# TengdaHan/DPC

Measured on AMD Instinct MI355X. Metric: clips/sec (train step, B x8x3x5xHxW), higher is better.
Workload: dtype bf16; 1 GPU; cfg2: resnet18 2d3d, img_dim 128, seq_len 5, num_seq 8, pred_step 3, batch 128/GPU, full train step (fwd+CE/top-k+bwd+all-reduce+Adam); global_batch=128, parallelism=dp1, init=reference init, random, launch=hipGraph replay, streams=2

## Files before the change

### dpc_amd/_lib.py

```python
from __future__ import annotations

import ctypes as C
import os
from typing import Optional

import torch

_HERE = os.path.dirname(os.path.abspath(__file__))
HIP_LIB_PATH = os.path.join(_HERE, "libdpc_hip.so")
EMU_LIB_PATH = os.path.join(os.path.dirname(_HERE), "tests", "simt_emu", "libdpc_emu.so")

F32, BF16 = 0, 1
ERR_ARG, ERR_LAUNCH, ERR_UNSUPPORTED = -1, -2, -3
ABI_VERSION = 2


def dtype_code(dt: torch.dtype) -> int:
    if dt == torch.float32:
        return F32
    if dt == torch.bfloat16:
        return BF16
    raise TypeError(f"unsupported dtype {dt}")


class ConvDesc(C.Structure):
    _fields_ = [(n, C.c_int32) for n in (
        "dtype_in", "dtype_out", "mode", "N", "RT", "RH", "RW", "ST", "SH", "SW", "Ci", "src_ld",
        "Co", "ldw", "ldo", "KT", "KH", "KW", "st", "sh", "sw", "pt", "ph", "pw")]


class GruChainDesc(C.Structure):
    _fields_ = ([(n, C.c_int32) for n in ("dtype", "M", "D", "SQ", "P", "n_agg", "n_steps", "reserved")] +
                [("p_drop", C.c_float), ("reserved2", C.c_uint32), ("seed", C.c_uint64)] +
                [(n, C.c_void_p) for n in ("step_dev", "drop_masks", "packed", "bias_u", "bias_r", "bias_o", "bias_1", "bias_2",
                                           "X_all", "H_all", "HR_all", "U_all", "R_all", "O_all", "P1_all", "pred",
                                           "d_pred", "G_all", "dP1", "dP2", "d_x", "ws", "d_hlast")])


class LcHeadDesc(C.Structure):
    _fields_ = ([(n, C.c_int32) for n in ("dtype", "B", "SQ", "D", "num_class", "train")] +
                [("p_drop", C.c_float), ("momentum", C.c_float), ("eps", C.c_float), ("reserved", C.c_uint32), ("seed", C.c_uint64)] +
                [(n, C.c_void_p) for n in ("step_dev", "drop_mask", "h_last", "bn_weight", "bn_bias", "bn_running_mean", "bn_running_var",
                                           "bn_num_batches", "fc_weight", "fc_bias", "target", "ctx", "xhat", "bn_out", "y", "stat",
                                           "logits", "dlogits", "row_ws", "result", "g_fc_weight", "g_fc_bias", "g_bn_weight",
                                           "g_bn_bias", "dctx", "d_hlast", "d_bn_out")])


class AdamSegment(C.Structure):
    _fields_ = [("begin", C.c_int64), ("end", C.c_int64), ("lr", C.c_float), ("weight_decay", C.c_float), ("active", C.c_int32),
                ("reserved", C.c_int32)]


ADAM_MAX_SEGMENTS = 512


class GradState(C.Structure):
    _fields_ = [("sumsq", C.c_double), ("norm", C.c_float), ("coef", C.c_float), ("skip", C.c_int32), ("n_skipped", C.c_int32),
                ("n_clipped", C.c_int32), ("reserved", C.c_int32)]


GRAD_PARTIALS = 1024
ACCUM_ADD, ACCUM_FINISH = 0, 1


class LambSegment(C.Structure):
    _fields_ = [("begin", C.c_int64), ("end", C.c_int64), ("lr", C.c_float), ("weight_decay", C.c_float), ("active", C.c_int32),
                ("adapt", C.c_int32), ("chunk0", C.c_int32), ("n_chunks", C.c_int32), ("reserved", C.c_int32 * 2)]


class LambChunk(C.Structure):
    _fields_ = [("begin", C.c_int64), ("len", C.c_int32), ("seg", C.c_int32)]


class LambRecord(C.Structure):
    _fields_ = [("sum_p2", C.c_double), ("sum_u2", C.c_double), ("pnorm", C.c_float), ("unorm", C.c_float), ("ratio", C.c_float),
                ("reserved", C.c_int32)]


LAMB_CHUNK = 4096

LR_CONSTANT, LR_COSINE, LR_LINEAR, LR_MULTISTEP = 0, 1, 2, 3
LR_MAX_MILESTONES = 8


class LrSchedule(C.Structure):
    _fields_ = [("kind", C.c_int32), ("warmup_steps", C.c_int32), ("total_steps", C.c_int32), ("n_milestones", C.c_int32),
                ("min_mult", C.c_double), ("gamma", C.c_double), ("milestones", C.c_int32 * LR_MAX_MILESTONES)]


class LrState(C.Structure):
    _fields_ = [("mult", C.c_float), ("k", C.c_int32), ("reserved", C.c_int32 * 2)]


class ConvEpilogue(C.Structure):
    _fields_ = [(n, C.c_void_p) for n in ("addend", "addend_mask", "bn_raw", "bn_mask", "bn_mean", "bn_invstd", "stats")]


class Resample(C.Structure):
    _fields_ = [("xb", C.c_void_p), ("xk", C.c_void_p), ("yb", C.c_void_p), ("yk", C.c_void_p), ("ksx", C.c_int32), ("ksy", C.c_int32)]


class RecipeDesc(C.Structure):
    _fields_ = ([(n, C.c_double) for n in ("sized_p", "gray_p", "jitter_p", "brightness", "contrast", "saturation", "hue")] +
                [("flip_code", C.c_int32), ("flags", C.c_int32)])


RECIPE_JITTER_CONSISTENT, RECIPE_SCALE_AFTER_SIZED = 1, 2


def recipe_slots(n_frames: int) -> int:
    return 58 + 9 * n_frames


class PackEntry(C.Structure):
    _fields_ = [("in_", C.c_void_p), ("out", C.c_void_p), ("d0", C.c_int32), ("d1", C.c_int32), ("d2", C.c_int32), ("block0", C.c_int32),
                ("s0", C.c_int64), ("s1", C.c_int64), ("s2", C.c_int64)]


class Copy2dEntry(C.Structure):
    _fields_ = [("src", C.c_void_p), ("dst", C.c_void_p), ("src_ld", C.c_int64), ("dst_ld", C.c_int64), ("rows", C.c_int32), ("cols", C.c_int32),
                ("block0", C.c_int32), ("pad", C.c_int32)]


class DpcError(RuntimeError):
    pass


_vp, _i32, _i64, _f32, _f64 = C.c_void_p, C.c_int32, C.c_int64, C.c_float, C.c_double
_SIGS = {
    "dpc_abi_version": [],
    "dpc_conv_stats_rows": [C.POINTER(ConvDesc)],
    "dpc_conv_igemm": [C.POINTER(ConvDesc), _vp, _vp, _vp, _vp, _vp, _vp],
    "dpc_conv_igemm_ex": [C.POINTER(ConvDesc), _vp, _vp, _vp, C.POINTER(ConvEpilogue), _vp],
    "dpc_gemm_nt_splitk": [_i32, _i32, _i32, _i32, _vp, _i32, _vp, _i32, _vp, C.POINTER(_i32), _vp],
    "dpc_gemm_tn_splitk": [_i32, _i32, _i32, _i32, _vp, _i32, _vp, _i32, _vp, C.POINTER(_i32), _vp],
    "dpc_conv_wgrad": [C.POINTER(ConvDesc), _vp, _vp, _i32, _vp, C.POINTER(_i32), _vp],
    "dpc_conv_plan": [C.POINTER(ConvDesc), _i32, _i32, _i32, C.c_char_p, _i32],
    "dpc_last_kernel": [C.c_char_p, _i32],
    "dpc_set_reserved_cus": [_i32],
    "dpc_set_f32_matmul": [_i32],
    "dpc_diag_squat": [_i32, _i32, _i32, _i32, _i32, _vp, _i64, _vp, _vp, _vp],
    "dpc_pack3d": [_vp, _vp, _i32, _i32, _i32, _i32, _i64, _i64, _i64, _vp],
    "dpc_pack3d_multi": [_vp, _i32, _i32, _i32, _vp],
    "dpc_reduce_unpack": [_vp, _i32, _vp, _i32, _i32, _i32, _i64, _i64, _i64, _i32, _vp],
    "dpc_transpose2d_bf16x2": [_vp, _vp, _i32, _vp, _vp, _i32, _i32, _i32, _vp],
    "dpc_transpose2d": [_vp, _i32, _i32, _vp, _i32, _i32, _i32, _i32, _vp],
    "dpc_pack_input_s2d": [_vp, _vp, _i32, _i32, _i32, _i32, _i32, _vp],
    "dpc_synthetic_input": [_vp, _vp, _i32, _i32, _i32, _i32, _i32, C.c_uint64, _vp, _vp],
    "dpc_synthetic_labels": [_vp, _i32, _i32, C.c_uint64, _vp, _vp],
    "dpc_pack_stem_weight": [_vp, _vp, _i32, _i32, _vp],
    "dpc_unpack_stem_wgrad": [_vp, _i32, _vp, _i32, _vp],
    "dpc_bn_finalize": [_vp, _i32, _i32, _f64, _vp, _vp, _f32, _vp, _vp, _vp, _vp, _vp],
    "dpc_bn_apply": [_vp, _vp, _i32, _i64, _i32, _vp, _vp, _vp, _vp, _vp, _i32, _vp, _vp],
    "dpc_bn_bwd_reduce": [_vp, _vp, _vp, _vp, _i32, _i64, _i32, _vp, _vp, _i32, _vp, C.POINTER(_i32), _vp],
    "dpc_bn_bwd_finalize": [_vp, _i32, _i32, _f64, _vp, _vp, _vp, _vp],
    "dpc_bn_bwd_apply": [_vp, _vp, _vp, _vp, _i32, _i64, _i32, _vp, _vp, _vp, _vp, _i32, _vp, _vp, _vp],
    "dpc_bn_relu_maxpool_fwd": [_vp, _i32, _i32, _i32, _i32, _i32, _vp, _vp, _vp, _vp, _vp],
    "dpc_maxpool_bwd": [_vp, _vp, _i32, _i32, _i32, _i32, _i32, _vp, _vp],
    "dpc_tpool_split_fwd": [_vp, _i32, _i32, _i32, _i32, _i32, _i32, _i32, _vp, _vp, _vp],
    "dpc_tpool_split_bwd": [_vp, _vp, _vp, _i32, _i32, _i32, _i32, _i32, _i32, _i32, _vp, _vp],
    "dpc_colsum": [_vp, _i32, _i32, _i32, _i32, _vp, _i32, _vp, _i64, _vp],
    "dpc_pool_bn_bwd_reduce": [_vp, _vp, _vp, _i32, _i32, _i32, _i32, _i32, _vp, _vp, _vp, C.POINTER(_i32), _vp],
    "dpc_pooled_bn_bwd_reduce": [_vp, _vp, _vp, _i32, _i64, _i32, _vp, _vp, _vp, C.POINTER(_i32), _vp],
    "dpc_pool_bn_bwd_apply": [_vp, _vp, _vp, _i32, _i32, _i32, _i32, _i32, _vp, _vp, _vp, _vp, _vp, _vp],
    "dpc_mask_gen": [_vp, _i32, _i32, _i32, _vp],
    "dpc_ce_topk": [_vp, _i32, _i32, _i32, _vp, _vp, _vp, _i32, _i32, _vp],
    "dpc_ce_topk_bf16": [_vp, _i32, _i32, _i32, _vp, _vp, _vp, _i32, _vp],
    "dpc_step_advance": [_vp, _vp, _f64, _f64, _vp],
    "dpc_adam_dev": [_vp, _vp, _vp, _vp, _i64, _f32, _f64, _f64, _f32, _f32, _vp, _f32, _vp],
    "dpc_adam_groups_dev": [_vp, _vp, _vp, _vp, _i64, _vp, _i32, _f64, _f64, _f32, _vp, _f32, _vp],
    "dpc_grad_sumsq": [_vp, _i64, _vp, _i32, _vp, _vp],
    "dpc_grad_verdict": [_vp, _i32, _f64, _i32, _vp, _vp],
    "dpc_step_advance_gated": [_vp, _vp, _f64, _f64, _vp, _vp],
    "dpc_adam_dev_ex": [_vp, _vp, _vp, _vp, _i64, _f32, _f64, _f64, _f32, _f32, _vp, _f32, _vp, _vp],
    "dpc_adam_groups_dev_ex": [_vp, _vp, _vp, _vp, _i64, _vp, _i32, _f64, _f64, _f32, _vp, _f32, _vp, _vp],
    "dpc_grad_scale": [_vp, _i64, _vp, _i32, _vp, _vp],
    "dpc_grad_accumulate": [_vp, _vp, _i64, _i64, _i64, _vp, _i32, _i32, _f32, _vp],
    "dpc_adam_dev_ema": [_vp, _vp, _vp, _vp, _i64, _f32, _f64, _f64, _f32, _f32, _vp, _f32, _vp, _vp, _vp, _f32, _vp],
    "dpc_adam_groups_dev_ema": [_vp, _vp, _vp, _vp, _i64, _vp, _i32, _f64, _f64, _f32, _vp, _f32, _vp, _vp, _vp, _f32, _vp],
    "dpc_arena_swap": [_vp, _vp, _i64, _vp],
    "dpc_step_advance_sched": [_vp, _vp, _f64, _f64, _vp, C.POINTER(LrSchedule), _vp, _vp],
    "dpc_adam_dev_sched": [_vp, _vp, _vp, _vp, _i64, _f32, _f64, _f64, _f32, _f32, _vp, _f32, _vp, _vp, _vp, _f32, _vp, _vp],
    "dpc_adam_groups_dev_sched": [_vp, _vp, _vp, _vp, _i64, _vp, _i32, _f64, _f64, _f32, _vp, _f32, _vp, _vp, _vp, _f32, _vp, _vp],
    "dpc_adamw_dev": [_vp, _vp, _vp, _vp, _i64, _f32, _f64, _f64, _f32, _f32, _vp, _f32, _vp, _vp, _vp, _f32, _vp, _vp],
    "dpc_adamw_groups_dev": [_vp, _vp, _vp, _vp, _i64, _vp, _i32, _f64, _f64, _f32, _vp, _f32, _vp, _vp, _vp, _f32, _vp, _vp],
    "dpc_lamb_build_chunks": [C.POINTER(LambSegment), _i32, _i64, C.POINTER(LambChunk), _i32],
    "dpc_lamb_moments": [_vp, _vp, _vp, _vp, _i64, _vp, _i32, _vp, _i32, _f64, _f64, _f32, _vp, _f32, _vp, _vp, _vp],
    "dpc_lamb_ratios": [_vp, _i32, _vp, _i32, _vp, _vp, _vp],
    "dpc_lamb_apply": [_vp, _vp, _vp, _i64, _vp, _i32, _vp, _i32, _f32, _vp, _vp, _vp, _vp, _vp, _f32, _vp, _vp],
    "dpc_counter_advance": [_vp, _vp],
    "dpc_copy2d_f32": [_vp, _i64, _vp, _i64, _i32, _i32, _vp],
    "dpc_copy2d_multi": [_vp, _i32, _i32, _vp],
    "dpc_dropout_mask": [_vp, _i64, _f32, C.c_uint64, _vp, _vp],
    "dpc_gru_pack": [_vp, _vp, _vp, _vp, _vp, _i32, _i32, _vp, _vp],
    "dpc_gru_chain_fwd": [C.POINTER(GruChainDesc), _vp],
    "dpc_gru_chain_bwd": [C.POINTER(GruChainDesc), _vp],
    "dpc_score_ws_floats": [_i32, _i32, C.POINTER(_i64), C.POINTER(_i64)],
    "dpc_score_fwd": [_vp, _vp, _i32, _i32, _vp, _vp, _vp, _vp, _vp, _vp],
    "dpc_score_bwd": [_vp, _vp, _vp, _i32, _i32, _i32, _vp, _i32, _vp, _vp],
    "dpc_ce_finalize": [_vp, _i32, _vp, _vp],
    "dpc_bn_finalize_running": [_vp, _i32, _i32, _f64, _vp, _vp, _f32, _vp, _vp, _vp, _vp, _vp, _vp, _vp, _f32, _vp],
    "dpc_bn_eval_coeffs": [_vp, _vp, _vp, _vp, _f32, _i32, _vp, _vp, _vp, _vp, _vp],
    "dpc_relu_tpool_fwd": [_vp, _i32, _i32, _i32, _i32, _i32, _i32, _vp, _vp],
    "dpc_relu_tpool_bwd": [_vp, _vp, _i32, _i32, _i32, _i32, _i32, _i32, _vp, _vp],
    "dpc_lc_head_fwd": [C.POINTER(LcHeadDesc), _vp],
    "dpc_lc_head_bwd": [C.POINTER(LcHeadDesc), _vp],
    "dpc_frames_to_input": [_vp, _i32, _i32, _i32, _i32, _vp, _vp, _i32, _i32, _i32, _i32, _i32, _vp, _vp, _i32, _i32,
                            C.POINTER(C.c_float), C.POINTER(C.c_float), _vp, _vp, _i32, _vp],
    "dpc_frames_to_input_ex": [_vp, _i32, _i32, _i32, _i32, _vp, _vp, _i32, _i32, _i32, _i32, _i32, C.POINTER(Resample), _vp, _vp, _vp,
                               C.POINTER(C.c_float), C.POINTER(C.c_float), _vp, _vp, _i32, _vp],
    "dpc_video_windows_to_input": [_vp, _i32, _i32, _i32, _i32, _vp, _i32, _i32, _i32, _i32, _i32, C.POINTER(Resample),
                                   C.POINTER(C.c_float), C.POINTER(C.c_float), _vp, _vp, _i32, _vp],
    "dpc_store_to_input": [_vp, _i32, _i64, _i32, _i32, _vp, _vp, _i32, _i32, _i32, _i32, _i32, C.POINTER(Resample), _vp, _vp, _vp,
                           C.POINTER(C.c_float), C.POINTER(C.c_float), _vp, _vp, _i32, _vp, _vp],
    "dpc_draw_recipe": [C.POINTER(RecipeDesc), _vp, _vp, _vp, _i32, _i32, _i32, _i32, _i32, _i32, _i32, _i32, _i32, _vp, C.c_uint64, _vp, _vp,
                        _vp, _vp, _vp, _vp, _vp, _vp, _vp, _vp, _vp],
    "dpc_draw_recipe_ex": [C.POINTER(RecipeDesc), _vp, _vp, _vp, _vp, _vp, _i32, _i32, _i32, _i32, _i32, _i32, _i32, _i32, _i32, _vp, C.c_uint64,
                           _vp, _vp, _vp, _vp, _vp, _vp, _vp, _vp, _vp, _vp, _vp, _vp],
    "dpc_lc_test_accumulate": [_vp, _i32, _i32, _i32, _i32, _vp, _vp, _vp, _vp],
    "dpc_lc_test_finish": [_vp, _vp, _vp, _i32, _i32, _vp, _vp, _vp, _vp, _vp],
    "dpc_embed_accumulate": [_vp, _i32, _i32, _i32, _i32, _vp, _vp, _vp],
    "dpc_embed_finish": [_vp, _vp, _i32, _f32, _vp, _vp],
    "dpc_knn_ws_bytes": [_i32, _i32, _i32],
    "dpc_knn_topk": [_vp, _i32, _i32, _vp, _i32, _i32, _i32, _i32, _vp, _i32, _vp, _vp, _vp, _i64, _vp],
    "dpc_knn_recall": [_vp, _i32, _i32, _vp, _vp, _i32, _i32, _vp, _i32, _vp, _vp, _vp, _vp],
    "dpc_stem_wgrad_fused": [C.POINTER(ConvDesc), _vp, _vp, _vp, _vp, _vp, _vp, _vp, _vp, _vp, C.POINTER(_i32), _vp],
    "dpc_adam": [_vp, _vp, _vp, _vp, _i64, _f32, _f32, _f32, _f32, _f32, _f32, _f32, _f32, _vp],
}


class Lib:

    def __init__(self, path: str, kind: str):
        if not os.path.exists(path):
            raise DpcError(
                f"{path} not found: build it with `make` (or __graft_entry__.build()); "
                "dpc_amd has no CPU/eager fallback")
        self.kind = kind
        self.path = path
        self.c = C.CDLL(path)
        self._bound = {}
        if self.call("dpc_abi_version") != ABI_VERSION:
            raise DpcError("ABI version mismatch")

    def _fn(self, name: str):
        fn = self._bound.get(name)
        if fn is None:
            fn = getattr(self.c, name)
            fn.argtypes = _SIGS[name]
            fn.restype = C.c_int
            self._bound[name] = fn
        return fn

    def missing_symbols(self):
        return [n for n in _SIGS if not hasattr(self.c, n)]

    def stream(self) -> C.c_void_p:
        if self.kind == "hip":
            return C.c_void_p(torch.cuda.current_stream().cuda_stream)
        return C.c_void_p(0)

    def call(self, name: str, *args) -> int:
        conv = [C.c_void_p(a.data_ptr()) if isinstance(a, torch.Tensor) else a for a in args]
        rc = self._fn(name)(*conv)
        if rc < 0:
            raise DpcError(f"{name} failed with code {rc}")
        return rc


PLAN_IGEMM, PLAN_WGRAD, PLAN_ADDEND, PLAN_STATS, PLAN_ADDEND_MASK, PLAN_BNRED = 0, 1, 1, 2, 4, 8


def conv_plan(lib: "Lib", desc: ConvDesc, op: int = PLAN_IGEMM, addend: bool = False, stats: bool = False, dy_ld: int = 0,
              addend_mask: bool = False, bnred: bool = False) -> str:
    buf = C.create_string_buffer(192)
    flags = ((PLAN_ADDEND if addend else 0) | (PLAN_STATS if stats else 0) | (PLAN_ADDEND_MASK if addend_mask else 0) |
             (PLAN_BNRED if bnred else 0))
    rc = lib._fn("dpc_conv_plan")(C.byref(desc), op, flags, dy_ld or desc.Co, buf, 192)
    if rc == -3:
        return ""
    if rc < 0:
        raise DpcError(f"dpc_conv_plan failed with code {rc}")
    return buf.value.decode()


def last_kernel(lib: "Lib") -> str:
    buf = C.create_string_buffer(192)
    lib.call("dpc_last_kernel", buf, 192)
    return buf.value.decode()
# ... 27 lines not shown
```

### dpc_amd/csrc/conv_wgrad.hip

```cpp
#include "conv_common.h"
#include <stdlib.h>

struct WgradParams {
    GatherGeom g;
    const void* src;
    const void* dy;
    float* part;
    int Co, dy_ld;
    int nks, kcps;
    int ntm, ntn;
    int x6;
};

template <class T> struct Transposer;
template <> struct Transposer<float> {
    static __device__ __forceinline__ void run(const u32x4 (&v)[4], u32x4 (&o)[4]) {
        DPC_UNROLL
        for (int c = 0; c < 4; ++c) {
            u32x4 t = {v[0][c], v[1][c], v[2][c], v[3][c]};
            o[c] = t;
        }
    }
};
template <> struct Transposer<bf16_t> {
// ... 79 lines not shown
        u_pg[i] = loc / per_row;
        u_tp[i] = decode_k(g, tile_n * TN + u_cu[i] * E);
    }

    f32x16 acc[MI][NT];
    DPC_UNROLL
    for (int i = 0; i < MI; ++i)
        DPC_UNROLL
        for (int j = 0; j < NT; ++j)
            DPC_UNROLL
            for (int r = 0; r < 16; ++r) acc[i][j][r] = 0.f;

    const char* const zero = (const char*)dpc_zero16;
    u32x4 rv[NU][E];
    auto load_chunk = [&](int chunk) {
        DPC_UNROLL
        for (int i = 0; i < NU; ++i) {
            const int m_first = chunk * BKP + u_pg[i] * E;
            if (!u_on[i]) continue;
            if (u_isA[i]) {
                const int co = tile_m * TM + u_cu[i] * E;
                const bool cok = co + E <= p.dy_ld && co < p.Co;
                const char* a = (const char*)p.dy + ((long long)m_first * p.dy_ld + co) * esz;
                DPC_UNROLL
                for (int e = 0; e < E; ++e) {
                    const bool ok = cok && m_first + e < g.M;
                    rv[i][e] = *(const u32x4*)(ok ? a + (long long)e * p.dy_ld * esz : zero);
                }
            } else if (ROWFAST) {
                const RowIt it = rowit_decode(g, m_first < g.M ? m_first : 0);
                const TapPos& tp = u_tp[i];
                const int ti = it.rt * g.st - g.pt + tp.kt, hi = it.rh * g.sh - g.ph + tp.kh;
                const int wi0 = it.rw * g.sw - g.pw + tp.kw;
                const bool rok = tp.ok && m_first < g.M && (unsigned)ti < (unsigned)g.ST && (unsigned)hi < (unsigned)g.SH;
                const long long off0 = ((((long long)(it.n * g.ST + ti) * g.SH + hi) * g.SW) + wi0) * g.src_ld + tp.ci;
                const char* a = (const char*)p.src + off0 * esz;
                const long long step = (long long)g.sw * g.src_ld * esz;
                DPC_UNROLL
                for (int e = 0; e < E; ++e) {
                    const bool ok = rok && (unsigned)(wi0 + e * g.sw) < (unsigned)g.SW;
                    rv[i][e] = *(const u32x4*)(ok ? a + e * step : zero);
                }
            } else {
                RowIt it = rowit_decode(g, m_first < g.M ? m_first : 0);
                DPC_UNROLL
                for (int e = 0; e < E; ++e) {
                    const int m = m_first + e;
                    long long off = gather_off(g, rowit_pos(g, it), u_tp[i]);
                    if (m >= g.M) off = -1;
                    rv[i][e] = *(const u32x4*)(off >= 0 ? (const char*)p.src + off * esz : zero);
                    rowit_next(g, it);
                }
            }
        }
    };
    auto store_chunk = [&](int buf) {
        unsigned char* As = lds + buf * (TM + TN) * 128;
        unsigned char* Bs = As + TM * 128;
        DPC_UNROLL
        for (int i = 0; i < NU; ++i) {
            if (!u_on[i]) continue;
            u32x4 o[E];
            Transposer<T>::run(rv[i], o);
            unsigned char* base = u_isA[i] ? As : Bs;
            DPC_UNROLL
            for (int c = 0; c < E; ++c) *(u32x4*)(base + lds_unit_off3(u_cu[i] * E + c, u_pg[i])) = o[c];
        }
    };

    if (c_begin < c_end) {
        load_chunk(c_begin);
        store_chunk(0);
    }
    __syncthreads();
    for (int ch = c_begin; ch < c_end; ++ch) {
        const int buf = (ch - c_begin) & 1;
        if (ch + 1 < c_end) load_chunk(ch + 1);
        const unsigned char* As = lds + buf * (TM + TN) * 128;
        const unsigned char* Bs = As + TM * 128;
        bool done = false;
        if constexpr (sizeof(T) == 4) {
            if (p.x6) {
                DPC_UNROLL
                for (int kp = 0; kp < 2; ++kp) {
                    const int u0 = 4 * kp + lhi, u1 = u0 + 2;
                    Split3 sa[MI], sb[NT];
                    DPC_UNROLL
                    for (int i = 0; i < MI; ++i)
                        sa[i] = split3_f32x8(*(const u32x4*)(As + lds_unit_off3(wm * (TM / 2) + i * 32 + l31, u0)),
                                             *(const u32x4*)(As + lds_unit_off3(wm * (TM / 2) + i * 32 + l31, u1)));
                    DPC_UNROLL
                    for (int j = 0; j < NT; ++j)
                        sb[j] = split3_f32x8(*(const u32x4*)(Bs + lds_unit_off3(wn * (TN / 2) + j * 32 + l31, u0)),
                                             *(const u32x4*)(Bs + lds_unit_off3(wn * (TN / 2) + j * 32 + l31, u1)));
                    DPC_UNROLL
                    for (int i = 0; i < MI; ++i)
                        DPC_UNROLL
                        for (int j = 0; j < NT; ++j) acc[i][j] = mfma_f32x6(sa[i], sb[j], acc[i][j]);
                }
                done = true;
            }
        }
        if (!done) {
        DPC_UNROLL
        for (int kk = 0; kk < 4; ++kk) {
            const int unit = 2 * kk + lhi;
            u32x4 fa[MI], fb[NT];
            DPC_UNROLL
            for (int i = 0; i < MI; ++i) fa[i] = *(const u32x4*)(As + lds_unit_off3(wm * (TM / 2) + i * 32 + l31, unit));
            DPC_UNROLL
            for (int j = 0; j < NT; ++j) fb[j] = *(const u32x4*)(Bs + lds_unit_off3(wn * (TN / 2) + j * 32 + l31, unit));
            DPC_UNROLL
            for (int i = 0; i < MI; ++i)
                DPC_UNROLL
                for (int j = 0; j < NT; ++j) acc[i][j] = mfma_unit<T>(fa[i], fb[j], acc[i][j]);
        }
        }
        if (ch + 1 < c_end) store_chunk(buf ^ 1);
        __syncthreads();
    }

    DPC_UNROLL
    for (int j = 0; j < NT; ++j) {
        const int col = tile_n * TN + wn * (TN / 2) + j * 32 + l31;
        if (col < g.Kp) {
            DPC_UNROLL
            for (int i = 0; i < MI; ++i)
                DPC_UNROLL
                for (int r = 0; r < 16; ++r) {
                    const int row = tile_m * TM + wm * (TM / 2) + i * 32 + (r & 3) + 8 * (r >> 2) + 4 * lhi;
                    if (row < p.Co) p.part[((long long)ks * p.Co + row) * g.Kp + col] = acc[i][j][r];
                }
        }
    }
}


struct Wgrad2Params {
    GatherGeom g;
    const void* src;
    const void* dy;
    float* part;
    int Co, dy_ld;
    int nks, kcps;
    int ntm, ntn;
    int lRW, lRH;
    int RWm, RHm;
    int Mv;
    int xcd_remap;
    int x6;
};

template <class T, int NWM, int NWN, bool PU>
__global__ __launch_bounds__(64 * NWM * NWN, 2) void wgrad2_kernel(Wgrad2Params p) {
    constexpr int E = Elt<T>::PER16;
    constexpr int ESZ = (int)sizeof(T);
    constexpr int BKP = 8 * E;
    constexpr int RB = 64 * ESZ;
    constexpr int SPR = RB / 16;
    constexpr int RPI = 64 / SPR;
    constexpr int SUB = BKP * RB;
    constexpr int NW = NWM * NWN, NS = NWM + NWN;
    constexpr int RR = (8 + NW - 1) / NW;
    constexpr int STAGE = NS * SUB;
    constexpr int TM = 64 * NWM, TN = 64 * NWN;
    __shared__ __attribute__((aligned(1024))) unsigned char lds[2 * STAGE];

    const GatherGeom& g = p.g;
    const int tid = threadIdx.x;
    const int lane = tid & 63;
#ifdef DPC_SIMT_EMU
    const int wv = tid >> 6;
#else
    const int wv = __builtin_amdgcn_readfirstlane(tid >> 6);
#endif
    const int wm = wv / NWN, wn = wv % NWN;
    const int l31 = lane & 31, lhi = lane >> 5;
    int id = blockIdx.x;
    if (p.xcd_remap) {
        const int nwg = gridDim.x, q = nwg >> 3, r = nwg & 7, x = id & 7;
        id = (x < r ? x * (q + 1) : r * (q + 1) + (x - r) * q) + (id >> 3);
    }
    const int tile_n = id % p.ntn; id /= p.ntn;
    const int tile_m = id % p.ntm;
    const int ks = id / p.ntm;

    const int nchunks_total = (p.Mv + BKP - 1) / BKP;
    const int c_begin = ks * p.kcps;
    const int c_end = (c_begin + p.kcps < nchunks_total) ? c_begin + p.kcps : nchunks_total;

    const int rowlane = lane / SPR, pslot = lane % SPR;
    const int lslot = (ESZ == 2) ? (pslot ^ (2 * (rowlane & 3))) : pslot;
    const int cch = lslot * E;
    int r_row[RR], r_w[RR], r_h[RR], r_q[RR], r_dh[RR], r_real[RR];
    bool r_wok[RR];
    DPC_UNROLL
    for (int rr = 0; rr < RR; ++rr) {
        const int r = (wv + rr * NW) * RPI + rowlane;
        r_row[rr] = r;
        r_w[rr] = (r & p.RWm) * g.sw - g.pw;
        r_h[rr] = ((r >> p.lRW) & p.RHm) * g.sh - g.ph;
        r_q[rr] = r >> (p.lRW + p.lRH);
        r_dh[rr] = r >> p.lRW;
        r_wok[rr] = (r & p.RWm) < g.RW;
        r_real[rr] = r_dh[rr] * g.RW + (r & p.RWm);
    }
    int a_off[RR][NWM];
    DPC_UNROLL
    for (int sa = 0; sa < NWM; ++sa) {
        const int co = tile_m * TM + sa * 64 + cch;
        const bool ok = co + E <= p.dy_ld && co < p.Co;
        DPC_UNROLL
        for (int rr = 0; rr < RR; ++rr) a_off[rr][sa] = ok && r_wok[rr] ? (r_real[rr] * p.dy_ld + co) * ESZ : -1;
    }
    TapPos tp[NWN];
    int b_off[RR][NWN], b_h[RR][NWN];
    const int ldb = g.src_ld * ESZ;
    DPC_UNROLL
    for (int sb = 0; sb < NWN; ++sb) {
        tp[sb] = decode_k(g, tile_n * TN + sb * 64 + cch);
        DPC_UNROLL
        for (int rr = 0; rr < RR; ++rr) {
            const int wi = r_w[rr] + tp[sb].kw;
            const bool ok = tp[sb].ok && (unsigned)wi < (unsigned)g.SW;
            b_h[rr][sb] = ok ? r_h[rr] + tp[sb].kh : (1 << 29);
            b_off[rr][sb] = ((tp[sb].kt * g.SH + r_h[rr] + tp[sb].kh) * g.SW + wi) * ldb + tp[sb].ci * ESZ;
        }
    }

    f32x16 acc[2][2];
    DPC_UNROLL
    for (int i = 0; i < 2; ++i)
        DPC_UNROLL
        for (int j = 0; j < 2; ++j)
            DPC_UNROLL
            for (int r = 0; r < 16; ++r) acc[i][j][r] = 0.f;

    const char* const zero = (const char*)dpc_zero16;
    auto issue = [&](int chunk, int buf) {
        const int m0 = chunk * BKP;
        unsigned char* stage = lds + buf * STAGE;
        const unsigned q0 = (unsigned)m0 >> (p.lRW + p.lRH);
        const int h0v = PU ? (int)(((unsigned)m0 >> p.lRW) & (unsigned)p.RHm) : 0;
        const int h0 = h0v * g.sh;
        const long long m0r = PU ? ((long long)q0 * g.RH + h0v) * g.RW : (long long)m0;
        const char* abase = (const char*)p.dy + m0r * p.dy_ld * ESZ;
        const char* bbase = (const char*)p.src;
        bool tv[NWN];
        if (PU) {
            const unsigned n = fdiv(q0, g.dRT);
            const int t00 = ((int)q0 - (int)n * g.RT) * g.st - g.pt;
            bbase += (long long)(((int)n * g.ST + t00) * g.SH + h0) * g.SW * ldb;
            DPC_UNROLL
            for (int sb = 0; sb < NWN; ++sb) tv[sb] = (unsigned)(t00 + tp[sb].kt) < (unsigned)g.ST;
        }
        DPC_UNROLL
        for (int rr = 0; rr < RR; ++rr) {
            const int rg = wv + rr * NW;
            if (rg < 8) {
                const bool mok = m0 + r_row[rr] < p.Mv && r_wok[rr] && (!PU || h0v + r_dh[rr] < g.RH);
                DPC_UNROLL
                for (int sa = 0; sa < NWM; ++sa)
                    glds16((mok & (a_off[rr][sa] >= 0)) ? abase + a_off[rr][sa] : zero, stage + sa * SUB + rg * 1024, lane);
                if (PU) {
                    DPC_UNROLL
                    for (int sb = 0; sb < NWN; ++sb) {
                        const bool ok = mok & tv[sb] & ((unsigned)(h0 + b_h[rr][sb]) < (unsigned)g.SH);
                        glds16(ok ? bbase + b_off[rr][sb] : zero, stage + (NWM + sb) * SUB + rg * 1024, lane);
                    }
                } else {
                    const unsigned q = q0 + (unsigned)r_q[rr];
                    const unsigned n = fdiv(q, g.dRT);
                    const int t0 = ((int)q - (int)n * g.RT) * g.st - g.pt;
                    const char* pb = bbase + (long long)(((int)n * g.ST + t0) * g.SH) * g.SW * ldb;
                    DPC_UNROLL
                    for (int sb = 0; sb < NWN; ++sb) {
                        const bool ok = mok & ((unsigned)(t0 + tp[sb].kt) < (unsigned)g.ST) & ((unsigned)b_h[rr][sb] < (unsigned)g.SH);
                        glds16(ok ? pb + b_off[rr][sb] : zero, stage + (NWM + sb) * SUB + rg * 1024, lane);
                    }
                }
            }
        }
    };

    int fo[2];
    if (ESZ == 2) {
        const int gq = lane >> 4, s16 = lane & 15;
        DPC_UNROLL
        for (int i = 0; i < 2; ++i) {
            const int colb = (i * 32 + (gq & 1) * 16 + 4 * (s16 & 3)) * 2;
            fo[i] = ((gq >> 1) * 8 + (s16 >> 2)) * RB + ((((colb >> 4) ^ (2 * (s16 >> 2))) & 7) << 4) + (colb & 15);
        }
    } else {
        DPC_UNROLL
        for (int i = 0; i < 2; ++i) fo[i] = lhi * RB + (i * 32 + l31) * 4;
    }

    auto compute = [&](int buf) {
        const unsigned char* As = lds + buf * STAGE + wm * SUB;
        const unsigned char* Bs = lds + buf * STAGE + (NWM + wn) * SUB;
#ifndef DPC_SIMT_EMU
        if constexpr (ESZ == 2) {
            constexpr int LOOKAHEAD = 4;
            const uint32_t as = (uint32_t)(uintptr_t)(__attribute__((address_space(3))) const unsigned char*)As;
            const uint32_t bs = (uint32_t)(uintptr_t)(__attribute__((address_space(3))) const unsigned char*)Bs;
            uint32_t ad[2][2];
            DPC_UNROLL
            for (int i = 0; i < 2; ++i) { ad[0][i] = as + fo[i]; ad[1][i] = bs + fo[i]; }
            u32x2 lo[2][2][2], hi[2][2][2];
            auto load = [&](auto Ic) {
                constexpr int I = decltype(Ic)::value;
                constexpr int kk = I / 4, r4 = I % 4;
                constexpr int op = (r4 == 1 || r4 == 2) ? 1 : 0, fr = (r4 >= 2) ? 1 : 0;
                asm volatile("ds_read_b64_tr_b16 %0, %1 offset:%2" : "=v"(lo[kk & 1][op][fr]) : "v"(ad[op][fr]), "n"((kk * 16) * RB) : "memory");
                __builtin_amdgcn_sched_barrier(0);
                asm volatile("ds_read_b64_tr_b16 %0, %1 offset:%2" : "=v"(hi[kk & 1][op][fr]) : "v"(ad[op][fr]), "n"((kk * 16 + 4) * RB) : "memory");
                __builtin_amdgcn_sched_barrier(0);
            };
            __builtin_amdgcn_sched_barrier(0);
            static_for<16>([&](auto Mc) {
                constexpr int m = decltype(Mc)::value;
                constexpr int kk = m / 4, q = m % 4;
                constexpr int idx = 4 * kk + (q == 0 ? 1 : q == 1 ? 2 : 3);
                constexpr int idx_prev = m == 0 ? -1 : (q == 0 ? 4 * (kk - 1) + 3 : 4 * kk + (q == 1 ? 1 : q == 2 ? 2 : 3));
                constexpr int f_prev = m == 0 ? 0 : (idx_prev + 1 + LOOKAHEAD < 16 ? idx_prev + 1 + LOOKAHEAD : 16);
                constexpr int f_now = idx + 1 + LOOKAHEAD < 16 ? idx + 1 + LOOKAHEAD : 16;
                static_for<f_now - f_prev>([&](auto Dc) { load(std::integral_constant<int, f_prev + decltype(Dc)::value>{}); });
                asm volatile("s_waitcnt lgkmcnt(%0)" ::"n"(2 * (f_now - idx - 1)) : "memory");
                __builtin_amdgcn_sched_barrier(0);
                constexpr int i = q >> 1, j = q & 1, s = kk & 1;
                const u32x4 av = {lo[s][0][i][0], lo[s][0][i][1], hi[s][0][i][0], hi[s][0][i][1]};
                const u32x4 bv = {lo[s][1][j][0], lo[s][1][j][1], hi[s][1][j][0], hi[s][1][j][1]};
                acc[i][j] = mfma_32x32x16_bf16(av, bv, acc[i][j]);
                __builtin_amdgcn_sched_barrier(0);
            });
            return;
        }
#endif
        if (ESZ == 2) {
            DPC_UNROLL
            for (int kk = 0; kk < 4; ++kk) {
                u32x4 fa[2], fb[2];
                DPC_UNROLL
                for (int i = 0; i < 2; ++i) {
                    const u32x2 a0 = lds_read_tr16(As + fo[i] + (kk * 16) * RB);
                    const u32x2 a1 = lds_read_tr16(As + fo[i] + (kk * 16 + 4) * RB);
                    const u32x2 b0 = lds_read_tr16(Bs + fo[i] + (kk * 16) * RB);
                    const u32x2 b1 = lds_read_tr16(Bs + fo[i] + (kk * 16 + 4) * RB);
                    u32x4 ta = {a0[0], a0[1], a1[0], a1[1]};
                    u32x4 tb = {b0[0], b0[1], b1[0], b1[1]};
                    fa[i] = ta; fb[i] = tb;
                }
                DPC_UNROLL
                for (int i = 0; i < 2; ++i)
                    DPC_UNROLL
                    for (int j = 0; j < 2; ++j) acc[i][j] = mfma_32x32x16_bf16(fa[i], fb[j], acc[i][j]);
            }
        } else if (p.x6) {
            DPC_UNROLL
            for (int s16 = 0; s16 < BKP / 16; ++s16) {
                Split3 sa[2], sb[2];
                DPC_UNROLL
                for (int i = 0; i < 2; ++i) {
                    float xa[8], xb[8];
                    DPC_UNROLL
                    for (int e = 0; e < 8; ++e) {
                        xa[e] = *(const float*)(As + fo[i] + 2 * (8 * s16 + e) * RB);
                        xb[e] = *(const float*)(Bs + fo[i] + 2 * (8 * s16 + e) * RB);
                    }
                    sa[i] = split3_f32(xa);
                    sb[i] = split3_f32(xb);
                }
                DPC_UNROLL
                for (int i = 0; i < 2; ++i)
                    DPC_UNROLL
                    for (int j = 0; j < 2; ++j) acc[i][j] = mfma_f32x6(sa[i], sb[j], acc[i][j]);
            }
        } else {
            DPC_UNROLL
            for (int s2 = 0; s2 < BKP / 2; ++s2) {
                float fa[2], fb[2];
                DPC_UNROLL
                for (int i = 0; i < 2; ++i) {
                    fa[i] = *(const float*)(As + fo[i] + 2 * s2 * RB);
                    fb[i] = *(const float*)(Bs + fo[i] + 2 * s2 * RB);
                }
                DPC_UNROLL
                for (int i = 0; i < 2; ++i)
                    DPC_UNROLL
                    for (int j = 0; j < 2; ++j) acc[i][j] = mfma_32x32x2_f32(fa[i], fb[j], acc[i][j]);
            }
        }
    };

    if (c_begin < c_end) issue(c_begin, 0);
    __syncthreads();
    for (int ch = c_begin; ch < c_end; ++ch) {
        const int buf = (ch - c_begin) & 1;
        if (ch + 1 < c_end) issue(ch + 1, buf ^ 1);
        compute(buf);
        __syncthreads();
    }

    DPC_UNROLL
    for (int j = 0; j < 2; ++j) {
        const int col = tile_n * TN + wn * 64 + j * 32 + l31;
        if (col < g.Kp) {
            DPC_UNROLL
            for (int i = 0; i < 2; ++i)
                DPC_UNROLL
                for (int r = 0; r < 16; ++r) {
                    const int row = tile_m * TM + wm * 64 + i * 32 + (r & 3) + 8 * (r >> 2) + 4 * lhi;
                    if (row < p.Co) p.part[((long long)ks * p.Co + row) * g.Kp + col] = acc[i][j][r];
                }
        }
    }
}

template <class T, int NWM, int NWN>
static int launch_wgrad2_t(const Wgrad2Params& p, bool pu, hipStream_t stream) {
    dim3 grid((unsigned)(p.ntm * p.ntn * p.nks)), block(64 * NWM * NWN);
    dpc_plan_detail("T=%s nwm=%d nwn=%d padded=%d", sizeof(T) == 2 ? "bf16" : "f32", NWM, NWN,
                    (int)(((p.RWm + 1) != p.g.RW) || ((p.RHm + 1) != p.g.RH)));
    if (pu) {
        DPC_LAUNCH((wgrad2_kernel<T, NWM, NWN, true>), grid, block, stream, p);
    } else {
        DPC_LAUNCH((wgrad2_kernel<T, NWM, NWN, false>), grid, block, stream, p);
    }
    return dpc_launch_status();
}

template <class T>
static int launch_wgrad2(const Wgrad2Params& p, int nwm, int nwn, bool pu, hipStream_t stream) {
    if (nwm == 1 && nwn == 3) return launch_wgrad2_t<T, 1, 3>(p, pu, stream);
    if (nwm == 1 && nwn == 4) return launch_wgrad2_t<T, 1, 4>(p, pu, stream);
    if (nwm == 2 && nwn == 2) return launch_wgrad2_t<T, 2, 2>(p, pu, stream);
    return launch_wgrad2_t<T, 2, 3>(p, pu, stream);
}

template <class T, bool RF>
static int launch_wgrad_rf(const WgradParams& p, int tm, int tn, hipStream_t stream) {
    dim3 grid((unsigned)(p.ntm * p.ntn * p.nks)), block(256);
    dpc_plan_detail("T=%s", sizeof(T) == 2 ? "bf16" : "f32");
    if (tm == 64 && tn == 64) {
        DPC_LAUNCH((wgrad_kernel<T, 64, 64, RF>), grid, block, stream, p);
    } else if (tm == 64 && tn == 128) {
        DPC_LAUNCH((wgrad_kernel<T, 64, 128, RF>), grid, block, stream, p);
    } else {
        DPC_LAUNCH((wgrad_kernel<T, 128, 128, RF>), grid, block, stream, p);
    }
    return dpc_launch_status();
}

template <class T>
static int launch_wgrad(const WgradParams& p, int tm, int tn, hipStream_t stream) {
    if (p.g.RW % Elt<T>::PER16 == 0) return launch_wgrad_rf<T, true>(p, tm, tn, stream);
    return launch_wgrad_rf<T, false>(p, tm, tn, stream);
}

extern "C" int dpc_conv_wgrad(const dpc_conv_desc* d, const void* src, const void* dy, int32_t dy_ld,
                              float* part, int32_t* nsplit, dpc_stream_t stream_) {
    hipStream_t stream = (hipStream_t)stream_;
    WgradParams p;
    p.x6 = dpc_f32_matmul_mode();
    if (!d || d->mode != 0) return DPC_ERR_ARG;
    int rc = make_gather_geom(d, &p.g);
    if (rc) return rc;
    const int per16 = d->dtype_in == DPC_BF16 ? 8 : 4;
    if (dy_ld % per16 || dy_ld < d->Co) return DPC_ERR_UNSUPPORTED;
    rc = dpc_wgrad_patch_try(d, src, dy, dy_ld, part, nsplit, stream);
    if (rc != 1) return rc;
    rc = dpc_wgrad_stem_try(d, src, dy, dy_ld, part, nsplit, stream);
    if (rc != 1) return rc;
    const int bkp = 8 * per16;
    int rwp = 1, rhp = 1;
    while (rwp < d->RW) rwp <<= 1;
    while (rhp < d->RH) rhp <<= 1;
    const bool padded = rwp != d->RW || rhp != d->RH;
    const long long mv = (long long)d->N * d->RT * rhp * rwp;
    static const int pad_on = getenv("DPC_WGRAD2_PAD") ? atoi(getenv("DPC_WGRAD2_PAD")) : 1;
    const bool v2 = bkp % rwp == 0 && mv < (1ll << 31) &&
                    (!padded || (pad_on && (rwp * rhp) % bkp == 0 && (long long)d->RW * d->RH * 10 >= (long long)rwp * rhp * 6));
    const int lrw = ilog2_exact(rwp), lrh = ilog2_exact(rhp);
    const int nchunks = (int)(((v2 ? mv : (long long)p.g.M) + bkp - 1) / bkp);
    int tm, tn, nwm = 0, nwn = 0;
    if (v2) {
        nwm = d->Co > 64 ? 2 : 1;
        const int na = nwm == 1 ? 4 : 2, nb = 3;
        const int pa = (p.g.Kp + 64 * na - 1) / (64 * na) * (64 * na), pb = (p.g.Kp + 64 * nb - 1) / (64 * nb) * (64 * nb);
        nwn = (pb < pa) ? nb : na;
        tm = 64 * nwm; tn = 64 * nwn;
    } else {
        tm = d->Co > 64 ? 128 : 64;
        tn = (p.g.Kp >= 128 || tm == 128) ? 128 : 64;
    }
    p.ntm = (d->Co + tm - 1) / tm;
    p.ntn = (p.g.Kp + tn - 1) / tn;
    static const int min_chunks = getenv("DPC_WGRAD_MINCHUNKS") ? atoi(getenv("DPC_WGRAD_MINCHUNKS")) : 16;
    static const int target_blocks = getenv("DPC_WGRAD_BLOCKS") ? atoi(getenv("DPC_WGRAD_BLOCKS")) : 512;
    int want = target_blocks / (p.ntm * p.ntn);
    if (want > nchunks / min_chunks) want = nchunks / min_chunks;
    if (want < 1) want = 1;
    if (want > nchunks) want = nchunks;
    p.kcps = (nchunks + want - 1) / want;
    p.nks = (nchunks + p.kcps - 1) / p.kcps;
    if (nsplit) *nsplit = p.nks;
    if (!part) return DPC_OK;
    if (!src || !dy) return DPC_ERR_ARG;
    p.src = src; p.dy = dy; p.part = part; p.Co = d->Co; p.dy_ld = dy_ld;
    if (v2) {
        Wgrad2Params q;
        q.g = p.g; q.src = src; q.dy = dy; q.part = part; q.Co = d->Co; q.dy_ld = dy_ld;
        q.nks = p.nks; q.kcps = p.kcps; q.ntm = p.ntm; q.ntn = p.ntn; q.lRW = lrw; q.lRH = lrh;
        q.RWm = rwp - 1; q.RHm = rhp - 1; q.Mv = (int)mv; q.x6 = p.x6;
        q.xcd_remap = 1;
        const bool pu = (rwp * rhp) % bkp == 0;
        if (d->dtype_in == DPC_F32) return launch_wgrad2<float>(q, nwm, nwn, pu, stream);
        return launch_wgrad2<bf16_t>(q, nwm, nwn, pu, stream);
    }
    if (d->dtype_in == DPC_F32) return launch_wgrad<float>(p, tm, tn, stream);
    return launch_wgrad<bf16_t>(p, tm, tn, stream);
}
```

### dpc_amd/csrc/gru.hip

```cpp
#include "dpc_rt.h"
#include "../../include/dpc_hip.h"
#include "philox.h"

static inline unsigned grid_for(long long n, int block = 256, int cap = 8192) {
    long long g = (n + block - 1) / block;
    if (g < 1) g = 1;
    if (g > cap) g = cap;
    return (unsigned)g;
}

template <class T>
__global__ __launch_bounds__(256) void colsum_kernel(const T* x, int ld, int M, int D, float* out, int rows_per_y) {
    __shared__ float red[8][32];
    const int col = blockIdx.x * 32 + (threadIdx.x & 31);
    const int rg = threadIdx.x >> 5;
    const int m0 = blockIdx.y * rows_per_y;
    const int m1 = (m0 + rows_per_y < M) ? m0 + rows_per_y : M;
    float s = 0.f;
    if (col < D)
        for (int m = m0 + rg; m < m1; m += 8) s += Elt<T>::to_f32(x[(long long)m * ld + col]);
    red[rg][threadIdx.x & 31] = s;
    __syncthreads();
    if (threadIdx.x < 32 && col < D) {
        float t = 0.f;
        DPC_UNROLL
        for (int g = 0; g < 8; ++g) t += red[g][threadIdx.x];
        out[(long long)blockIdx.y * D + col] = t;
    }
}

__global__ void colsum_finish_kernel(const float* ws, int ny, int D, float* out, int accumulate) {
    const int d = blockIdx.x * blockDim.x + threadIdx.x;
    if (d >= D) return;
    float t = 0.f;
    for (int y = 0; y < ny; ++y) t += ws[(long long)y * D + d];
    out[d] = accumulate ? out[d] + t : t;
}

extern "C" int dpc_colsum(const void* x, int32_t dtype, int32_t ld, int32_t M, int32_t D, float* out, int32_t accumulate,
                          float* ws, int64_t ws_floats, dpc_stream_t stream_) {
    hipStream_t stream = (hipStream_t)stream_;
    if (!x || !out || M <= 0 || D <= 0 || ld < D) return DPC_ERR_ARG;
    int ny = (M + 255) / 256;
    if (ny > 64) ny = 64;
    if (!ws || ws_floats < (long long)ny * D) return DPC_ERR_ARG;
    const int rpy = (M + ny - 1) / ny;
    dim3 grid((D + 31) / 32, ny), block(256);
    if (dtype == DPC_F32) {
        DPC_LAUNCH((colsum_kernel<float>), grid, block, stream, (const float*)x, ld, M, D, ws, rpy);
    } else if (dtype == DPC_BF16) {
        DPC_LAUNCH((colsum_kernel<bf16_t>), grid, block, stream, (const bf16_t*)x, ld, M, D, ws, rpy);
    } else {
        return DPC_ERR_ARG;
    }
    DPC_LAUNCH(colsum_finish_kernel, dim3((D + 255) / 256), dim3(256), stream, (const float*)ws, ny, D, out, accumulate);
    return dpc_launch_status();
}

__global__ void dropout_mask_kernel(float* mask, long long n4, long long n, unsigned long long seed, const int32_t* step_dev,
                                    uint32_t thresh24, float inv_keep) {
    const uint32_t step = (uint32_t)step_dev[0];
    for (long long i = (long long)blockIdx.x * blockDim.x + threadIdx.x; i < n4; i += (long long)gridDim.x * blockDim.x) {
        float k[4];
        dropout_keep4(seed, step, (uint32_t)i, thresh24, inv_keep, k);
        if (i * 4 + 4 <= n) {
            ((f32x4*)mask)[i] = f32x4{k[0], k[1], k[2], k[3]};
        } else {
            for (long long e = i * 4; e < n; ++e) mask[e] = k[e - i * 4];
        }
    }
}

extern "C" int dpc_dropout_mask(float* mask, int64_t n, float p, uint64_t seed, const int32_t* step_dev, dpc_stream_t stream_) {
    hipStream_t stream = (hipStream_t)stream_;
    if (!mask || n <= 0 || !step_dev || !(p >= 0.f) || !(p < 1.f) || n >= (1ll << 33)) return DPC_ERR_ARG;
    const long long n4 = (n + 3) / 4;
    DPC_LAUNCH(dropout_mask_kernel, dim3(grid_for(n4)), dim3(256), stream, mask, n4, (long long)n, (unsigned long long)seed, step_dev,
               dropout_thresh24(p), 1.f / (1.f - p));
    return dpc_launch_status();
}
```

### dpc_amd/csrc/pack.hip

```cpp
#include "dpc_rt.h"
#include "../../include/dpc_hip.h"

template <class TO>
__global__ void pack3d_kernel(const float* in, TO* out, int d0, int d1, int d2, long long s0, long long s1, long long s2) {
    const long long n = (long long)d0 * d1 * d2;
    for (long long i = (long long)blockIdx.x * blockDim.x + threadIdx.x; i < n; i += (long long)gridDim.x * blockDim.x) {
        const int i2 = (int)(i % d2);
        const long long q = i / d2;
        const int i1 = (int)(q % d1);
        const int i0 = (int)(q / d1);
        out[i] = Elt<TO>::from_f32(in[i0 * s0 + i1 * s1 + i2 * s2]);
    }
}

static inline unsigned grid_for(long long n, int block = 256, int cap = 4096) {
    long long g = (n + block - 1) / block;
    if (g < 1) g = 1;
    if (g > cap) g = cap;
    return (unsigned)g;
}

extern "C" int dpc_pack3d(const float* in, void* out, int32_t dtype_out, int32_t d0, int32_t d1, int32_t d2,
                          int64_t s0, int64_t s1, int64_t s2, dpc_stream_t stream_) {
    hipStream_t stream = (hipStream_t)stream_;
    if (!in || !out || d0 <= 0 || d1 <= 0 || d2 <= 0) return DPC_ERR_ARG;
    const long long n = (long long)d0 * d1 * d2;
    if (dtype_out == DPC_F32) {
        DPC_LAUNCH((pack3d_kernel<float>), dim3(grid_for(n)), dim3(256), stream, in, (float*)out, d0, d1, d2, (long long)s0, (long long)s1, (long long)s2);
    } else if (dtype_out == DPC_BF16) {
        DPC_LAUNCH((pack3d_kernel<bf16_t>), dim3(grid_for(n)), dim3(256), stream, in, (bf16_t*)out, d0, d1, d2, (long long)s0, (long long)s1, (long long)s2);
    } else {
        return DPC_ERR_ARG;
    }
    return dpc_launch_status();
}

template <class TO>
__global__ void pack3d_multi_kernel(const dpc_pack_entry* tab, int n_entries, TO* ) {
    int e = 0;
    while (e + 1 < n_entries && (int)blockIdx.x >= tab[e + 1].block0) ++e;
    const dpc_pack_entry t = tab[e];
    const long long n = (long long)t.d0 * t.d1 * t.d2;
    const int nblk = (e + 1 < n_entries ? tab[e + 1].block0 : (int)gridDim.x) - t.block0;
    const float* in = (const float*)t.in;
    TO* out = (TO*)t.out;
    constexpr int TJ = 64, TI_MAX = 64;
    __shared__ float tile[TJ][TI_MAX + 1];
    if (t.s1 == 1 && t.d1 <= TI_MAX && t.d1 > 1) {
        const int nj = (t.d2 + TJ - 1) / TJ;
        const int ntiles = t.d0 * nj;
        for (int tl = (int)blockIdx.x - t.block0; tl < ntiles; tl += nblk) {
            const int i0 = tl / nj, j0 = (tl - i0 * nj) * TJ;
            const int jn = t.d2 - j0 < TJ ? t.d2 - j0 : TJ;
            const float* src = in + (long long)i0 * t.s0 + (long long)j0 * t.s2;
            for (int idx = threadIdx.x; idx < jn * t.d1; idx += blockDim.x) {
                const int j = idx / t.d1, i1 = idx - j * t.d1;
                tile[j][i1] = src[(long long)j * t.s2 + i1];
            }
            __syncthreads();
            TO* dst = out + ((long long)i0 * t.d1) * t.d2 + j0;
            for (int idx = threadIdx.x; idx < t.d1 * TJ; idx += blockDim.x) {
                const int i1 = idx / TJ, j = idx - i1 * TJ;
                if (j < jn) dst[(long long)i1 * t.d2 + j] = Elt<TO>::from_f32(tile[j][i1]);
            }
            __syncthreads();
        }
        return;
    }
    for (long long i = (long long)((int)blockIdx.x - t.block0) * blockDim.x + threadIdx.x; i < n; i += (long long)nblk * blockDim.x) {
        const int i2 = (int)(i % t.d2);
        const long long q = i / t.d2;
        const int i1 = (int)(q % t.d1);
        const int i0 = (int)(q / t.d1);
        out[i] = Elt<TO>::from_f32(in[i0 * t.s0 + i1 * t.s1 + i2 * t.s2]);
    }
}

extern "C" int dpc_pack3d_multi(const dpc_pack_entry* table_dev, int32_t n_entries, int32_t total_blocks, int32_t dtype_out,
                                dpc_stream_t stream_) {
    hipStream_t stream = (hipStream_t)stream_;
    if (!table_dev || n_entries <= 0 || total_blocks < n_entries) return DPC_ERR_ARG;
    if (dtype_out == DPC_F32) {
        DPC_LAUNCH((pack3d_multi_kernel<float>), dim3((unsigned)total_blocks), dim3(256), stream, table_dev, n_entries, (float*)nullptr);
    } else if (dtype_out == DPC_BF16) {
        DPC_LAUNCH((pack3d_multi_kernel<bf16_t>), dim3((unsigned)total_blocks), dim3(256), stream, table_dev, n_entries, (bf16_t*)nullptr);
    } else {
        return DPC_ERR_ARG;
    }
    return dpc_launch_status();
}

__global__ __launch_bounds__(256) void reduce_unpack_kernel(const float* part, int nsplit, float* out, int d0, int d1, int d2, long long s0,
                                     long long s1, long long s2, int accumulate) {
    __shared__ float red[8][32];
    const long long n = (long long)d0 * d1 * d2;
    const int ol = threadIdx.x & 31, sl = threadIdx.x >> 5;
    const long long i = (long long)blockIdx.x * 32 + ol;
    float s = 0.f;
    if (i < n)
        for (int k = sl; k < nsplit; k += 8) s += part[(long long)k * n + i];
    red[sl][ol] = s;
    __syncthreads();
    if (sl == 0 && i < n) {
        float t = 0.f;
        DPC_UNROLL
        for (int k = 0; k < 8; ++k) t += red[k][ol];
        const int i2 = (int)(i % d2);
        const long long q = i / d2;
        const int i1 = (int)(q % d1);
        const int i0 = (int)(q / d1);
        float* o = out + i0 * s0 + i1 * s1 + i2 * s2;
        *o = accumulate ? (*o + t) : t;
    }
}

__global__ __launch_bounds__(256) void reduce_unpack4_kernel(const float* part, int nsplit, float* out, int d0, int d1, int d2, long long s0,
                                      long long s1, long long s2, int accumulate) {
    __shared__ float red[8][32][4];
    const long long n = (long long)d0 * d1 * d2;
    const int ol = threadIdx.x & 31, sl = threadIdx.x >> 5;
    const long long i = ((long long)blockIdx.x * 32 + ol) * 4;
    float acc[8][4];
    DPC_UNROLL
    for (int j = 0; j < 8; ++j)
        DPC_UNROLL
        for (int e = 0; e < 4; ++e) acc[j][e] = 0.f;
    if (i < n) {
        int k = sl;
        for (; k + 56 < nsplit; k += 64) {
            u32x4 v[8];
            DPC_UNROLL
            for (int j = 0; j < 8; ++j) v[j] = *(const u32x4*)(part + (long long)(k + 8 * j) * n + i);
            DPC_UNROLL
            for (int j = 0; j < 8; ++j)
                DPC_UNROLL
                for (int e = 0; e < 4; ++e) acc[j][e] += unit_get<float>(v[j], e);
        }
        DPC_UNROLL
        for (int j = 0; j < 8; ++j)
            if (k + 8 * j < nsplit) {
                const u32x4 v0 = *(const u32x4*)(part + (long long)(k + 8 * j) * n + i);
                DPC_UNROLL
                for (int e = 0; e < 4; ++e) acc[j][e] += unit_get<float>(v0, e);
            }
    }
    float a[4], b[4];
    DPC_UNROLL
    for (int e = 0; e < 4; ++e) {
        a[e] = (acc[0][e] + acc[1][e]) + (acc[2][e] + acc[3][e]);
        b[e] = (acc[4][e] + acc[5][e]) + (acc[6][e] + acc[7][e]);
    }
    DPC_UNROLL
    for (int e = 0; e < 4; ++e) red[sl][ol][e] = a[e] + b[e];
    __syncthreads();
    if (sl == 0 && i < n) {
        const int i2 = (int)(i % d2);
        const long long q = i / d2;
        const int i1 = (int)(q % d1);
        const int i0 = (int)(q / d1);
        float* o = out + i0 * s0 + i1 * s1 + i2 * s2;
        DPC_UNROLL
        for (int e = 0; e < 4; ++e) {
            float t = 0.f;
            DPC_UNROLL
            for (int k = 0; k < 8; ++k) t += red[k][ol][e];
            o[e * s2] = accumulate ? (o[e * s2] + t) : t;
        }
    }
}

template <int NS>
__global__ __launch_bounds__(256) void reduce_unpack_few_kernel(const float* part, float* out, int d0, int d1, int d2, long long s0, long long s1,
                                                                long long s2, int accumulate) {
    const long long n = (long long)d0 * d1 * d2;
    const long long i = ((long long)blockIdx.x * 256 + threadIdx.x) * 4;
    if (i >= n) return;
    u32x4 v[NS];
    DPC_UNROLL
    for (int k = 0; k < NS; ++k) v[k] = *(const u32x4*)(part + (long long)k * n + i);
    const int i2 = (int)(i % d2);
    const long long q = i / d2;
    const int i1 = (int)(q % d1);
    const int i0 = (int)(q / d1);
    float* o = out + i0 * s0 + i1 * s1 + i2 * s2;
    DPC_UNROLL
    for (int e = 0; e < 4; ++e) {
        float t = 0.f;
        DPC_UNROLL
        for (int k = 0; k < NS; ++k) t += unit_get<float>(v[k], e);
        o[e * s2] = accumulate ? (o[e * s2] + t) : t;
    }
}

constexpr int RUT_CW = 64, RUT_MAXT = 32;
__global__ __launch_bounds__(256) void reduce_unpack_t_kernel(const float* part, int nsplit, float* out, int Co, int taps, int Ci, int accumulate) {
    __shared__ float tile[RUT_CW * (RUT_MAXT + 1)];
    const int co = blockIdx.x, c0 = blockIdx.y * RUT_CW;
    const int cw = Ci - c0 < RUT_CW ? Ci - c0 : RUT_CW;
    const int ldt = taps | 1;
    const long long n = (long long)Co * taps * Ci;
    const float* base = part + ((long long)co * taps) * Ci + c0;
    for (int e = threadIdx.x; e < taps * RUT_CW; e += 256) {
        const int tap = e / RUT_CW, c = e - tap * RUT_CW;
        if (c < cw) {
            const float* p = base + (long long)tap * Ci + c;
            float a0 = 0.f, a1 = 0.f, a2 = 0.f, a3 = 0.f;
            int k = 0;
            for (; k + 4 <= nsplit; k += 4) {
                a0 += p[(long long)k * n];
                a1 += p[(long long)(k + 1) * n];
                a2 += p[(long long)(k + 2) * n];
                a3 += p[(long long)(k + 3) * n];
            }
            for (; k < nsplit; ++k) a0 += p[(long long)k * n];
            tile[c * ldt + tap] = (a0 + a1) + (a2 + a3);
        }
    }
    __syncthreads();
    float* o = out + ((long long)co * Ci + c0) * taps;
    for (int j = threadIdx.x; j < cw * taps; j += 256) {
        const int c = j / taps, tap = j - c * taps;
        const float v = tile[c * ldt + tap];
        o[j] = accumulate ? o[j] + v : v;
    }
}

extern "C" int dpc_reduce_unpack(const float* part, int32_t nsplit, float* out, int32_t d0, int32_t d1, int32_t d2,
                                 int64_t s0, int64_t s1, int64_t s2, int32_t accumulate, dpc_stream_t stream_) {
    hipStream_t stream = (hipStream_t)stream_;
    if (!part || !out || nsplit <= 0 || d0 <= 0 || d1 <= 0 || d2 <= 0) return DPC_ERR_ARG;
    if (nsplit <= 16 && d1 > 1 && d1 <= RUT_MAXT && s1 == 1 && s2 == d1 && s0 == (int64_t)d1 * d2 && d0 <= 65535) {
        DPC_LAUNCH(reduce_unpack_t_kernel, dim3((unsigned)d0, (unsigned)((d2 + RUT_CW - 1) / RUT_CW)), dim3(256), stream, part, nsplit, out, d0, d1, d2,
                   accumulate);
        return dpc_launch_status();
    }
    const long long n = (long long)d0 * d1 * d2;
    if (d2 % 4 == 0 && ((uintptr_t)part % 16) == 0 && nsplit <= 8) {
        const dim3 grid((unsigned)((n / 4 + 255) / 256)), block(256);
#define DPC_RUF(NS) case NS: DPC_LAUNCH((reduce_unpack_few_kernel<NS>), grid, block, stream, part, out, d0, d1, d2, (long long)s0, (long long)s1, (long long)s2, accumulate); break
        switch (nsplit) { DPC_RUF(1); DPC_RUF(2); DPC_RUF(3); DPC_RUF(4); DPC_RUF(5); DPC_RUF(6); DPC_RUF(7); DPC_RUF(8); }
#undef DPC_RUF
        return dpc_launch_status();
    }
    if (d2 % 4 == 0 && ((uintptr_t)part % 16) == 0) {
        DPC_LAUNCH(reduce_unpack4_kernel, dim3((unsigned)((n / 4 + 31) / 32)), dim3(256), stream, part, nsplit, out, d0, d1, d2, (long long)s0, (long long)s1,
                   (long long)s2, accumulate);
        return dpc_launch_status();
    }
    DPC_LAUNCH(reduce_unpack_kernel, dim3((unsigned)((n + 31) / 32)), dim3(256), stream, part, nsplit, out, d0, d1, d2, (long long)s0, (long long)s1, (long long)s2, accumulate);
    return dpc_launch_status();
}

template <class TI, class TO>
__global__ void transpose2d_kernel(const TI* in, int ld_in, TO* out, int ld_out, int rows, int cols) {
    __shared__ float tile[32][33];
    const int bx = blockIdx.x * 32, by = blockIdx.y * 32;
    const int tx = threadIdx.x & 31, ty = threadIdx.x >> 5;
    for (int r = ty; r < 32; r += 8) {
        const int row = by + r, col = bx + tx;
        tile[r][tx] = (row < rows && col < cols) ? Elt<TI>::to_f32(in[(long long)row * ld_in + col]) : 0.f;
    }
    __syncthreads();
    for (int r = ty; r < 32; r += 8) {
        const int orow = bx + r, ocol = by + tx;
        if (orow < cols && ocol < rows) out[(long long)orow * ld_out + ocol] = Elt<TO>::from_f32(tile[tx][r]);
    }
}

extern "C" int dpc_transpose2d(const void* in, int32_t dtype_in, int32_t ld_in, void* out, int32_t dtype_out,
                               int32_t ld_out, int32_t rows, int32_t cols, dpc_stream_t stream_) {
    hipStream_t stream = (hipStream_t)stream_;
    if (!in || !out || rows <= 0 || cols <= 0) return DPC_ERR_ARG;
    dim3 grid((cols + 31) / 32, (rows + 31) / 32), block(256);
    if (dtype_in == DPC_F32 && dtype_out == DPC_F32) {
        DPC_LAUNCH((transpose2d_kernel<float, float>), grid, block, stream, (const float*)in, ld_in, (float*)out, ld_out, rows, cols);
    } else if (dtype_in == DPC_F32 && dtype_out == DPC_BF16) {
        DPC_LAUNCH((transpose2d_kernel<float, bf16_t>), grid, block, stream, (const float*)in, ld_in, (bf16_t*)out, ld_out, rows, cols);
    } else if (dtype_in == DPC_BF16 && dtype_out == DPC_BF16) {
        DPC_LAUNCH((transpose2d_kernel<bf16_t, bf16_t>), grid, block, stream, (const bf16_t*)in, ld_in, (bf16_t*)out, ld_out, rows, cols);
    } else if (dtype_in == DPC_BF16 && dtype_out == DPC_F32) {
        DPC_LAUNCH((transpose2d_kernel<bf16_t, float>), grid, block, stream, (const bf16_t*)in, ld_in, (float*)out, ld_out, rows, cols);
    } else {
        return DPC_ERR_ARG;
    }
    return dpc_launch_status();
}

__global__ __launch_bounds__(256) void transpose2d_bf16x2_kernel(const bf16_t* in0, const bf16_t* in1, int ld_in, bf16_t* out0, bf16_t* out1, int ld_out,
                                                                int rows, int cols) {
    __shared__ unsigned short tile[64][66];
    const bf16_t* in = blockIdx.z ? in1 : in0;
    bf16_t* out = blockIdx.z ? out1 : out0;
    const int bx = blockIdx.x * 64, by = blockIdx.y * 64;
    const int t = threadIdx.x;
    {
        DPC_UNROLL
        for (int it = 0; it < 2; ++it) {
            const int r = (t >> 3) + 32 * it, u = t & 7;
            const int row = by + r, col = bx + u * 8;
            u32x4 v = {0u, 0u, 0u, 0u};
            if (row < rows && col + 7 < cols) v = *(const u32x4*)(in + (long long)row * ld_in + col);
            else if (row < rows) {
                unsigned short e[8];
                DPC_UNROLL
                for (int k = 0; k < 8; ++k) e[k] = col + k < cols ? *(const unsigned short*)(in + (long long)row * ld_in + col + k) : (unsigned short)0;
                v[0] = e[0] | ((unsigned)e[1] << 16); v[1] = e[2] | ((unsigned)e[3] << 16);
                v[2] = e[4] | ((unsigned)e[5] << 16); v[3] = e[6] | ((unsigned)e[7] << 16);
            }
            DPC_UNROLL
            for (int k = 0; k < 4; ++k) {
                tile[r][u * 8 + 2 * k] = (unsigned short)(v[k] & 0xffffu);
                tile[r][u * 8 + 2 * k + 1] = (unsigned short)(v[k] >> 16);
            }
        }
    }
    __syncthreads();
    DPC_UNROLL
    for (int it = 0; it < 2; ++it) {
        const int c = (t >> 3) + 32 * it, u = t & 7;
        const int orow = bx + c, ocol = by + u * 8;
        if (orow >= cols) continue;
        unsigned short e[8];
        DPC_UNROLL
        for (int k = 0; k < 8; ++k) e[k] = tile[u * 8 + k][c];
        if (ocol + 7 < rows) {
            const u32x4 v = {e[0] | ((unsigned)e[1] << 16), e[2] | ((unsigned)e[3] << 16), e[4] | ((unsigned)e[5] << 16), e[6] | ((unsigned)e[7] << 16)};
            *(u32x4*)(out + (long long)orow * ld_out + ocol) = v;
        } else {
            DPC_UNROLL
            for (int k = 0; k < 8; ++k)
                if (ocol + k < rows) *(unsigned short*)(out + (long long)orow * ld_out + ocol + k) = e[k];
        }
    }
}

extern "C" int dpc_transpose2d_bf16x2(const void* in0, const void* in1, int32_t ld_in, void* out0, void* out1, int32_t ld_out, int32_t rows,
                                      int32_t cols, dpc_stream_t stream_) {
    hipStream_t stream = (hipStream_t)stream_;
    if (!in0 || !out0 || rows <= 0 || cols <= 0 || ld_in < cols || ld_out < rows) return DPC_ERR_ARG;
    if (ld_in % 8 || ld_out % 8 || (((uintptr_t)in0 | (uintptr_t)in1 | (uintptr_t)out0 | (uintptr_t)out1) % 16)) return DPC_ERR_UNSUPPORTED;
    dim3 grid((cols + 63) / 64, (rows + 63) / 64, in1 ? 2 : 1), block(256);
    DPC_LAUNCH(transpose2d_bf16x2_kernel, grid, block, stream, (const bf16_t*)in0, (const bf16_t*)in1, ld_in, (bf16_t*)out0, (bf16_t*)out1, ld_out, rows, cols);
    return dpc_launch_status();
}

template <class TO>
__global__ void pack_input_s2d_kernel(const float* in, TO* out, int BN, int T, int H, int W, int rev) {
    const int Hb = H / 2, Wb = W / 2;
    const long long cells = (long long)BN * T * Hb * Wb;
    const long long stride = (long long)gridDim.x * blockDim.x, first = (long long)blockIdx.x * blockDim.x + threadIdx.x;
    const long long nsweep = first < cells ? (cells - 1 - first) / stride + 1 : 0;
    for (long long k = 0; k < nsweep; ++k) {
        const long long i = first + (rev ? nsweep - 1 - k : k) * stride;
        const unsigned ci = (unsigned)i;
        const unsigned q1 = ci / (unsigned)Wb;
        const int wb = (int)(ci - q1 * (unsigned)Wb);
        const unsigned q2 = q1 / (unsigned)Hb;
        const int hb = (int)(q1 - q2 * (unsigned)Hb);
        const unsigned n_ = q2 / (unsigned)T;
        const int t = (int)(q2 - n_ * (unsigned)T);
        const int n = (int)n_;
        float v[16];
        DPC_UNROLL
        for (int k = 12; k < 16; ++k) v[k] = 0.f;
        DPC_UNROLL
        for (int c = 0; c < 3; ++c)
            DPC_UNROLL
            for (int sy = 0; sy < 2; ++sy) {
                const float* p = in + ((((long long)n * 3 + c) * T + t) * H + (2 * hb + sy)) * W + 2 * wb;
                const float2 x = *(const float2*)p;
                v[(sy * 2 + 0) * 3 + c] = x.x;
                v[(sy * 2 + 1) * 3 + c] = x.y;
            }
        u32x4* o = (u32x4*)(out + i * 16);
        constexpr int EPO = Elt<TO>::PER16;
        DPC_UNROLL
        for (int k = 0; k < 16 / EPO; ++k) o[k] = unit_pack<TO>(v + k * EPO);
    }
}

extern "C" int dpc_pack_input_s2d(const float* block, void* out, int32_t dtype_out, int32_t BN, int32_t T, int32_t H,
                                  int32_t W, dpc_stream_t stream_) {
    hipStream_t stream = (hipStream_t)stream_;
    if (!block || !out || BN <= 0 || T <= 0 || H <= 0 || W <= 0) return DPC_ERR_ARG;
    if ((H & 1) || (W & 1)) return DPC_ERR_UNSUPPORTED;
    const long long cells = (long long)BN * T * (H / 2) * (W / 2);
    static const int rev = getenv("DPC_PACK_REV") ? atoi(getenv("DPC_PACK_REV")) : 0;
    static const int cap = getenv("DPC_PACK_GRID") ? atoi(getenv("DPC_PACK_GRID")) : 16384;
    if (rev && (dtype_out == DPC_F32 || dtype_out == DPC_BF16)) dpc_plan_detail("rev");
    if (dtype_out == DPC_F32) {
        DPC_LAUNCH((pack_input_s2d_kernel<float>), dim3(grid_for(cells, 256, cap)), dim3(256), stream, block, (float*)out, BN, T, H, W, rev);
    } else if (dtype_out == DPC_BF16) {
        DPC_LAUNCH((pack_input_s2d_kernel<bf16_t>), dim3(grid_for(cells, 256, cap)), dim3(256), stream, block, (bf16_t*)out, BN, T, H, W, rev);
    } else {
        return DPC_ERR_ARG;
    }
    return dpc_launch_status();
}

template <class TO>
__global__ void pack_stem_weight_kernel(const float* w, TO* out, int Co) {
    const int n = Co * 256;
// ... 124 lines not shown
```

### dpc_amd/engine.py

```python
from __future__ import annotations

import atexit
import contextlib
import ctypes as C
import os
import weakref
import math
from typing import Dict, List, Optional, Sequence, Tuple

import torch

from . import _lib as L
from .plan import LAYER_PLAN, LAYER_WIDTH, block_geometry, fold_decision, out_shape_of, unit_descs, walk_blocks
BN_EPS = 1e-5


def param_shapes(network: str, widths: Sequence[int] = LAYER_WIDTH) -> "Dict[str, Tuple[int, ...]]":
    D = widths[3]
    out: Dict[str, Tuple[int, ...]] = {}
    out["backbone.conv1.weight"] = (widths[0], 3, 1, 7, 7)
    out["backbone.bn1.weight"] = (widths[0],)
    out["backbone.bn1.bias"] = (widths[0],)
    for pre, cin, planes, is3d, stride, has_ds, _ in walk_blocks(network, widths):
        pre, k = "backbone." + pre, block_geometry(is3d, stride)[0]
        out[pre + "conv1.weight"] = (planes, cin) + k
        out[pre + "bn1.weight"] = (planes,)
        out[pre + "bn1.bias"] = (planes,)
        out[pre + "conv2.weight"] = (planes, planes) + k
        out[pre + "bn2.weight"] = (planes,)
        out[pre + "bn2.bias"] = (planes,)
        if has_ds:
            out[pre + "downsample.0.weight"] = (planes, cin, 1, 1, 1)
            out[pre + "downsample.1.weight"] = (planes,)
            out[pre + "downsample.1.bias"] = (planes,)
    for gate in ("reset_gate", "update_gate", "out_gate"):
        out[f"agg.ConvGRUCell_00.{gate}.weight"] = (D, 2 * D, 1, 1)
        out[f"agg.ConvGRUCell_00.{gate}.bias"] = (D,)
    for idx in (0, 2):
        out[f"network_pred.{idx}.weight"] = (D, D, 1, 1)
        out[f"network_pred.{idx}.bias"] = (D,)
    return out


class KernelTimer:

    def __init__(self, names):
        self.names = set(names)
        self.records = []
        self.enabled = True

    def timed(self, eng, name, args):
        if not self.enabled:
            return eng.lib.call(name, *args, eng.lib.stream())
        a, b = torch.cuda.Event(enable_timing=True), torch.cuda.Event(enable_timing=True)
        a.record()
        rc = eng.lib.call(name, *args, eng.lib.stream())
        b.record()
        fl, by = algorithmic_cost(name, args)
        xf = fl * executed_fraction(name, args, L.last_kernel(eng.lib)) if fl else 0.0
        self.records.append((TIMER_FAMILY.get(name, name), eng._tag, a, b, fl, by, xf))
        return rc

    def summary(self, steps: int = 1):
        torch.cuda.synchronize()
        out = {}
        times = [r[2].elapsed_time(r[3]) for r in self.records]
        n = len(times)
        if steps > 1 and n % steps == 0:
            per = n // steps
            same = all(self.records[i][0] == self.records[i % per][0] for i in range(n))
            if same:
                for i in range(per):
                    col = sorted(times[i + k * per] for k in range(steps))
                    med = col[len(col) // 2] if len(col) % 2 else 0.5 * (col[len(col) // 2 - 1] + col[len(col) // 2])
                    for k in range(steps):
                        times[i + k * per] = med
        for (name, tag, a, b, fl, by, xf), ms in zip(self.records, times):
            for key in (name,) + ((f"tag:{tag}",) if tag else ()):
                d = out.setdefault(key, {"launches": 0, "ms": 0.0, "flops": 0.0, "bytes": 0.0, "executed_flops": 0.0})
                d["launches"] += 1
                d["ms"] += ms
                d["flops"] += fl
                d["bytes"] += by
                d["executed_flops"] += xf
        return out


TIMER_FAMILY = {"dpc_conv_igemm_ex": "dpc_conv_igemm"}
HBM_FAMILY = ("dpc_bn_apply", "dpc_bn_bwd_reduce", "dpc_bn_bwd_apply", "dpc_bn_relu_maxpool_fwd", "dpc_pool_bn_bwd_apply",
              "dpc_pooled_bn_bwd_reduce", "dpc_pack_input_s2d")


def _esz(dc):
    return 2 if dc == L.BF16 else 4


def algorithmic_cost(name, args):
    if name == "dpc_bn_apply":
        n = args[3] * args[4] * _esz(args[2])
        return 0.0, float(n * (2 + (args[7] is not None)) + (n // 16 if args[11] is not None else 0))
    if name == "dpc_bn_bwd_reduce":
        n = args[5] * args[6] * _esz(args[4])
        return 0.0, float(2 * n + (n // 16 if args[2] is not None else (n if args[1] is not None else 0)))
    if name == "dpc_bn_bwd_apply":
        n = args[5] * args[6] * _esz(args[4])
        return 0.0, float(3 * n + (n if args[13] is not None else 0) + (n // 16 if args[2] is not None else (n if args[1] is not None else 0)))
    if name == "dpc_bn_relu_maxpool_fwd":
        e, NT, H, W, Cc = _esz(args[1]), args[2], args[3], args[4], args[5]
        return 0.0, float(NT * H * W * Cc * e + NT * ((H - 1) // 2 + 1) * ((W - 1) // 2 + 1) * Cc * (e + 1))
    if name == "dpc_pool_bn_bwd_apply":
        e, NT, H, W, Cc = _esz(args[3]), args[4], args[5], args[6], args[7]
        return 0.0, float(2 * NT * H * W * Cc * e + NT * ((H - 1) // 2 + 1) * ((W - 1) // 2 + 1) * Cc * (e + 1))
    if name == "dpc_pooled_bn_bwd_reduce":
        return 0.0, float(args[4] * args[5] * (2 * _esz(args[3]) + 1))
    if name == "dpc_pack_input_s2d":
        px = args[3] * args[4] * args[5] * args[6]
        return 0.0, float(px * 3 * 4 + px * 4 * _esz(args[2]))
    if name == "dpc_score_fwd":
        return 2.0 * args[2] * args[2] * args[3], float(2 * args[2] * args[3] * 2)
    if name == "dpc_score_bwd":
        return 2.0 * args[4] * args[4] * args[5], float(2 * args[4] * args[5] * 2 + args[4] * args[5] * 4)
    if name in ("dpc_gemm_nt_splitk", "dpc_gemm_tn_splitk"):
        e = _esz(args[0])
        return 2.0 * args[1] * args[2] * args[3], float((args[1] + args[2]) * args[3] * e + args[1] * args[2] * 4)
    if name not in ("dpc_conv_igemm", "dpc_conv_igemm_ex", "dpc_conv_wgrad"):
        return 0.0, 0.0
    d = args[0]._obj
    esz = 2 if d.dtype_in == L.BF16 else 4
    osz = 2 if d.dtype_out == L.BF16 else 4
    taps = d.KT * d.KH * d.KW
    rows_out = d.N * d.RT * d.RH * d.RW
    rows_src = d.N * d.ST * d.SH * d.SW
    if name in ("dpc_conv_igemm", "dpc_conv_igemm_ex") and d.mode == 1:
        macs = rows_src * d.Ci * d.Co * taps
    else:
        macs = rows_out * d.Co * d.Ci * taps
    if taps == 16 and d.Ci == 16 and d.KT == 1:
        macs = macs * 147 // 256
    if name == "dpc_conv_igemm":
        by = rows_src * d.Ci * esz + d.Co * d.Ci * taps * esz + rows_out * d.Co * osz
    elif name == "dpc_conv_igemm_ex":
        ep = args[4]._obj
        n = rows_out * d.Co * osz
        by = rows_src * d.Ci * esz + d.Co * d.Ci * taps * esz + n
        by += (n if ep.addend else 0) + (n // 16 if ep.addend_mask else 0) + (n if ep.bn_raw else 0) + (n // 16 if ep.bn_mask else 0)
        name = "dpc_conv_igemm"
    else:
        by = rows_src * d.Ci * esz + rows_out * d.Co * esz + d.Co * d.Ci * taps * 4
    return 2.0 * macs, float(by)


def executed_fraction(name, args, kernel: str) -> float:
    if name not in ("dpc_conv_igemm", "dpc_conv_igemm_ex") or not kernel.startswith("igemm_ws_kernel"):
        return 1.0
    if os.environ.get("DPC_IGEMM_WS_TGROUP", "1") == "0":
        return 1.0
    d = args[0]._obj
    unit = d.st == 1 and d.sh == 1 and d.sw == 1
# ... 117 lines not shown
        self._coef_ready = False
        e.call("dpc_bn_bwd_apply", dy, None if mask is not None else y, mask, self.raw, dc, self.rows, self.Co, self.mean,
               self.invstd, e.PRM[self.bnname + ".weight"], e.coef, gated, dx, dz)

    def bn_prepare(self, dy: torch.Tensor, y: Optional[torch.Tensor], relu: bool, ext_mask: Optional[torch.Tensor] = None):
        e = self.eng
        dc = L.dtype_code(e.cdtype)
        mask = ext_mask if ext_mask is not None else (self.mask if relu else None)
        gated = int(relu or ext_mask is not None)
        if self.reduced_rows:
            prow, self.reduced_rows = self.reduced_rows, 0
        else:
            pr = C.c_int32(0)
            e.call("dpc_bn_bwd_reduce", dy, None if mask is not None else y, mask, self.raw, dc, self.rows, self.Co, self.mean,
                   self.invstd, gated, e.stats, C.byref(pr))
            prow = pr.value
        e.call("dpc_bn_bwd_finalize", e.stats, prow, self.Co, float(self.rows), e.G[self.bnname + ".weight"],
               e.G[self.bnname + ".bias"], e.coef)
        self._coef_ready = True

    def wgrad(self, x: torch.Tensor, draw: torch.Tensor):
        e = self.eng
        ns = C.c_int32(0)
        e.call("dpc_conv_wgrad", C.byref(self.desc_w), x, draw, self.Co, e.part, C.byref(ns))
        g = e.G[self.wname]
        if self.stem:
            e.call("dpc_unpack_stem_wgrad", e.part, ns.value, g, self.Co)
        else:
            Ci, t = self.Ci, self.taps
            e.call("dpc_reduce_unpack", e.part, ns.value, g, self.Co, t, Ci, Ci * t, 1, t, 0)

    def dgrad(self, draw: torch.Tensor, dx: torch.Tensor, addend: Optional[torch.Tensor], addend_mask: Optional[torch.Tensor] = None,
              red: "Optional[_ConvBN]" = None):
        e = self.eng
        e.side_wait()
        if addend_mask is None and red is None:
            e.call("dpc_conv_igemm", C.byref(self.desc_d), draw, self.wd, dx, addend, None)
            return
        ep = L.ConvEpilogue()
        ep.addend = addend.data_ptr() if addend is not None else None
        ep.addend_mask = addend_mask.data_ptr() if addend_mask is not None else None
        if red is not None:
            ep.bn_raw, ep.bn_mean, ep.bn_invstd = red.raw.data_ptr(), red.mean.data_ptr(), red.invstd.data_ptr()
            ep.bn_mask = red.mask.data_ptr() if red.mask is not None else None
            ep.stats = e.stats.data_ptr()
        e.call("dpc_conv_igemm_ex", C.byref(self.desc_d), draw, self.wd, dx, C.byref(ep))
        if red is not None:
            red.reduced_rows = self.stat_rows_d if not e.reserve_cus else e.lib.call("dpc_conv_stats_rows", C.byref(self.desc_d))


class _Block:

    def __init__(self, eng, pre: str, Ci: int, Co: int, is3d: bool, stride: int, in_shape, has_ds: bool, final_relu: bool):
        self.eng = eng
        k, s, p = block_geometry(is3d, stride)
        self.c1 = _ConvBN(eng, pre + "conv1.weight", pre + "bn1", Ci, Co, k, s, p, in_shape)
        self.c2 = _ConvBN(eng, pre + "conv2.weight", pre + "bn2", Co, Co, k, (1, 1, 1), p, self.c1.out_shape)
        self.ds = _ConvBN(eng, pre + "downsample.0.weight", pre + "downsample.1", Ci, Co, (1, 1, 1), s, (0, 0, 0),
                          in_shape) if has_ds else None
        self.final_relu = final_relu
        self.site = pre[len("backbone."):]
        self.out_shape = self.c2.out_shape
        self.Co = Co
        self.act1 = eng.empty(self.c1.out_shape + (Co,), eng.cdtype)
        self.out = eng.empty(self.out_shape + (Co,), eng.cdtype)
        self.x_in: Optional[torch.Tensor] = None

    def units(self):
        return [u for u in (self.c1, self.c2, self.ds) if u is not None]

    def forward(self, x):
        self.x_in = x
        self.c1.forward(x)
        self.c1.apply(self.act1, relu=True)
        self.c2.forward(self.act1)
        if self.ds is not None:
            self.ds.forward(x)
            self.c2.apply(self.out, relu=self.final_relu, res=self.ds.raw, res_unit=self.ds)
        else:
            self.c2.apply(self.out, relu=self.final_relu, res=x)
        return self.out

    def plan_backward(self, prev: "Optional[_Block]"):
        e = self.eng
        fold_c1, gate, fold_prev = (False, False, False) if not e.fold else fold_decision(
            e.lib, self.c1.desc_d, self.c2.desc_d, self.ds is not None, self.final_relu, prev is not None)
        red = bool(int(os.environ.get("DPC_FOLD_RED", "1")))
        self.fold_c1, self.gate, self.fold_prev = red and fold_c1, gate, red and fold_prev
        self.prev = prev

    def backward(self, dout: torch.Tensor, need_dx: bool = True) -> Optional[torch.Tensor]:
        e = self.eng
        oshape = tuple(self.out.shape)
        ishape = tuple(self.x_in.shape)
        omask = self.c2.mask if self.final_relu else None
        draw2 = e.scratch(oshape, exclude=[dout])
        dz = None
        if self.ds is None and not self.gate and need_dx:
            dz = e.scratch(oshape, exclude=[dout, draw2])
        self.c2.bn_backward(dout, self.out if self.final_relu else None, self.final_relu, draw2, dz)
        draw_d = None
        if self.ds is not None:
            draw_d = e.scratch(oshape, exclude=[dout, draw2])
            self.ds.bn_backward(dout, None, False, draw_d, ext_mask=omask)
        dact1 = e.scratch(oshape, exclude=[dout, draw2, draw_d, dz])
        self.c2.dgrad(draw2, dact1, None, red=self.c1 if self.fold_c1 else None)
        if self.fold_c1:
            self.c1.bn_prepare(dact1, self.act1, True)
        with e.side(reads=[draw2, draw_d], site=self.site + "c2"):
            if self.ds is not None:
                self.ds.wgrad(self.x_in, draw_d)
            self.c2.wgrad(self.act1, draw2)
        draw1 = draw2 if e._side is None or e.timer is not None else e.scratch(oshape, exclude=[dout, draw2, draw_d, dz, dact1])
        self.c1.bn_backward(dact1, self.act1, True, draw1)
        if not need_dx:
            with e.side(reads=[draw1], site=self.site + "c1"):
                self.c1.wgrad(self.x_in, draw1)
            return None
        if self.ds is not None:
            dx = e.scratch(ishape, exclude=[])
            self.c1.dgrad(draw1, dx, None)
            self.ds.dgrad(draw_d, dx, dx)
        elif self.gate:
            dx = dout
            self.c1.dgrad(draw1, dx, dout, addend_mask=omask, red=self.prev.c2 if self.fold_prev else None)
            if self.fold_prev:
                pv = self.prev
                pv.c2.bn_prepare(dx, pv.out if pv.final_relu else None, pv.final_relu)
        else:
            dx = dact1
            self.c1.dgrad(draw1, dx, dz)
        with e.side(reads=[draw1], site=self.site + "c1"):
            self.c1.wgrad(self.x_in, draw1)
        return dx


ENGINES: "weakref.WeakValueDictionary[int, BackboneEngine]" = weakref.WeakValueDictionary()


def engine_of(param: torch.Tensor) -> "Optional[BackboneEngine]":
    a = param.data_ptr()
    for base, eng in list(ENGINES.items()):
        if base <= a < base + eng.flat_p.numel() * 4:
            return eng
    return None


class BackboneEngine:
    BN_MOMENTUM = 0.1

    def __init__(self, shapes: "Dict[str, Tuple[int, ...]]", network: str, sample_size: int, num_seq: int, seq_len: int, batch: int,
                 device, compute_dtype, widths: Sequence[int], lib: Optional[L.Lib], lr: float, wd: float, gru_dropout: float, seed: int,
                 stem_fused: bool | None = None, fold: bool | None = None, reserve_cus: int | None = None,
                 f32_matmul: str | None = None, bn_running: bool = False):
        self.device = torch.device(device)
        self.lib = L.lib_for(self.device, lib)
        self.cdtype = compute_dtype
        self.network, self.size, self.N, self.SL, self.B = network, sample_size, num_seq, seq_len, batch
        self.widths = tuple(widths)
        self.D = widths[3]
        self.lr, self.wd, self.p_drop = lr, wd, gru_dropout
        self.last_duration = int(math.ceil(seq_len / 4))
        self.last_size = int(math.ceil(sample_size / 32))
        self.SQ = self.last_size ** 2
        if sample_size % 2:
            raise ValueError("sample_size must be even (space-to-depth stem)")
        self._stats_need = 0
        self._part_need = 0
        self._scratch: Dict[Tuple[int, ...], List[torch.Tensor]] = {}
        self._step_count = 0
        self._groups, self._groups_key, self._seg_host, self._seg_dev, self._seg_n = None, None, None, None, 0
        self._guard, self._guard_state, self._guard_partials = None, None, None
        self._steps_unsure = False
        self._ema, self.flat_ema, self._ema_swapped = None, None, False
        self._lr_sched, self._lr_desc, self._lr_state = None, None, None
        self._opt_kind, self._opt_x1d, self._opt_key, self._opt_host = "adam", False, None, b""
        self._lamb, self._aw_seg_dev, self._aw_seg_n = None, None, 0
        self._accum_n, self._accum_pos, self.flat_acc = 1, 0, None
        self.seg_uploads = 0
        self.no_grad_params = frozenset()
        self.seed = int(seed)
        self.timer: Optional["KernelTimer"] = None
        self._tag: Optional[str] = None
        self._capture_events: Optional[list] = None
        self._captures: Dict[tuple, object] = {}
        self._capture_graphs: list = []
        self._launches = 0
        weakref.finalize(self, _park_graphs, self._capture_graphs)
        self._carved = False

        self._want_stem_fused = bool(int(os.environ.get("DPC_STEM_FUSED", "1"))) if stem_fused is None else bool(stem_fused)
        self.fold = bool(int(os.environ.get("DPC_FOLD", "1"))) if fold is None else bool(fold)
        self.reserve_cus = int(os.environ.get("DPC_RESERVE_CUS", "0")) if reserve_cus is None else int(reserve_cus)
        mm = (f32_matmul or os.environ.get("DPC_F32_MATMUL", "exact")).lower()
        if mm not in ("exact", "bf16x6"):
            raise ValueError("f32_matmul must be 'exact' or 'bf16x6'")
        self.f32_matmul = mm
        self._x6 = 1 if (mm == "bf16x6" and compute_dtype == torch.float32) else 0
        self._pack_table = None
        self._side = (torch.cuda.Stream(self.device) if self.device.type == "cuda" and int(os.environ.get("DPC_WGRAD_STREAM", "1")) else None)
        self._on_side = False
        self.side_off = frozenset(x for x in os.environ.get("DPC_SIDE_OFF", "").split(",") if x)
        self._busy = []
        self.bn_running = bool(bn_running)
        self.train_mode = True
        self.BUF: Dict[str, torch.Tensor] = {}
        self.shapes = shapes
        self.offsets: Dict[str, Tuple[int, int]] = {}
        off = 0
        for k, shp in self.shapes.items():
            n = int(math.prod(shp))
            self.offsets[k] = (off, n)
            off += (n + 3) // 4 * 4
        self.numel = off
        self.flat_p = torch.zeros(off, dtype=torch.float32, device=self.device)
        self.flat_g = torch.zeros_like(self.flat_p)
        self.flat_m = torch.zeros_like(self.flat_p)
        self.flat_v = torch.zeros_like(self.flat_p)
        self.PRM = {k: self.flat_p[o:o + n].view(self.shapes[k]) for k, (o, n) in self.offsets.items()}
        ENGINES[self.flat_p.data_ptr()] = self
        self.G = {k: self.flat_g[o:o + n].view(self.shapes[k]) for k, (o, n) in self.offsets.items()}

        BN, H = batch * num_seq, sample_size
        dt = self.cdtype
        self.x_s2d = self.empty((BN, seq_len, H // 2, H // 2, 16), dt)
        self.dev_input = torch.zeros(1, dtype=torch.int32, device=self.device)
        self._resident_ws = None
        self.stem =_ConvBN(self, "backbone.conv1.weight", "backbone.bn1", 16, widths[0], (1, 4, 4), (1, 1, 1), (0, 2, 2),
                            (BN, seq_len, H // 2, H // 2), stem=True)
        hp = (H // 2 - 1) // 2 + 1
        self.pool_shape = (BN, seq_len, hp, hp)
        self.pooled = self.empty(self.pool_shape + (widths[0],), dt)
        self.pool_arg = torch.empty(self.pool_shape + (widths[0],), dtype=torch.uint8, device=self.device)
        self.blocks: List[_Block] = []
        shape = self.pool_shape
        for pre, cin, planes, is3d, stride, has_ds, last in walk_blocks(network, widths):
            blk = _Block(self, "backbone." + pre, cin, planes, is3d, stride, shape, has_ds, final_relu=not last)
            self.blocks.append(blk)
            shape = blk.out_shape
        for i, blk in enumerate(self.blocks):
            blk.plan_backward(self.blocks[i - 1] if i > 0 else None)
        self.n_head_blocks = LAYER_PLAN[network][0]
        self.grad_split = self.offsets["backbone.layer2.0.conv1.weight"][0]
        self.feat_shape = shape
        if shape[1] != self.last_duration or shape[2] != self.last_size or shape[3] != self.last_size:
            raise ValueError(f"backbone output {shape} does not match last_duration/last_size "
                             f"({self.last_duration},{self.last_size}); see dpc/model_3d.py:24-25,53-55")
        self.units: List[_ConvBN] = [self.stem] + [u for b in self.blocks for u in b.units()]

        self.dev_step = torch.zeros(1, dtype=torch.int32, device=self.device)
        self.dev_bc = torch.ones(2, dtype=torch.float32, device=self.device)
        self.dev_draw = torch.zeros(1, dtype=torch.int32, device=self.device)

    def _build_gru(self, n_agg: int, n_steps: int, P: int):
        N, D, SQ, dt, f32 = self.N, self.D, self.SQ, self.cdtype, torch.float32
        if D % 32 or D > 256:
            raise ValueError("feature size must be a multiple of 32, at most 256 (fused ConvGRU recurrence)")
        M = self.B * SQ
        ns = n_steps
        self.M, self.n_agg, self.n_steps = M, n_agg, ns
        self.feat_relu = self.empty((N, M, D), dt)
        self.X_all = self.feat_relu[:ns]
        self.H_all = torch.zeros((ns + 1, M, D), dtype=dt, device=self.device)
        self.HR_all = self.empty((ns, M, D), dt)
        self.G_all = self.empty((ns, M, 3 * D), dt)
        self.U_all, self.R_all, self.O_all = (self.empty((ns, M, D), f32) for _ in range(3))
        self.drop_all: Optional[torch.Tensor] = None
        self.d_featrelu = self.empty((n_agg, M, D), f32)
        self.d_feat = self.empty(self.feat_shape + (D,), dt)
        self.gru_packed = self.empty((16 * D * D,), dt)
        self.gru_ws = self.empty((2, M, D), f32)
        self.dWx = self.empty((3 * D, D), f32)
        self.dWh = self.empty((2 * D, D), f32)
        self.dWo = self.empty((D, D), f32)
        self.db = self.empty((3 * D,), f32)
        for (co, kk) in ((3 * D, D), (2 * D, D), (D, D)):
            self._need_wgrad(ns * M, co, kk)
        self.need_part(64 * 3 * D)
        self._gate_table = None
        gd, Pm = L.GruChainDesc(), self.PRM
        gd.dtype, gd.M, gd.D, gd.SQ, gd.P, gd.n_agg, gd.n_steps = L.dtype_code(dt), M, D, SQ, P, n_agg, ns
        gd.p_drop, gd.seed = float(self.p_drop), self.seed
        for name, t in (("packed", self.gru_packed), ("bias_u", Pm["agg.ConvGRUCell_00.update_gate.bias"]),
                        ("bias_r", Pm["agg.ConvGRUCell_00.reset_gate.bias"]), ("bias_o", Pm["agg.ConvGRUCell_00.out_gate.bias"]),
                        ("X_all", self.X_all), ("H_all", self.H_all), ("HR_all", self.HR_all), ("U_all", self.U_all),
                        ("R_all", self.R_all), ("O_all", self.O_all), ("G_all", self.G_all), ("d_x", self.d_featrelu),
                        ("ws", self.gru_ws)):
            setattr(gd, name, t.data_ptr())
        self.gru_desc = gd

    def _gru_param_grads(self, dc):
        D, M, ns, Gm = self.D, self.M, self.n_steps, self.G
        self.gemm_tn(self.G_all, 3 * D, self.X_all, D, self.dWx, ns * M, 3 * D, D)
        self.gemm_tn(self.G_all, 3 * D, self.H_all, D, self.dWh, ns * M, 2 * D, D)
        self.gemm_tn(self.G_all[:, :, 2 * D:], 3 * D, self.HR_all, D, self.dWo, ns * M, D, D)
        self.call("dpc_colsum", self.G_all, dc, 3 * D, ns * M, 3 * D, self.db, 0, self.part, self.part.numel())
        if self._gate_table is None:
            ents = []
            for i, (g, n) in enumerate((("u", "update_gate"), ("r", "reset_gate"), ("o", "out_gate"))):
                w = Gm[f"agg.ConvGRUCell_00.{n}.weight"].view(D, 2 * D)
                ents += [(self.dWx[i * D:(i + 1) * D], D, w, 2 * D, D, D),
                         (self.dWh[i * D:(i + 1) * D] if g != "o" else self.dWo, D, w[:, D:], 2 * D, D, D),
                         (self.db[i * D:(i + 1) * D], D, Gm[f"agg.ConvGRUCell_00.{n}.bias"], D, 1, D)]
            tab = (L.Copy2dEntry * len(ents))()
            blk = 0
            for i, (src, sld, dst, dld, r, c) in enumerate(ents):
                tab[i] = L.Copy2dEntry(src.data_ptr(), dst.data_ptr(), sld, dld, r, c, blk, 0)
                blk += max(1, min(64, (r * c + 1023) // 1024))
            raw = torch.frombuffer(bytearray(bytes(tab)), dtype=torch.uint8).clone()
            self._gate_table = (raw.to(self.device), len(ents), blk)
        self.call("dpc_copy2d_multi", *self._gate_table)

    def dropout_masks_of_step(self) -> torch.Tensor:
        buf = self.empty((self.n_steps, self.M, self.D), torch.float32)
        self.call("dpc_dropout_mask", buf, buf.numel(), float(self.p_drop), self.seed, self.dev_draw)
        return buf

    def _finish_buffers(self):
        widths, dt, f32 = self.widths, self.cdtype, torch.float32
        prs = C.c_int32(0)
        ps_ = self.pool_shape
        self.lib.call("dpc_pooled_bn_bwd_reduce", None, None, None, L.dtype_code(dt), ps_[0] * ps_[1] * ps_[2] * ps_[3], widths[0],
                      None, None, None, C.byref(prs), self.lib.stream())
        self.need_stats(prs.value * 2 * widths[0])
        self.coef = self.empty((2, max(widths)), f32)
        self.stats = self.empty((max(self._stats_need, 1),), f32)
        self.part = self.empty((max(self._part_need, 1),), f32)
        ns = C.c_int32(0)
        self._stem_fused = False
        if dt == torch.bfloat16 and self._want_stem_fused:
            try:
                self._stem_fused = self.lib.call("dpc_stem_wgrad_fused", C.byref(self.stem.desc_w), None, None, None, None, None, None, None,
                                                 None, None, C.byref(ns), self.lib.stream()) == 0
            except L.DpcError:
                self._stem_fused = False
        if self._stem_fused:
            self.need_part(ns.value * widths[0] * 256)
            self.part = self.empty((max(self._part_need, 1),), f32)
            self.stem_dz = None
        else:
            self.stem_dz = self.empty(tuple(self.stem.raw.shape), dt)
        self.packed_for_step = -1

    @property
    def part(self) -> torch.Tensor:
        return self._part_side if self._on_side else self._part_main

    @part.setter
    def part(self, t: torch.Tensor):
        self._part_main = t
        self._part_side = torch.empty_like(t) if self._side is not None else t

    def empty(self, shape, dtype):
        return torch.empty(tuple(shape), dtype=dtype, device=self.device)

    def need_stats(self, n):
        self._stats_need = max(self._stats_need, int(n))

    def need_part(self, n):
        self._part_need = max(self._part_need, int(n))

    def _need_wgrad(self, M, Co, K):
        d = self._gemm_desc(M, Co, K, K, K, Co, out_f32=True)
        ns = C.c_int32(0)
        self.lib.call("dpc_conv_wgrad", C.byref(d), None, None, (Co + 7) // 8 * 8, None, C.byref(ns), self.lib.stream())
        self.need_part(ns.value * Co * K)

    def call(self, name, *args):
        self._launches += 1
        if getattr(self.lib, "_f32_mode", 0) != self._x6:
            self.lib.call("dpc_set_f32_matmul", self._x6)
            self.lib._f32_mode = self._x6
        tm = self.timer
        if tm is not None and name in tm.names:
            return tm.timed(self, name, args)
        return self.lib.call(name, *args, self.lib.stream())

    @contextlib.contextmanager
    def tag(self, name: str):
        prev, self._tag = self._tag, name
        try:
            yield
        finally:
            self._tag = prev

    def scratch(self, shape, exclude):
        pool = self._scratch.setdefault(tuple(shape), [])

        def free():
            for t in pool:
                if all(t is not x for x in exclude if x is not None) and all(t is not b for _, bufs in self._busy for b in bufs):
                    return t
            return None
        t = free()
        while t is None and self._busy:
            ev, _ = self._busy.pop(0)
            torch.cuda.current_stream(self.device).wait_event(ev)
            t = free()
        if t is None:
            t = self.empty(shape, self.cdtype)
            pool.append(t)
        return t

    @contextlib.contextmanager
    def side(self, reads=(), site: str = ""):
        if self._side is None or self.timer is not None or site in self.side_off:
            yield
            return
        main = torch.cuda.current_stream(self.device)
        ev = torch.cuda.Event()
        ev.record(main)
        self._side.wait_event(ev)
        with torch.cuda.stream(self._side):
            self._on_side = True
            try:
                yield
            finally:
                self._on_side = False
            done = torch.cuda.Event()
            done.record(self._side)
        self._busy.append((done, [t for t in reads if t is not None]))
        if self._capture_events is not None:
            self._capture_events += [ev, done]

    def side_wait(self):
        if self._busy:
            torch.cuda.current_stream(self.device).wait_event(self._busy[-1][0])

    def side_join(self):
        if self._busy:
            torch.cuda.current_stream(self.device).wait_event(self._busy[-1][0])
            self._busy.clear()

    def _gemm_desc(self, M, N, K, lda, ldb, ldo, out_f32=True):
        dc = L.dtype_code(self.cdtype)
        return L.ConvDesc(dc, L.F32 if out_f32 else dc, 0, M, 1, 1, 1, 1, 1, 1, K, lda, N, ldb, ldo, 1, 1, 1, 1, 1, 1, 0, 0, 0)

    def gemm(self, A, Bm, out, M, N, K, lda=None, ldb=None, ldo=None, addend=None, out_f32=True):
        d = self._gemm_desc(M, N, K, lda or K, ldb or K, ldo or N, out_f32)
        self.call("dpc_conv_igemm", C.byref(d), A, Bm, out, addend, None)

    def gemm_splitk(self, A, Bm, out, M, N, K, lda, ldb):
        ns = C.c_int32(0)
        self.call("dpc_gemm_nt_splitk", L.dtype_code(self.cdtype), M, N, K, A, lda, Bm, ldb, self.part, C.byref(ns))
        self.call("dpc_reduce_unpack", self.part, ns.value, out, M, 1, N, N, 0, 1, 0)

    def gemm_tn(self, dy, dy_ld, X, x_ld, out, M, Co, K):
        d = self._gemm_desc(M, Co, K, x_ld, K, Co)
        ns = C.c_int32(0)
        self.call("dpc_conv_wgrad", C.byref(d), X, dy, dy_ld, self.part, C.byref(ns))
        self.call("dpc_reduce_unpack", self.part, ns.value, out, Co, 1, K, K, 0, 1, 0)

    def load_params(self, params: Dict[str, torch.Tensor]):
        self._not_swapped("load_params")
        for k, v in params.items():
            k = k[7:] if k.startswith("module.") else k
            if k.startswith("agg.cell_list.0."):
                continue
            dst, shp = self.PRM.get(k), self.shapes.get(k)
            if dst is None or shp is None:
                raise KeyError(f"{k}: not a parameter of this {self.network} engine ({len(self.PRM)} parameters, {len(self.shapes)} shapes, "
                               f"in PRM: {k in self.PRM}, in shapes: {k in self.shapes})")
            dst.copy_(v.to(torch.float32).reshape(shp))
        self.packed_for_step = -1
        if self._ema is not None:
            self.flat_ema.copy_(self.flat_p)

    def adopt_optimizer_state(self, old: "BackboneEngine"):
        if old.numel != self.numel or list(old.offsets) != list(self.offsets):
            raise ValueError("adopt_optimizer_state: the engines hold different parameter sets")
        self.flat_m.copy_(old.flat_m)
        self.flat_v.copy_(old.flat_v)
        self.dev_step.copy_(old.dev_step)
        self.dev_bc.copy_(old.dev_bc)
        self.dev_draw.copy_(old.dev_draw)
        self._step_count, self._steps_unsure = old._step_count, old._steps_unsure
        self.lr, self.wd = old.lr, old.wd
        if old.param_groups:
            self.set_param_groups(old.param_groups)
        if old._guard_state is not None:
            self._guard_alloc()
            self._guard_state.copy_(old._guard_state)
            self._guard = old._guard
        if old.flat_ema is not None:
            old._not_swapped("adopt_optimizer_state")
            self._ema_alloc()
            self.flat_ema.copy_(old.flat_ema)
            self._ema = old._ema
        if old._lr_desc is not None:
            self._lr_alloc()
            self._lr_state.copy_(old._lr_state)
            self._lr_sched, self._lr_desc = old._lr_sched, old._lr_desc
        if old._opt_kind != "adam":
            self.set_optimizer(old._opt_kind, old._opt_x1d)
# ... 697 lines not shown
            if eng._baked_scalars() != baked:
                raise RuntimeError(f"lr / wd / dropout / gradient guard / EMA decay / lr schedule changed since this step was captured ({baked} -> {eng._baked_scalars()}): "
                                   f"call {again}")
            return run(eng, graphs)

        replay.graphs = graphs
        replay.kernels = kernels
        replay.events = events
        replay.refill = refill
        for k, v in attrs.items():
            setattr(replay, k, v)
        self._capture_graphs.append(_Capture(graphs, events))
        if not all(kernels):
            raise L.DpcError(f"the captured {what} step was cut into an empty hipGraph (kernel launches per graph: {kernels})")
        self._captures[key] = replay
        return replay

    def _forward_loss(self, block: Optional[torch.Tensor], train: bool):
        raise NotImplementedError

    def _backward_reaches_backbone(self) -> bool:
        return True

    def capture_train_step(self, block: Optional[torch.Tensor], allreduce=None, warmup: int = 2, refill=None):
        buf = self.x_s2d if block is None else block
        need_backbone = self._backward_reaches_backbone()
        key = (buf.data_ptr(), tuple(buf.shape), id(allreduce) if allreduce is not None else None, self.reserve_cus, tuple(sorted(self.side_off)),
               id(refill) if refill is not None else None, tuple(sorted(self.no_grad_params))) + self._baked_scalars()
        two_bucket = allreduce is not None and hasattr(allreduce, "start")
        split = self.grad_split if need_backbone else 0
        tail, head, whole, result = self.flat_g[self.grad_split:], self.flat_g[:split], self.flat_g, self.result

        def warm():
            for _ in range(warmup):
                self.train_step(block, allreduce=allreduce)

        def body(cut):
            self._forward_loss(block, True)
            if two_bucket and not need_backbone:
                self.backward(on_tail_ready=lambda _tail: None)
                cut()
            else:
                self.backward(on_tail_ready=cut if two_bucket else None)
                if allreduce is not None:
                    cut()
            host_steps, unsure = self._step_count, self._steps_unsure
            self.adam_step()
            self._step_count, self._steps_unsure = host_steps, unsure

        def run(eng, graphs):
            eng._not_swapped("replay of a captured train step")
            graphs[0].replay()
            if two_bucket:
                allreduce.start(tail)
                if need_backbone:
                    graphs[1].replay()
                allreduce.finish(head)
                graphs[-1].replay()
            elif allreduce is not None:
                allreduce(whole)
                graphs[1].replay()
            eng._count_step()
            eng.packed_for_step = -1
            return result

        if self._accum_n > 1:
            return self._capture_accum_step(key, block, buf, allreduce, warmup, refill, run)
        return self._capture(key, "train", "capture_train_step() again (it captures a new step for the new values)", warm, body, run,
                             refill, block=buf)

    def _capture_accum_step(self, key: tuple, block, buf, allreduce, warmup: int, refill, run_last):
        hit = self._captures.get(key)
        if hit is not None:
            return hit
        n, result = self._accum_n, self.result
        again = "capture_train_step() again (it captures a new step for the new values)"
        if warmup and self._accum_pos:
            raise RuntimeError("capture_train_step: a warm-up under gradient accumulation runs whole cycles and must start at a cycle "
                               f"boundary ({self._accum_pos} of {n} micro-batches are pending)")

        def warm():
            for _ in range(warmup * n):
                self.train_step(block, allreduce=allreduce)

        def body_micro(cut):
            self._forward_loss(block, True)
            self.backward()
            self._accum_launch(L.ACCUM_ADD, 0, self.numel)

        def run_micro(eng, graphs):
            eng._not_swapped("replay of a captured train step")
            graphs[0].replay()
            return result

        def body_last(cut):
            self._forward_loss(block, True)
            self._accum_finish_and_exchange(allreduce, cut)
            host_steps, unsure = self._step_count, self._steps_unsure
            self.adam_step()
            self._step_count, self._steps_unsure = host_steps, unsure

        micro = self._capture(key + ("micro",), "train", again, warm, body_micro, run_micro, refill, block=buf)
        last = self._capture(key + ("last",), "train", again, lambda: None, body_last, run_last, refill, block=buf)
        me = weakref.ref(self)

        def replay():
            eng = me()
            if eng is None:
                raise RuntimeError("replay of a captured train step whose engine is gone")
            if eng._accum_pos < n - 1:
                res = micro()
                eng._accum_pos += 1
            else:
                res = last()
                eng._accum_pos = 0
            return res

        replay.micro, replay.last = micro, last
        replay.graphs, replay.kernels = micro.graphs + last.graphs, micro.kernels + last.kernels
        replay.events, replay.refill, replay.block = (micro.events or []) + (last.events or []), refill, buf
        self._captures[key] = replay
        return replay

    def capture_eval_step(self, refill=None):
        key = ("eval", self.x_s2d.data_ptr(), tuple(sorted(self.side_off)), id(refill) if refill is not None else None) + self._baked_scalars()
        result = self.result

        def warm():
            if self._pack_table is None:
                self.pack_weights()

        def body(cut):
            self._forward_loss(None, False)

        def run(eng, graphs):
            graphs[0].replay()
            return result

        return self._capture(key, "evaluation", "capture_eval_step() again", warm, body, run, refill)

    def release_captures(self):
        torch.cuda.synchronize(self.device)
        self._captures.clear()
        _park_graphs(list(self._capture_graphs))
        self._capture_graphs.clear()


class DPCEngine(BackboneEngine):

    def __init__(self, network: str = "resnet18", sample_size: int = 128, num_seq: int = 8, seq_len: int = 5,
                 pred_step: int = 3, batch: int = 4, device="cuda", compute_dtype=torch.float32,
                 widths: Sequence[int] = LAYER_WIDTH, lib: Optional[L.Lib] = None,
                 lr: float = 1e-3, wd: float = 1e-5, dropout: float = 0.1, seed: int = 233, score_path: str = "auto", stem_fused: bool | None = None,
                 fold: bool | None = None, reserve_cus: int | None = None, f32_matmul: str | None = None):
        self.P = pred_step
        self.score_mode = "materialised"
        super().__init__(param_shapes(network, widths), network, sample_size, num_seq, seq_len, batch, device, compute_dtype, widths, lib,
                         lr, wd, dropout, seed, stem_fused, fold, reserve_cus, f32_matmul)
        self._build_head(score_path)
        self._finish_buffers()

    def _build_head(self, score_path: str):
        dt, f32 = self.cdtype, torch.float32
        B, P, SQ, D, N = self.B, self.P, self.SQ, self.D, self.N
        if score_path not in ("auto", "fused", "materialised"):
            raise ValueError("score_path must be auto, fused or materialised")
        self._build_gru(n_agg=N - P, n_steps=(N - P) + P - 1, P=P)
        M = self.M
        self.feat_inf = self.empty((B, P, SQ, D), dt)
        self.pred = self.empty((B, P, SQ, D), dt)
        self.P1_all = self.empty((P, M, D), dt)
        self.dP1 = self.empty((P, M, D), dt)
        self.dP2 = self.empty((P, M, D), dt)
        self.Hpred = self.H_all[self.n_agg:]
        R = B * P * SQ
        self.R = R
        self.score = self.empty((R, R), f32)
        E = 8 if dt == torch.bfloat16 else 4
        self.ld_d = (R + E - 1) // E * E
        self.dscore = self.empty((R, self.ld_d), dt)
        self.row_ws = self.empty((R, 2), f32)
        self.result = self.empty((4,), f32)
        self.predT = torch.zeros((D, self.ld_d), dtype=dt, device=self.device)
        self.finfT = torch.zeros((D, self.ld_d), dtype=dt, device=self.device)
        fusable = dt == torch.bfloat16 and D in (256, 32)
        self.score_fusable = fusable and score_path == "fused"
        self._score_fused = False
        if self.score_fusable:
            nf, nb = C.c_int64(0), C.c_int64(0)
            self.lib.call("dpc_score_ws_floats", R, D, C.byref(nf), C.byref(nb))
            self.score_ws = self.empty((max(nf.value, nb.value),), f32)
            self.score_diag, self.score_lse2 = self.empty((R,), f32), self.empty((R,), f32)
        self.score16 = None
        if dt == torch.bfloat16 and R % 64 == 0 and R <= 16384 and D in (256, 32) and not self.score_fusable and int(os.environ.get("DPC_SCORE_BF16", "1")):
            self.score16 = self.empty((R, R), dt)
        self._score16_live = False
        self.d_pred = self.empty((B, P, SQ, D), f32)
        self.d_finf = self.empty((B, P, SQ, D), f32)
        self.mask: Optional[torch.Tensor] = None
        self._need_wgrad(R, R, D)
        nsk = C.c_int32(0)
        self.lib.call("dpc_gemm_nt_splitk", L.dtype_code(dt), R, D, self.ld_d, None, self.ld_d, None, self.ld_d, None, C.byref(nsk), self.lib.stream())
        self.need_part(nsk.value * R * D)
        self._tn_splits = None
        if dt == torch.bfloat16:
            rc = self.lib._fn("dpc_gemm_tn_splitk")(L.dtype_code(dt), R, D, R, None, self.ld_d, None, self.ld_d, None, C.byref(nsk), self.lib.stream())
            if rc == 0:
                self._tn_splits = nsk.value
                self.need_part(nsk.value * R * D)
        gd, Pm = self.gru_desc, self.PRM
        for name, t in (("bias_1", Pm["network_pred.0.bias"]), ("bias_2", Pm["network_pred.2.bias"]), ("P1_all", self.P1_all),
                        ("pred", self.pred), ("d_pred", self.d_pred), ("dP1", self.dP1), ("dP2", self.dP2)):
            setattr(gd, name, t.data_ptr())

    def forward(self, block: torch.Tensor, train: bool = False, dropout_masks: Optional[torch.Tensor] = None,
                materialise: bool = True, new_draw: bool = True):
        B, N, P, SQ, D, M = self.B, self.N, self.P, self.SQ, self.D, self.M
        if block is not None:
            if tuple(block.shape) != (B, N, 3, self.SL, self.size, self.size) or block.dtype != torch.float32:
                raise ValueError(f"block must be float32 [B,N,3,SL,H,W] = {(B, N, 3, self.SL, self.size, self.size)}, got {tuple(block.shape)}")
            if block.device != self.device:
                raise ValueError("block is on the wrong device")
        x = self._backbone_forward(block)
        dc = L.dtype_code(self.cdtype)
        fs = self.feat_shape
        self.call("dpc_tpool_split_fwd", x, dc, B, N, fs[1], SQ, D, P, self.feat_relu, self.feat_inf)
        if dropout_masks is not None:
            self.drop_all = dropout_masks.to(self.device, torch.float32).contiguous()
            if tuple(self.drop_all.shape) != (self.n_steps, M, D):
                raise ValueError(f"dropout_masks must be [n_steps, M, D] = {(self.n_steps, M, D)}")
        else:
            self.drop_all = None
        gd = self.gru_desc
        gd.drop_masks = self.drop_all.data_ptr() if dropout_masks is not None else None
        draw = dropout_masks is None and train and self.p_drop > 0
        if draw and new_draw:
            self.call("dpc_counter_advance", self.dev_draw)
        gd.step_dev = self.dev_draw.data_ptr() if draw else None
        self.call("dpc_gru_chain_fwd", C.byref(gd))
        R = self.R
        self._score_fused = bool(self.score_fusable and not materialise)
        if self._score_fused:
            with self.tag("score"):
                self.call("dpc_score_fwd", self.pred, self.feat_inf, R, D, self.score_diag, self.score_lse2, self.row_ws, None,
                          self.score_ws)
            self.score_mode = "fused"
            return None
        self._score16_live = bool(self.score16 is not None and not materialise)
        if self._score16_live:
            self.score_mode = "materialised (bf16 logits)"
            with self.tag("score"):
                self.gemm(self.pred, self.feat_inf, self.score16, R, R, D, out_f32=False)
            return None
        self.score_mode = "materialised"
        with self.tag("score"):
            self.gemm(self.pred, self.feat_inf, self.score, R, R, D)
        return self.score.view(B, P, SQ, B, P, SQ)

    def get_mask(self) -> torch.Tensor:
        if self.mask is None:
            B, P, SQ = self.B, self.P, self.SQ
            self.mask = torch.empty((B, P, SQ, B, P, SQ), dtype=torch.int8, device=self.device)
            self.call("dpc_mask_gen", self.mask, B, P, SQ)
        return self.mask

    def loss_topk(self, with_grad: bool = True) -> torch.Tensor:
        R = self.R
        if self._score_fused:
            self.call("dpc_ce_finalize", self.row_ws, R, self.result)
            return self.result
        if self._score16_live:
            self.call("dpc_ce_topk_bf16", self.score16, R, R, R, self.row_ws, self.result, self.dscore if with_grad else None, self.ld_d)
            return self.result
        self.call("dpc_ce_topk", self.score, R, R, R, self.row_ws, self.result, self.dscore if with_grad else None,
                  L.dtype_code(self.cdtype), self.ld_d)
        return self.result

    def backward(self, dscore_external: Optional[torch.Tensor] = None, on_tail_ready=None):
        self._backbone_backward(self._head_backward(dscore_external), on_tail_ready)

    def _head_backward(self, dscore_external: Optional[torch.Tensor] = None) -> torch.Tensor:
        B, N, P, SQ, D, M, R = self.B, self.N, self.P, self.SQ, self.D, self.M, self.R
        dc = L.dtype_code(self.cdtype)
        if dscore_external is not None:
            src = dscore_external.reshape(R, R).to(torch.float32).contiguous()
            if self.ld_d != R:
                self.dscore.zero_()
            self.dscore[:, :R].copy_(src)
        both = self.cdtype == torch.bfloat16 and ((self._score_fused and dscore_external is None) or bool(self._tn_splits))
        if both:
            self.call("dpc_transpose2d_bf16x2", self.feat_inf, self.pred, D, self.finfT, self.predT, self.ld_d, R, D)
        else:
            self.call("dpc_transpose2d", self.feat_inf, dc, D, self.finfT, dc, self.ld_d, R, D)
        if self._score_fused and dscore_external is None:
            if not both:
                self.call("dpc_transpose2d", self.pred, dc, D, self.predT, dc, self.ld_d, R, D)
            with self.tag("score"):
                for own, oth, othT, by_owner, out in ((self.pred, self.feat_inf, self.finfT, 1, self.d_pred),
                                                      (self.feat_inf, self.pred, self.predT, 0, self.d_finf)):
                    n = self.call("dpc_score_bwd", own, oth, othT, self.ld_d, R, D, self.score_lse2, by_owner, self.score_ws)
                    self.call("dpc_reduce_unpack", self.score_ws, n, out, R, 1, D, D, 0, 1, 0)
        else:
            if self._score_fused:
                raise L.DpcError("backward(dscore_external=...) needs a materialised score: call forward(materialise=True)")
            with self.tag("score"):
                self.gemm_splitk(self.dscore, self.finfT, self.d_pred, R, D, self.ld_d, self.ld_d, self.ld_d)
                if self._tn_splits:
                    ns = C.c_int32(0)
                    self.call("dpc_gemm_tn_splitk", dc, R, D, R, self.dscore, self.ld_d, self.predT, self.ld_d, self.part, C.byref(ns))
                    self.call("dpc_reduce_unpack", self.part, ns.value, self.d_finf, R, 1, D, D, 0, 1, 0)
                else:
                    self.gemm_tn(self.dscore, self.ld_d, self.pred, D, self.d_finf, R, R, D)
        self.call("dpc_gru_chain_bwd", C.byref(self.gru_desc))
        fs = self.feat_shape
        self.call("dpc_tpool_split_bwd", self.blocks[-1].out, self.d_featrelu, self.d_finf, dc, B, N, fs[1], SQ, D, P, self.d_feat)
        with self.side(site="head"):
            self._head_param_grads(dc)
        return self.d_feat

    def _head_param_grads(self, dc):
        D, M, P, Gm = self.D, self.M, self.P, self.G
        self._gru_param_grads(dc)
        self.gemm_tn(self.dP1, D, self.Hpred, D, Gm["network_pred.0.weight"].view(D, D), P * M, D, D)
        self.gemm_tn(self.dP2, D, self.P1_all, D, Gm["network_pred.2.weight"].view(D, D), P * M, D, D)
        self.call("dpc_colsum", self.dP1, dc, D, P * M, D, Gm["network_pred.0.bias"], 0, self.part, self.part.numel())
        self.call("dpc_colsum", self.dP2, dc, D, P * M, D, Gm["network_pred.2.bias"], 0, self.part, self.part.numel())

    def _forward_loss(self, block: Optional[torch.Tensor], train: bool, dropout_masks: Optional[torch.Tensor] = None):
        self.forward(block, train=train, dropout_masks=dropout_masks, materialise=False)
        self.loss_topk(with_grad=train)

    def train_step(self, block: torch.Tensor, dropout_masks: Optional[torch.Tensor] = None, allreduce=None) -> torch.Tensor:
        self._not_swapped("train_step")
        self._forward_loss(block, True, dropout_masks=dropout_masks)
        if self._accum_n > 1:
            self._accum_micro_step(allreduce)
            return self.result
        self._backward_and_exchange(allreduce)
        self.adam_step()
        return self.result
```

### dpc_amd/lc.py

```python
from __future__ import annotations

import ctypes as C
from typing import Dict, Optional, Sequence, Tuple

import torch
import torch.nn as nn

from . import _lib as L
from .engine import BN_EPS, BackboneEngine, LAYER_WIDTH, param_shapes
from .model import _REPLICA_ERROR, _EngineModule, _attach, _init_reference_style


def lc_param_shapes(network: str, num_class: int, widths: Sequence[int] = LAYER_WIDTH) -> "Dict[str, Tuple[int, ...]]":
    base = param_shapes(network, widths)
    out = {k: v for k, v in base.items() if not k.startswith("network_pred.")}
    D = widths[3]
    out["final_bn.weight"] = (D,)
    out["final_bn.bias"] = (D,)
    out["final_fc.1.weight"] = (num_class, D)
    out["final_fc.1.bias"] = (num_class,)
    return out


def lc_state_dict_keys(network: str, num_class: int, widths: Sequence[int] = LAYER_WIDTH):
    keys = []
    shapes = lc_param_shapes(network, num_class, widths)
    names = list(shapes)
    for i, k in enumerate(names):
        keys.append(k)
        is_bn_bias = k.endswith(".bias") and (".bn" in k or k.startswith("backbone.bn1") or "downsample.1" in k or k.startswith("final_bn"))
        if is_bn_bias:
            pre = k[: -len("bias")]
            keys += [pre + "running_mean", pre + "running_var", pre + "num_batches_tracked"]
        if k == "agg.ConvGRUCell_00.out_gate.bias":
            keys += [n.replace("agg.ConvGRUCell_00.", "agg.cell_list.0.") for n in names if n.startswith("agg.ConvGRUCell_00.")]
    return keys


class LCEngine(BackboneEngine):

    def __init__(self, network: str = "resnet18", sample_size: int = 128, num_seq: int = 8, seq_len: int = 5, batch: int = 4,
                 device="cuda", compute_dtype=torch.float32, widths: Sequence[int] = LAYER_WIDTH, lib: Optional[L.Lib] = None,
                 lr: float = 1e-3, wd: float = 1e-3, dropout: float = 0.5, num_class: int = 101, gru_dropout: float = 0.1,
                 seed: int = 666):
        self.num_class = int(num_class)
        self.p_drop_fc = float(dropout)
        super().__init__(lc_param_shapes(network, self.num_class, widths), network, sample_size, num_seq, seq_len, batch, device,
                         compute_dtype, widths, lib, lr, wd, gru_dropout, seed, bn_running=True)
        self._build_head()
        self._finish_buffers()

    def _build_head(self):
        B, N, SQ, D, dt, NC = self.B, self.N, self.SQ, self.D, self.cdtype, self.num_class
        f32 = torch.float32
        self._build_gru(n_agg=N, n_steps=N, P=0)
        M = self.M
        self.d_hlast = self.empty((M, D), f32)
        self._ran_backbone_backward = True
        self._eval_ran = False
        self.d_context = self.empty((B, D), f32)
        self.BUF["final_bn.running_mean"] = torch.zeros(D, dtype=f32, device=self.device)
        self.BUF["final_bn.running_var"] = torch.ones(D, dtype=f32, device=self.device)
        self.BUF["final_bn.num_batches_tracked"] = torch.zeros((), dtype=torch.int64, device=self.device)
        self.target = torch.zeros(B, dtype=torch.int64, device=self.device)
        self.ctx, self.xhat, self.context, self.y_drop, self.dctx = (self.empty((B, D), f32) for _ in range(5))
        self.bn1d_stat = self.empty((2, D), f32)
        self.logits, self.dlogits = self.empty((B, NC), f32), self.empty((B, NC), f32)
        self.row_ws, self.result = self.empty((B, 2), f32), self.empty((2,), f32)
        Pm, gd = self.PRM, self.gru_desc
        for name, t in (("bias_1", Pm["agg.ConvGRUCell_00.out_gate.bias"]), ("bias_2", Pm["agg.ConvGRUCell_00.out_gate.bias"]),
                        ("d_hlast", self.d_hlast)):
            setattr(gd, name, t.data_ptr())
        hd = self.head_desc = L.LcHeadDesc()
        hd.dtype, hd.B, hd.SQ, hd.D, hd.num_class, hd.train = L.dtype_code(dt), B, SQ, D, NC, 1
        hd.p_drop, hd.momentum, hd.eps, hd.seed = self.p_drop_fc, self.BN_MOMENTUM, BN_EPS, self.seed
        G = self.G
        for name, t in (("h_last", self.H_all[N]), ("bn_weight", Pm["final_bn.weight"]), ("bn_bias", Pm["final_bn.bias"]),
                        ("bn_running_mean", self.BUF["final_bn.running_mean"]), ("bn_running_var", self.BUF["final_bn.running_var"]),
                        ("bn_num_batches", self.BUF["final_bn.num_batches_tracked"]), ("fc_weight", Pm["final_fc.1.weight"]),
                        ("fc_bias", Pm["final_fc.1.bias"]), ("target", self.target), ("ctx", self.ctx), ("xhat", self.xhat),
                        ("bn_out", self.context), ("y", self.y_drop), ("stat", self.bn1d_stat), ("logits", self.logits),
                        ("dlogits", self.dlogits), ("row_ws", self.row_ws), ("result", self.result),
                        ("g_fc_weight", G["final_fc.1.weight"]), ("g_fc_bias", G["final_fc.1.bias"]),
                        ("g_bn_weight", G["final_bn.weight"]), ("g_bn_bias", G["final_bn.bias"]), ("dctx", self.dctx),
                        ("d_hlast", self.d_hlast)):
            setattr(hd, name, t.data_ptr())

    def load_params(self, params: Dict[str, torch.Tensor]):
        own = {k: v for k, v in params.items() if (k[7:] if k.startswith("module.") else k) not in self.BUF}
        super().load_params(own)
        for k, v in params.items():
            k2 = k[7:] if k.startswith("module.") else k
            if k2 in self.BUF:
                self.BUF[k2].copy_(v.to(self.BUF[k2].dtype).reshape(self.BUF[k2].shape))

    def state_dict(self) -> Dict[str, torch.Tensor]:
        self._not_swapped("state_dict")
        self._not_mid_cycle("state_dict")
        out = {}
        for k in lc_state_dict_keys(self.network, self.num_class, self.widths):
            if k in self.PRM:
                out[k] = self.PRM[k].detach().clone()
            elif k in self.BUF:
                out[k] = self.BUF[k].detach().clone()
            else:
                out[k] = out[k.replace("agg.cell_list.0.", "agg.ConvGRUCell_00.")]
        return out

    def set_labels(self, target: torch.Tensor):
        self.target.copy_(target.reshape(self.B).to(self.device, torch.int64))

    def fill_synthetic(self, seed: int, block: Optional[torch.Tensor] = None):
        super().fill_synthetic(seed, block)
        self.call("dpc_synthetic_labels", self.target, self.B, self.num_class, int(seed) & 0xFFFFFFFFFFFFFFFF, self.dev_input)

    def forward(self, block: torch.Tensor, target: Optional[torch.Tensor] = None, train: bool = False,
                gru_masks: Optional[torch.Tensor] = None, fc_mask: Optional[torch.Tensor] = None):
        B, N, SQ, D, M = self.B, self.N, self.SQ, self.D, self.M
        if block is not None and (tuple(block.shape) != (B, N, 3, self.SL, self.size, self.size) or block.dtype != torch.float32):
            raise ValueError(f"block must be float32 [B,N,3,SL,H,W] = {(B, N, 3, self.SL, self.size, self.size)}")
        self.train_mode = bool(train)
        if target is not None:
            self.set_labels(target)
        if not train:
            self._eval_ran = True
        x = self._backbone_forward(block)
        dc = L.dtype_code(self.cdtype)
        self.call("dpc_relu_tpool_fwd", x, dc, B, N, self.feat_shape[1], SQ, D, self.feat_relu)
        gd, hd = self.gru_desc, self.head_desc
        self._keep = (gru_masks, fc_mask)
        if gru_masks is not None:
            gru_masks = gru_masks.to(self.device, torch.float32).contiguous()
            self._keep = (gru_masks, fc_mask)
        gd.drop_masks = gru_masks.data_ptr() if gru_masks is not None else None
        if train and (gru_masks is None or fc_mask is None):
            self.call("dpc_counter_advance", self.dev_draw)
        gd.step_dev = self.dev_draw.data_ptr() if (gru_masks is None and train and self.p_drop > 0) else None
        self.call("dpc_gru_chain_fwd", C.byref(gd))
        if fc_mask is not None:
            fc_mask = fc_mask.to(self.device, torch.float32).contiguous()
            self._keep = (gru_masks, fc_mask)
        hd.train = int(train)
        hd.drop_mask = fc_mask.data_ptr() if fc_mask is not None else None
        hd.step_dev = self.dev_draw.data_ptr()
        self.call("dpc_lc_head_fwd", C.byref(hd))
        return self.logits.view(B, 1, self.num_class), self.context.view(B, 1, D)

    def grad_wanted(self, wanted=None) -> Tuple[bool, bool]:
        if wanted is None:
            skip = set(self.frozen_params()) | set(self.no_grad_params)
            wanted = [k for k in self.offsets if k not in skip]
        backbone = any(k.startswith("backbone.") for k in wanted)
        return backbone, backbone or any(k.startswith("agg.") for k in wanted)

    def _first_bucket(self) -> torch.Tensor:
        return self.flat_g[:self.grad_split] if self._ran_backbone_backward else self.flat_g[:0]

    def backward(self, on_tail_ready=None, d_output: Optional[torch.Tensor] = None, d_context: Optional[torch.Tensor] = None,
                 wanted=None):
        if not self.train_mode:
            raise L.DpcError("LCEngine.backward needs a train-mode forward (BatchNorm with batch statistics)")
        B, N, SQ, D = self.B, self.N, self.SQ, self.D
        dc = L.dtype_code(self.cdtype)
        hd = self.head_desc
        if d_output is not None or d_context is not None:
            if d_output is None:
                self.dlogits.zero_()
            else:
                self.dlogits.copy_(d_output.reshape(B, self.num_class))
            if d_context is not None:
                self.d_context.copy_(d_context.reshape(B, D))
        hd.d_bn_out = self.d_context.data_ptr() if d_context is not None else None
        self.call("dpc_lc_head_bwd", C.byref(hd))
        hd.d_bn_out = None
        need_backbone, need_agg = self.grad_wanted(wanted)
        self._ran_backbone_backward = need_backbone
        if need_agg:
            self.call("dpc_gru_chain_bwd", C.byref(self.gru_desc))
            self._gru_param_grads(dc)
        if not need_backbone:
            if on_tail_ready is not None:
                self.side_join()
                on_tail_ready(self.flat_g[self.grad_split:])
            return
        self.call("dpc_relu_tpool_bwd", self.blocks[-1].out, self.d_featrelu, dc, B, N, self.feat_shape[1], SQ, D, self.d_feat)
        self._backbone_backward(self.d_feat, on_tail_ready)

    def _forward_loss(self, block: Optional[torch.Tensor], train: bool):
        self.forward(block, None, train=train)

    def _backward_reaches_backbone(self) -> bool:
        return self.grad_wanted()[0]

    def train_step(self, block: torch.Tensor, target: Optional[torch.Tensor] = None, allreduce=None, **masks) -> torch.Tensor:
        self._not_swapped("train_step")
        self.forward(block, target, train=True, **masks)
        if self._accum_n > 1:
            self._accum_micro_step(allreduce)
            return self.result
        self._backward_and_exchange(allreduce)
        self.adam_step()
# ... 202 lines not shown
```

### include/dpc_hip.h

```cpp
#ifndef DPC_HIP_H
#define DPC_HIP_H
#include <stdint.h>

#ifdef __cplusplus
extern "C" {
#endif

#define DPC_F32 0
#define DPC_BF16 1

#define DPC_ERR_ARG (-1)
#define DPC_ERR_LAUNCH (-2)
#define DPC_ERR_UNSUPPORTED (-3)

typedef void* dpc_stream_t;

int dpc_abi_version(void);

typedef struct dpc_conv_desc {
    int32_t dtype_in, dtype_out;
    int32_t mode;
    int32_t N, RT, RH, RW;
    int32_t ST, SH, SW;
    int32_t Ci, src_ld;
    int32_t Co, ldw, ldo;
    int32_t KT, KH, KW;
    int32_t st, sh, sw;
    int32_t pt, ph, pw;
} dpc_conv_desc;

int dpc_conv_stats_rows(const dpc_conv_desc* d);
int dpc_conv_igemm(const dpc_conv_desc* d, const void* src, const void* wgt, void* out,
                   const void* addend, float* stats, dpc_stream_t stream);

typedef struct dpc_conv_epilogue {
    const void* addend;
    const uint8_t* addend_mask;
    const void* bn_raw;
    const uint8_t* bn_mask;
    const float* bn_mean;
    const float* bn_invstd;
    float* stats;
} dpc_conv_epilogue;
int dpc_conv_igemm_ex(const dpc_conv_desc* d, const void* src, const void* wgt, void* out, const dpc_conv_epilogue* epi,
                      dpc_stream_t stream);

int dpc_gemm_nt_splitk(int32_t dtype, int32_t M, int32_t N, int32_t K, const void* A, int32_t lda, const void* B, int32_t ldb,
                       float* part, int32_t* nsplit, dpc_stream_t stream);
int dpc_gemm_tn_splitk(int32_t dtype, int32_t M, int32_t N, int32_t K, const void* A, int32_t lda, const void* B, int32_t ldb,
                       float* part, int32_t* nsplit, dpc_stream_t stream);

int dpc_conv_wgrad(const dpc_conv_desc* d, const void* src, const void* dy, int32_t dy_ld,
                   float* part, int32_t* nsplit, dpc_stream_t stream);

#define DPC_PLAN_IGEMM 0
#define DPC_PLAN_WGRAD 1
#define DPC_PLAN_ADDEND 1
#define DPC_PLAN_STATS 2
#define DPC_PLAN_ADDEND_MASK 4
#define DPC_PLAN_BNRED 8
int dpc_conv_plan(const dpc_conv_desc* d, int32_t op, int32_t flags, int32_t dy_ld, char* name, int32_t cap);
int dpc_last_kernel(char* name, int32_t cap);

int dpc_set_reserved_cus(int32_t n);

int dpc_set_f32_matmul(int32_t mode);

int dpc_diag_squat(int32_t n_wg, int32_t waves, int32_t lds_bytes, int32_t mode, int32_t usec, const void* scratch,
                   int64_t scratch_bytes, uint32_t* where, uint32_t* sink, dpc_stream_t stream);

int dpc_pack3d(const float* in, void* out, int32_t dtype_out, int32_t d0, int32_t d1, int32_t d2,
               int64_t s0, int64_t s1, int64_t s2, dpc_stream_t stream);
typedef struct dpc_pack_entry {
    const void* in;
    void* out;
    int32_t d0, d1, d2, block0;
    int64_t s0, s1, s2;
} dpc_pack_entry;
int dpc_pack3d_multi(const dpc_pack_entry* table_dev, int32_t n_entries, int32_t total_blocks, int32_t dtype_out, dpc_stream_t stream);
int dpc_reduce_unpack(const float* part, int32_t nsplit, float* out, int32_t d0, int32_t d1, int32_t d2,
                      int64_t s0, int64_t s1, int64_t s2, int32_t accumulate, dpc_stream_t stream);
int dpc_transpose2d_bf16x2(const void* in0, const void* in1, int32_t ld_in, void* out0, void* out1, int32_t ld_out, int32_t rows,
                           int32_t cols, dpc_stream_t stream);
int dpc_transpose2d(const void* in, int32_t dtype_in, int32_t ld_in, void* out, int32_t dtype_out, int32_t ld_out,
                    int32_t rows, int32_t cols, dpc_stream_t stream);

int dpc_pack_input_s2d(const float* block, void* out, int32_t dtype_out, int32_t BN, int32_t T, int32_t H, int32_t W,
                       dpc_stream_t stream);
int dpc_synthetic_input(float* block, void* out, int32_t dtype_out, int32_t BN, int32_t T, int32_t H, int32_t W, uint64_t seed,
                        const int32_t* draw_dev, dpc_stream_t stream);
int dpc_synthetic_labels(int64_t* target, int32_t B, int32_t num_class, uint64_t seed, const int32_t* draw_dev, dpc_stream_t stream);
int dpc_pack_stem_weight(const float* w, void* out, int32_t dtype_out, int32_t Co, dpc_stream_t stream);
int dpc_unpack_stem_wgrad(const float* part, int32_t nsplit, float* dw, int32_t Co, dpc_stream_t stream);

int dpc_bn_finalize(const float* partials, int32_t rows, int32_t C, double count, const float* gamma,
                    const float* beta, float eps, float* mean, float* invstd, float* scale, float* shift,
                    dpc_stream_t stream);
int dpc_bn_apply(const void* x, void* y, int32_t dtype, int64_t rows, int32_t C, const float* scale,
                 const float* shift, const void* res, const float* rscale, const float* rshift, int32_t relu,
                 uint8_t* mask, dpc_stream_t stream);
int dpc_bn_bwd_reduce(const void* dy, const void* y, const uint8_t* mask, const void* x, int32_t dtype, int64_t rows, int32_t C,
                      const float* mean, const float* invstd, int32_t relu, float* partials, int32_t* prow,
                      dpc_stream_t stream);
int dpc_bn_bwd_finalize(const float* partials, int32_t prow, int32_t C, double count, float* dgamma, float* dbeta,
                        float* coef, dpc_stream_t stream);
int dpc_bn_bwd_apply(const void* dy, const void* y, const uint8_t* mask, const void* x, int32_t dtype, int64_t rows, int32_t C,
                     const float* mean, const float* invstd, const float* gamma, const float* coef, int32_t relu,
                     void* dx, void* dz, dpc_stream_t stream);

int dpc_bn_relu_maxpool_fwd(const void* x, int32_t dtype, int32_t NT, int32_t H, int32_t W, int32_t C,
                            const float* scale, const float* shift, void* y, uint8_t* argmax, dpc_stream_t stream);
int dpc_maxpool_bwd(const void* dy, const uint8_t* argmax, int32_t dtype, int32_t NT, int32_t H, int32_t W, int32_t C,
                    void* dz, dpc_stream_t stream);

int dpc_pool_bn_bwd_reduce(const void* dy, const uint8_t* argmax, const void* x, int32_t dtype, int32_t NT, int32_t H,
                           int32_t W, int32_t C, const float* mean, const float* invstd, float* partials, int32_t* prow,
                           dpc_stream_t stream);
int dpc_pooled_bn_bwd_reduce(const void* dy, const uint8_t* argmax, const void* ypool, int32_t dtype, int64_t rows,
                             int32_t C, const float* gamma, const float* beta, float* partials, int32_t* prow,
                             dpc_stream_t stream);
int dpc_pool_bn_bwd_apply(const void* dy, const uint8_t* argmax, const void* x, int32_t dtype, int32_t NT, int32_t H,
                          int32_t W, int32_t C, const float* mean, const float* invstd, const float* gamma,
                          const float* coef, void* dx, dpc_stream_t stream);
int dpc_stem_wgrad_fused(const dpc_conv_desc* d, const void* src_s2d, const void* raw, const void* dpool, const uint8_t* argmax,
                         const float* mean, const float* invstd, const float* gamma, const float* coef, float* part,
                         int32_t* nsplit, dpc_stream_t stream);

int dpc_tpool_split_fwd(const void* x, int32_t dtype, int32_t B, int32_t N, int32_t T, int32_t SQ, int32_t D,
                        int32_t P, void* feat_relu, void* feat_inf, dpc_stream_t stream);
int dpc_tpool_split_bwd(const void* x, const void* d_relu, const float* d_inf, int32_t dtype, int32_t B, int32_t N,
                        int32_t T, int32_t SQ, int32_t D, int32_t P, void* dx, dpc_stream_t stream);

int dpc_colsum(const void* x, int32_t dtype, int32_t ld, int32_t M, int32_t D, float* out, int32_t accumulate,
               float* ws, int64_t ws_floats , dpc_stream_t stream);

int dpc_mask_gen(int8_t* mask, int32_t B, int32_t P, int32_t SQ, dpc_stream_t stream);
int dpc_ce_topk(const float* score, int32_t rows, int32_t cols, int32_t ld, float* row_ws, float* result,
                void* dscore, int32_t dtype_d, int32_t ld_d, dpc_stream_t stream);
int dpc_ce_topk_bf16(const void* score_bf16, int32_t rows, int32_t cols, int32_t ld, float* row_ws, float* result,
                     void* dscore_bf16, int32_t ld_d, dpc_stream_t stream);

int dpc_score_ws_floats(int32_t R, int32_t D, int64_t* fwd_floats, int64_t* bwd_floats);
int dpc_score_fwd(const void* pred, const void* finf, int32_t R, int32_t D, float* diag, float* lse2, float* row_ws,
                  float* score, float* ws, dpc_stream_t stream);
int dpc_score_bwd(const void* own, const void* oth, const void* othT, int32_t ldT, int32_t R, int32_t D, const float* lse2,
                  int32_t by_owner, float* out_part, dpc_stream_t stream);
int dpc_ce_finalize(const float* row_ws, int32_t rows, float* result, dpc_stream_t stream);

int dpc_adam(float* p, const float* g, float* m, float* v, int64_t n, float lr, float beta1, float beta2, float eps,
             float wd, float bias_corr1, float bias_corr2, float grad_scale, dpc_stream_t stream);

int dpc_step_advance(int32_t* step_dev, float* bias_corr_dev, double beta1, double beta2, dpc_stream_t stream);
int dpc_adam_dev(float* p, const float* g, float* m, float* v, int64_t n, float lr, double beta1, double beta2, float eps,
                 float wd, const float* bias_corr_dev, float grad_scale, dpc_stream_t stream);
#define DPC_ADAM_MAX_SEGMENTS 512
typedef struct dpc_adam_segment {
    int64_t begin, end;
    float lr, weight_decay;
    int32_t active;
    int32_t reserved;
} dpc_adam_segment;
int dpc_adam_groups_dev(float* p, const float* g, float* m, float* v, int64_t n, const dpc_adam_segment* segments_dev,
                        int32_t n_segments, double beta1, double beta2, float eps, const float* bias_corr_dev, float grad_scale,
                        dpc_stream_t stream);
#define DPC_GRAD_PARTIALS 1024
typedef struct dpc_grad_state {
    double sumsq;
    float norm;
    float coef;
    int32_t skip;
    int32_t n_skipped, n_clipped;
    int32_t reserved;
} dpc_grad_state;
int dpc_grad_sumsq(const float* g, int64_t n, const dpc_adam_segment* segments_dev, int32_t n_segments, double* partials,
                   dpc_stream_t stream);
int dpc_grad_verdict(const double* partials, int32_t n_partials, double max_norm, int32_t skip_nonfinite, dpc_grad_state* state_dev,
                     dpc_stream_t stream);
int dpc_step_advance_gated(int32_t* step_dev, float* bias_corr_dev, double beta1, double beta2, const dpc_grad_state* state_dev,
                           dpc_stream_t stream);
int dpc_adam_dev_ex(float* p, const float* g, float* m, float* v, int64_t n, float lr, double beta1, double beta2, float eps,
                    float wd, const float* bias_corr_dev, float grad_scale, const dpc_grad_state* state_dev, dpc_stream_t stream);
int dpc_adam_groups_dev_ex(float* p, const float* g, float* m, float* v, int64_t n, const dpc_adam_segment* segments_dev,
                           int32_t n_segments, double beta1, double beta2, float eps, const float* bias_corr_dev, float grad_scale,
                           const dpc_grad_state* state_dev, dpc_stream_t stream);
int dpc_grad_scale(float* g, int64_t n, const dpc_adam_segment* segments_dev, int32_t n_segments, const dpc_grad_state* state_dev,
                   dpc_stream_t stream);
#define DPC_ACCUM_ADD 0
#define DPC_ACCUM_FINISH 1
int dpc_grad_accumulate(float* acc, float* g, int64_t n, int64_t begin, int64_t end, const dpc_adam_segment* segments_dev,
                        int32_t n_segments, int32_t mode, float scale, dpc_stream_t stream);
int dpc_adam_dev_ema(float* p, const float* g, float* m, float* v, int64_t n, float lr, double beta1, double beta2, float eps,
                     float wd, const float* bias_corr_dev, float grad_scale, const dpc_grad_state* state_dev, float* ema,
                     const int32_t* step_dev, float decay, dpc_stream_t stream);
int dpc_adam_groups_dev_ema(float* p, const float* g, float* m, float* v, int64_t n, const dpc_adam_segment* segments_dev,
                            int32_t n_segments, double beta1, double beta2, float eps, const float* bias_corr_dev, float grad_scale,
                            const dpc_grad_state* state_dev, float* ema, const int32_t* step_dev, float decay, dpc_stream_t stream);
int dpc_arena_swap(float* a, float* b, int64_t n, dpc_stream_t stream);
#define DPC_LR_CONSTANT 0
#define DPC_LR_COSINE 1
#define DPC_LR_LINEAR 2
#define DPC_LR_MULTISTEP 3
#define DPC_LR_MAX_MILESTONES 8
typedef struct dpc_lr_schedule {
    int32_t kind;
    int32_t warmup_steps;
    int32_t total_steps;
// ... 198 lines not shown
```

Baseline: 5054 clips/s.

## Group head weight-gradient GEMMs, reductions and colsums into batched launches

Adds grouped wgrad2, reduce-unpack and colsum kernels. Each launch takes a table of up to eight problems and maps each block to its problem by prefix offsets. The GRU and prediction-head parameter-gradient GEMMs (dWx, dWh, dWo, pred0, pred1) and their bias column sums now run as a few launches instead of many small ones. The goal is to cut launch count and fill the GPU better on small head GEMMs. The colsum loops also gain 8-way unrolled loads. Costs are large kernel argument structs and a linear problem search in each block.

```diff
diff --git a/dpc_amd/_lib.py b/dpc_amd/_lib.py
--- a/dpc_amd/_lib.py
+++ b/dpc_amd/_lib.py
@@ -120,6 +120,18 @@
 class Copy2dEntry(C.Structure):
     _fields_ = [("src", C.c_void_p), ("dst", C.c_void_p), ("src_ld", C.c_int64), ("dst_ld", C.c_int64), ("rows", C.c_int32), ("cols", C.c_int32),
                 ("block0", C.c_int32), ("pad", C.c_int32)]
+
+
+GROUP_MAX = 8
+
+
+class ReduceEntry(C.Structure):
+    _fields_ = [("part", C.c_void_p), ("out", C.c_void_p), ("nsplit", C.c_int32), ("d0", C.c_int32), ("d1", C.c_int32), ("d2", C.c_int32),
+                ("s0", C.c_int64), ("s1", C.c_int64), ("s2", C.c_int64), ("accumulate", C.c_int32), ("reserved", C.c_int32)]
+
+
+class ColsumEntry(C.Structure):
+    _fields_ = [("x", C.c_void_p), ("out", C.c_void_p), ("ld", C.c_int32), ("M", C.c_int32), ("D", C.c_int32), ("accumulate", C.c_int32)]
 
 
 class DpcError(RuntimeError):
@@ -135,6 +147,9 @@
     "dpc_gemm_nt_splitk": [_i32, _i32, _i32, _i32, _vp, _i32, _vp, _i32, _vp, C.POINTER(_i32), _vp],
     "dpc_gemm_tn_splitk": [_i32, _i32, _i32, _i32, _vp, _i32, _vp, _i32, _vp, C.POINTER(_i32), _vp],
     "dpc_conv_wgrad": [C.POINTER(ConvDesc), _vp, _vp, _i32, _vp, C.POINTER(_i32), _vp],
+    "dpc_gemm_tn_group": [C.POINTER(ConvDesc), _i32, C.POINTER(_vp), C.POINTER(_vp), C.POINTER(_i32), _vp, C.POINTER(_i64), C.POINTER(_i32), _vp],
+    "dpc_reduce_unpack_group": [C.POINTER(ReduceEntry), _i32, _vp],
+    "dpc_colsum_group": [C.POINTER(ColsumEntry), _i32, _i32, _vp, _i64, _vp],
     "dpc_conv_plan": [C.POINTER(ConvDesc), _i32, _i32, _i32, C.c_char_p, _i32],
     "dpc_last_kernel": [C.c_char_p, _i32],
     "dpc_set_reserved_cus": [_i32],
diff --git a/dpc_amd/csrc/conv_wgrad.hip b/dpc_amd/csrc/conv_wgrad.hip
--- a/dpc_amd/csrc/conv_wgrad.hip
+++ b/dpc_amd/csrc/conv_wgrad.hip
@@ -255,7 +255,7 @@
 };
 
 template <class T, int NWM, int NWN, bool PU>
-__global__ __launch_bounds__(64 * NWM * NWN, 2) void wgrad2_kernel(Wgrad2Params p) {
+__device__ __forceinline__ void wgrad2_body(const Wgrad2Params& p, int wg, int nwg) {
     constexpr int E = Elt<T>::PER16;
     constexpr int ESZ = (int)sizeof(T);
     constexpr int BKP = 8 * E;
@@ -279,9 +279,9 @@
 #endif
     const int wm = wv / NWN, wn = wv % NWN;
     const int l31 = lane & 31, lhi = lane >> 5;
-    int id = blockIdx.x;
+    int id = wg;
     if (p.xcd_remap) {
-        const int nwg = gridDim.x, q = nwg >> 3, r = nwg & 7, x = id & 7;
+        const int q = nwg >> 3, r = nwg & 7, x = id & 7;
         id = (x < r ? x * (q + 1) : r * (q + 1) + (x - r) * q) + (id >> 3);
     }
     const int tile_n = id % p.ntn; id /= p.ntn;
@@ -520,6 +520,25 @@
     }
 }
 
+template <class T, int NWM, int NWN, bool PU>
+__global__ __launch_bounds__(64 * NWM * NWN, 2) void wgrad2_kernel(Wgrad2Params p) {
+    wgrad2_body<T, NWM, NWN, PU>(p, (int)blockIdx.x, (int)gridDim.x);
+}
+
+struct Wgrad2Group {
+    Wgrad2Params p[DPC_GROUP_MAX];
+    int start[DPC_GROUP_MAX + 1];
+    int n;
+};
+
+template <class T, int NWM, int NWN, bool PU>
+__global__ __launch_bounds__(64 * NWM * NWN, 2) void wgrad2_group_kernel(Wgrad2Group G) {
+    const int b = (int)blockIdx.x;
+    int i = 0;
+    while (i + 1 < G.n && b >= G.start[i + 1]) ++i;
+    wgrad2_body<T, NWM, NWN, PU>(G.p[i], b - G.start[i], G.start[i + 1] - G.start[i]);
+}
+
 template <class T, int NWM, int NWN>
 static int launch_wgrad2_t(const Wgrad2Params& p, bool pu, hipStream_t stream) {
     dim3 grid((unsigned)(p.ntm * p.ntn * p.nks)), block(64 * NWM * NWN);
@@ -539,6 +558,26 @@
     if (nwm == 1 && nwn == 4) return launch_wgrad2_t<T, 1, 4>(p, pu, stream);
     if (nwm == 2 && nwn == 2) return launch_wgrad2_t<T, 2, 2>(p, pu, stream);
     return launch_wgrad2_t<T, 2, 3>(p, pu, stream);
+}
+
+template <class T, int NWM, int NWN>
+static int launch_wgrad2_group_t(const Wgrad2Group& G, bool pu, hipStream_t stream) {
+    dim3 grid((unsigned)G.start[G.n]), block(64 * NWM * NWN);
+    dpc_plan_detail("T=%s nwm=%d nwn=%d problems=%d", sizeof(T) == 2 ? "bf16" : "f32", NWM, NWN, G.n);
+    if (pu) {
+        DPC_LAUNCH((wgrad2_group_kernel<T, NWM, NWN, true>), grid, block, stream, G);
+    } else {
+        DPC_LAUNCH((wgrad2_group_kernel<T, NWM, NWN, false>), grid, block, stream, G);
+    }
+    return dpc_launch_status();
+}
+
+template <class T>
+static int launch_wgrad2_group(const Wgrad2Group& G, int nwm, int nwn, bool pu, hipStream_t stream) {
+    if (nwm == 1 && nwn == 3) return launch_wgrad2_group_t<T, 1, 3>(G, pu, stream);
+    if (nwm == 1 && nwn == 4) return launch_wgrad2_group_t<T, 1, 4>(G, pu, stream);
+    if (nwm == 2 && nwn == 2) return launch_wgrad2_group_t<T, 2, 2>(G, pu, stream);
+    return launch_wgrad2_group_t<T, 2, 3>(G, pu, stream);
 }
 
 template <class T, bool RF>
@@ -561,20 +600,27 @@
     return launch_wgrad_rf<T, false>(p, tm, tn, stream);
 }
 
-extern "C" int dpc_conv_wgrad(const dpc_conv_desc* d, const void* src, const void* dy, int32_t dy_ld,
-                              float* part, int32_t* nsplit, dpc_stream_t stream_) {
-    hipStream_t stream = (hipStream_t)stream_;
+struct WgradPlan {
     WgradParams p;
-    p.x6 = dpc_f32_matmul_mode();
+    bool v2, pu;
+    int tm, tn, nwm, nwn;
+    int rwp, rhp, lrw, lrh;
+    long long mv;
+};
+
+static int wgrad_prepare(const dpc_conv_desc* d, int dy_ld, WgradPlan* w) {
+    w->p.x6 = dpc_f32_matmul_mode();
     if (!d || d->mode != 0) return DPC_ERR_ARG;
-    int rc = make_gather_geom(d, &p.g);
+    int rc = make_gather_geom(d, &w->p.g);
     if (rc) return rc;
     const int per16 = d->dtype_in == DPC_BF16 ? 8 : 4;
     if (dy_ld % per16 || dy_ld < d->Co) return DPC_ERR_UNSUPPORTED;
-    rc = dpc_wgrad_patch_try(d, src, dy, dy_ld, part, nsplit, stream);
-    if (rc != 1) return rc;
-    rc = dpc_wgrad_stem_try(d, src, dy, dy_ld, part, nsplit, stream);
-    if (rc != 1) return rc;
+    return DPC_OK;
+}
+
+static void wgrad_plan(const dpc_conv_desc* d, WgradPlan* w) {
+    WgradParams& p = w->p;
+    const int per16 = d->dtype_in == DPC_BF16 ? 8 : 4;
     const int bkp = 8 * per16;
     int rwp = 1, rhp = 1;
     while (rwp < d->RW) rwp <<= 1;
@@ -584,7 +630,6 @@
     static const int pad_on = getenv("DPC_WGRAD2_PAD") ? atoi(getenv("DPC_WGRAD2_PAD")) : 1;
     const bool v2 = bkp % rwp == 0 && mv < (1ll << 31) &&
                     (!padded || (pad_on && (rwp * rhp) % bkp == 0 && (long long)d->RW * d->RH * 10 >= (long long)rwp * rhp * 6));
-    const int lrw = ilog2_exact(rwp), lrh = ilog2_exact(rhp);
     const int nchunks = (int)(((v2 ? mv : (long long)p.g.M) + bkp - 1) / bkp);
     int tm, tn, nwm = 0, nwn = 0;
     if (v2) {
@@ -607,20 +652,88 @@
     if (want > nchunks) want = nchunks;
     p.kcps = (nchunks + want - 1) / want;
     p.nks = (nchunks + p.kcps - 1) / p.kcps;
+    w->v2 = v2; w->pu = (rwp * rhp) % bkp == 0;
+    w->tm = tm; w->tn = tn; w->nwm = nwm; w->nwn = nwn;
+    w->rwp = rwp; w->rhp = rhp; w->lrw = ilog2_exact(rwp); w->lrh = ilog2_exact(rhp); w->mv = mv;
+}
+
+static Wgrad2Params wgrad2_params(const dpc_conv_desc* d, const WgradPlan& w, const void* src, const void* dy, int dy_ld, float* part) {
+    Wgrad2Params q;
+    q.g = w.p.g; q.src = src; q.dy = dy; q.part = part; q.Co = d->Co; q.dy_ld = dy_ld;
+    q.nks = w.p.nks; q.kcps = w.p.kcps; q.ntm = w.p.ntm; q.ntn = w.p.ntn; q.lRW = w.lrw; q.lRH = w.lrh;
+    q.RWm = w.rwp - 1; q.RHm = w.rhp - 1; q.Mv = (int)w.mv; q.x6 = w.p.x6;
+    q.xcd_remap = 1;
+    return q;
+}
+
+extern "C" int dpc_conv_wgrad(const dpc_conv_desc* d, const void* src, const void* dy, int32_t dy_ld,
+                              float* part, int32_t* nsplit, dpc_stream_t stream_) {
+    hipStream_t stream = (hipStream_t)stream_;
+    WgradPlan w;
+    int rc = wgrad_prepare(d, dy_ld, &w);
+    if (rc) return rc;
+    rc = dpc_wgrad_patch_try(d, src, dy, dy_ld, part, nsplit, stream);
+    if (rc != 1) return rc;
+    rc = dpc_wgrad_stem_try(d, src, dy, dy_ld, part, nsplit, stream);
+    if (rc != 1) return rc;
+    wgrad_plan(d, &w);
+    WgradParams& p = w.p;
     if (nsplit) *nsplit = p.nks;
     if (!part) return DPC_OK;
     if (!src || !dy) return DPC_ERR_ARG;
     p.src = src; p.dy = dy; p.part = part; p.Co = d->Co; p.dy_ld = dy_ld;
-    if (v2) {
-        Wgrad2Params q;
-        q.g = p.g; q.src = src; q.dy = dy; q.part = part; q.Co = d->Co; q.dy_ld = dy_ld;
-        q.nks = p.nks; q.kcps = p.kcps; q.ntm = p.ntm; q.ntn = p.ntn; q.lRW = lrw; q.lRH = lrh;
-        q.RWm = rwp - 1; q.RHm = rhp - 1; q.Mv = (int)mv; q.x6 = p.x6;
-        q.xcd_remap = 1;
-        const bool pu = (rwp * rhp) % bkp == 0;
-        if (d->dtype_in == DPC_F32) return launch_wgrad2<float>(q, nwm, nwn, pu, stream);
-        return launch_wgrad2<bf16_t>(q, nwm, nwn, pu, stream);
-    }
-    if (d->dtype_in == DPC_F32) return launch_wgrad<float>(p, tm, tn, stream);
-    return launch_wgrad<bf16_t>(p, tm, tn, stream);
-}
+    if (w.v2) {
+        const Wgrad2Params q = wgrad2_params(d, w, src, dy, dy_ld, part);
+        if (d->dtype_in == DPC_F32) return launch_wgrad2<float>(q, w.nwm, w.nwn, w.pu, stream);
+        return launch_wgrad2<bf16_t>(q, w.nwm, w.nwn, w.pu, stream);
+    }
+    if (d->dtype_in == DPC_F32) return launch_wgrad<float>(p, w.tm, w.tn, stream);
+    return launch_wgrad<bf16_t>(p, w.tm, w.tn, stream);
+}
+
+extern "C" int dpc_gemm_tn_group(const dpc_conv_desc* descs, int32_t n, const void* const* src, const void* const* dy,
+                                 const int32_t* dy_ld, float* part, int64_t* part_off, int32_t* nsplit, dpc_stream_t stream_) {
+    hipStream_t stream = (hipStream_t)stream_;
+    if (!descs || n <= 0 || n > DPC_GROUP_MAX || !dy_ld || !part_off || !nsplit) return DPC_ERR_ARG;
+    WgradPlan w[DPC_GROUP_MAX];
+    long long off = 0;
+    for (int i = 0; i < n; ++i) {
+        const dpc_conv_desc* d = descs + i;
+        int rc = wgrad_prepare(d, dy_ld[i], &w[i]);
+        if (rc) return rc;
+        if (d->dtype_in != descs[0].dtype_in) return DPC_ERR_ARG;
+        int32_t ns = 0;
+        rc = dpc_wgrad_patch_try(d, nullptr, nullptr, dy_ld[i], nullptr, &ns, stream);
+        if (rc != 1) return rc < 0 ? rc : DPC_ERR_UNSUPPORTED;
+        rc = dpc_wgrad_stem_try(d, nullptr, nullptr, dy_ld[i], nullptr, &ns, stream);
+        if (rc != 1) return rc < 0 ? rc : DPC_ERR_UNSUPPORTED;
+        wgrad_plan(d, &w[i]);
+        if (!w[i].v2) return DPC_ERR_UNSUPPORTED;
+        nsplit[i] = w[i].p.nks;
+        part_off[i] = off;
+        off += ((long long)w[i].p.nks * d->Co * w[i].p.g.Kp + 3) / 4 * 4;
+    }
+    part_off[n] = off;
+    if (!part) return DPC_OK;
+    if (!src || !dy) return DPC_ERR_ARG;
+    for (int i = 0; i < n; ++i)
+        if (!src[i] || !dy[i]) return DPC_ERR_ARG;
+    bool done[DPC_GROUP_MAX] = {};
+    for (int i = 0; i < n; ++i) {
+        if (done[i]) continue;
+        Wgrad2Group G;
+        G.n = 0; G.start[0] = 0;
+        for (int j = i; j < n; ++j) {
+            if (done[j] || w[j].nwm != w[i].nwm || w[j].nwn != w[i].nwn || w[j].pu != w[i].pu) continue;
+            done[j] = true;
+            G.p[G.n] = wgrad2_params(descs + j, w[j], src[j], dy[j], dy_ld[j], part + part_off[j]);
+            G.start[G.n + 1] = G.start[G.n] + w[j].p.ntm * w[j].p.ntn * w[j].p.nks;
+            ++G.n;
+        }
+        for (int k = G.n; k < DPC_GROUP_MAX; ++k) { G.p[k] = G.p[0]; G.start[k + 1] = G.start[G.n]; }
+        const int rc = descs[0].dtype_in == DPC_F32 ? launch_wgrad2_group<float>(G, w[i].nwm, w[i].nwn, w[i].pu, stream)
+                                                    : launch_wgrad2_group<bf16_t>(G, w[i].nwm, w[i].nwn, w[i].pu, stream);
+        if (rc) return rc;
+    }
+    return DPC_OK;
+}
diff --git a/dpc_amd/csrc/gru.hip b/dpc_amd/csrc/gru.hip
--- a/dpc_amd/csrc/gru.hip
+++ b/dpc_amd/csrc/gru.hip
@@ -10,39 +10,123 @@
 }
 
 template <class T>
-__global__ __launch_bounds__(256) void colsum_kernel(const T* x, int ld, int M, int D, float* out, int rows_per_y) {
+__device__ __forceinline__ void colsum_body(int bx, int by, const T* x, int ld, int M, int D, float* out, int rows_per_y) {
     __shared__ float red[8][32];
-    const int col = blockIdx.x * 32 + (threadIdx.x & 31);
+    const int col = bx * 32 + (threadIdx.x & 31);
     const int rg = threadIdx.x >> 5;
-    const int m0 = blockIdx.y * rows_per_y;
+    const int m0 = by * rows_per_y;
     const int m1 = (m0 + rows_per_y < M) ? m0 + rows_per_y : M;
     float s = 0.f;
-    if (col < D)
-        for (int m = m0 + rg; m < m1; m += 8) s += Elt<T>::to_f32(x[(long long)m * ld + col]);
+    if (col < D) {
+        int m = m0 + rg;
+        for (; m + 56 < m1; m += 64) {
+            T v[8];
+            DPC_UNROLL
+            for (int j = 0; j < 8; ++j) v[j] = x[(long long)(m + 8 * j) * ld + col];
+            DPC_UNROLL
+            for (int j = 0; j < 8; ++j) s += Elt<T>::to_f32(v[j]);
+        }
+        for (; m < m1; m += 8) s += Elt<T>::to_f32(x[(long long)m * ld + col]);
+    }
     red[rg][threadIdx.x & 31] = s;
     __syncthreads();
     if (threadIdx.x < 32 && col < D) {
         float t = 0.f;
         DPC_UNROLL
         for (int g = 0; g < 8; ++g) t += red[g][threadIdx.x];
-        out[(long long)blockIdx.y * D + col] = t;
+        out[(long long)by * D + col] = t;
     }
 }
+template <class T>
+__global__ __launch_bounds__(256) void colsum_kernel(const T* x, int ld, int M, int D, float* out, int rows_per_y) {
+    colsum_body<T>((int)blockIdx.x, (int)blockIdx.y, x, ld, M, D, out, rows_per_y);
+}
 
-__global__ void colsum_finish_kernel(const float* ws, int ny, int D, float* out, int accumulate) {
-    const int d = blockIdx.x * blockDim.x + threadIdx.x;
+__device__ __forceinline__ void colsum_finish_body(int bx, const float* ws, int ny, int D, float* out, int accumulate) {
+    const int d = bx * blockDim.x + threadIdx.x;
     if (d >= D) return;
     float t = 0.f;
-    for (int y = 0; y < ny; ++y) t += ws[(long long)y * D + d];
+    int y = 0;
+    for (; y + 8 <= ny; y += 8) {
+        float v[8];
+        DPC_UNROLL
+        for (int j = 0; j < 8; ++j) v[j] = ws[(long long)(y + j) * D + d];
+        DPC_UNROLL
+        for (int j = 0; j < 8; ++j) t += v[j];
+    }
+    for (; y < ny; ++y) t += ws[(long long)y * D + d];
     out[d] = accumulate ? out[d] + t : t;
+}
+__global__ void colsum_finish_kernel(const float* ws, int ny, int D, float* out, int accumulate) {
+    colsum_finish_body((int)blockIdx.x, ws, ny, D, out, accumulate);
+}
+
+struct ColsumGroup {
+    dpc_colsum_entry e[DPC_GROUP_MAX];
+    int ny[DPC_GROUP_MAX], rpy[DPC_GROUP_MAX];
+    long long ws_off[DPC_GROUP_MAX];
+    int block0[DPC_GROUP_MAX + 1], fblock0[DPC_GROUP_MAX + 1];
+    int n;
+};
+template <class T>
+__global__ __launch_bounds__(256) void colsum_group_kernel(ColsumGroup G, float* ws) {
+    const int b = (int)blockIdx.x;
+    int i = 0;
+    while (i + 1 < G.n && b >= G.block0[i + 1]) ++i;
+    const dpc_colsum_entry& e = G.e[i];
+    const int gx = (e.D + 31) / 32, loc = b - G.block0[i];
+    colsum_body<T>(loc % gx, loc / gx, (const T*)e.x, e.ld, e.M, e.D, ws + G.ws_off[i], G.rpy[i]);
+}
+__global__ __launch_bounds__(256) void colsum_group_finish_kernel(ColsumGroup G, const float* ws) {
+    const int b = (int)blockIdx.x;
+    int i = 0;
+    while (i + 1 < G.n && b >= G.fblock0[i + 1]) ++i;
+    const dpc_colsum_entry& e = G.e[i];
+    colsum_finish_body(b - G.fblock0[i], ws + G.ws_off[i], G.ny[i], e.D, e.out, e.accumulate);
+}
+
+static inline int colsum_slices(int M) {
+    int ny = (M + 255) / 256;
+    return ny > 64 ? 64 : ny;
+}
+
+extern "C" int dpc_colsum_group(const dpc_colsum_entry* entries, int32_t n, int32_t dtype, float* ws, int64_t ws_floats,
+                                dpc_stream_t stream_) {
+    hipStream_t stream = (hipStream_t)stream_;
+    if (!entries || n <= 0 || n > DPC_GROUP_MAX || (dtype != DPC_F32 && dtype != DPC_BF16)) return DPC_ERR_ARG;
+    ColsumGroup G;
+    G.n = n; G.block0[0] = 0; G.fblock0[0] = 0;
+    long long off = 0;
+    for (int i = 0; i < n; ++i) {
+        const dpc_colsum_entry& e = entries[i];
+        if (!e.x || !e.out || e.M <= 0 || e.D <= 0 || e.ld < e.D) return DPC_ERR_ARG;
+        G.e[i] = e;
+        G.ny[i] = colsum_slices(e.M);
+        G.rpy[i] = (e.M + G.ny[i] - 1) / G.ny[i];
+        G.ws_off[i] = off;
+        off += (long long)G.ny[i] * e.D;
+        G.block0[i + 1] = G.block0[i] + (e.D + 31) / 32 * G.ny[i];
+        G.fblock0[i + 1] = G.fblock0[i] + (e.D + 255) / 256;
+    }
+    if (!ws || ws_floats < off) return DPC_ERR_ARG;
+    for (int i = n; i < DPC_GROUP_MAX; ++i) {
+        G.e[i] = G.e[0]; G.ny[i] = 0; G.rpy[i] = 0; G.ws_off[i] = 0;
+        G.block0[i + 1] = G.block0[n]; G.fblock0[i + 1] = G.fblock0[n];
+    }
+    if (dtype == DPC_F32) {
+        DPC_LAUNCH((colsum_group_kernel<float>), dim3((unsigned)G.block0[n]), dim3(256), stream, G, ws);
+    } else {
+        DPC_LAUNCH((colsum_group_kernel<bf16_t>), dim3((unsigned)G.block0[n]), dim3(256), stream, G, ws);
+    }
+    DPC_LAUNCH(colsum_group_finish_kernel, dim3((unsigned)G.fblock0[n]), dim3(256), stream, G, (const float*)ws);
+    return dpc_launch_status();
 }
 
 extern "C" int dpc_colsum(const void* x, int32_t dtype, int32_t ld, int32_t M, int32_t D, float* out, int32_t accumulate,
                           float* ws, int64_t ws_floats, dpc_stream_t stream_) {
     hipStream_t stream = (hipStream_t)stream_;
     if (!x || !out || M <= 0 || D <= 0 || ld < D) return DPC_ERR_ARG;
-    int ny = (M + 255) / 256;
-    if (ny > 64) ny = 64;
+    const int ny = colsum_slices(M);
     if (!ws || ws_floats < (long long)ny * D) return DPC_ERR_ARG;
     const int rpy = (M + ny - 1) / ny;
     dim3 grid((D + 31) / 32, ny), block(256);
diff --git a/dpc_amd/csrc/pack.hip b/dpc_amd/csrc/pack.hip
--- a/dpc_amd/csrc/pack.hip
+++ b/dpc_amd/csrc/pack.hip
@@ -90,12 +90,12 @@
     return dpc_launch_status();
 }
 
-__global__ __launch_bounds__(256) void reduce_unpack_kernel(const float* part, int nsplit, float* out, int d0, int d1, int d2, long long s0,
-                                     long long s1, long long s2, int accumulate) {
+__device__ __forceinline__ void reduce_unpack_body(unsigned bid, const float* part, int nsplit, float* out, int d0, int d1, int d2, long long s0,
+                                                   long long s1, long long s2, int accumulate) {
     __shared__ float red[8][32];
     const long long n = (long long)d0 * d1 * d2;
     const int ol = threadIdx.x & 31, sl = threadIdx.x >> 5;
-    const long long i = (long long)blockIdx.x * 32 + ol;
+    const long long i = (long long)bid * 32 + ol;
     float s = 0.f;
     if (i < n)
         for (int k = sl; k < nsplit; k += 8) s += part[(long long)k * n + i];
@@ -113,13 +113,17 @@
         *o = accumulate ? (*o + t) : t;
     }
 }
-
-__global__ __launch_bounds__(256) void reduce_unpack4_kernel(const float* part, int nsplit, float* out, int d0, int d1, int d2, long long s0,
-                                      long long s1, long long s2, int accumulate) {
+__global__ __launch_bounds__(256) void reduce_unpack_kernel(const float* part, int nsplit, float* out, int d0, int d1, int d2, long long s0,
+                                     long long s1, long long s2, int accumulate) {
+    reduce_unpack_body(blockIdx.x, part, nsplit, out, d0, d1, d2, s0, s1, s2, accumulate);
+}
+
+__device__ __forceinline__ void reduce_unpack4_body(unsigned bid, const float* part, int nsplit, float* out, int d0, int d1, int d2, long long s0,
+                                                    long long s1, long long s2, int accumulate) {
     __shared__ float red[8][32][4];
     const long long n = (long long)d0 * d1 * d2;
     const int ol = threadIdx.x & 31, sl = threadIdx.x >> 5;
-    const long long i = ((long long)blockIdx.x * 32 + ol) * 4;
+    const long long i = ((long long)bid * 32 + ol) * 4;
     float acc[8][4];
     DPC_UNROLL
     for (int j = 0; j < 8; ++j)
@@ -168,12 +172,16 @@
         }
     }
 }
+__global__ __launch_bounds__(256) void reduce_unpack4_kernel(const float* part, int nsplit, float* out, int d0, int d1, int d2, long long s0,
+                                      long long s1, long long s2, int accumulate) {
+    reduce_unpack4_body(blockIdx.x, part, nsplit, out, d0, d1, d2, s0, s1, s2, accumulate);
+}
 
 template <int NS>
-__global__ __launch_bounds__(256) void reduce_unpack_few_kernel(const float* part, float* out, int d0, int d1, int d2, long long s0, long long s1,
-                                                                long long s2, int accumulate) {
+__device__ __forceinline__ void reduce_unpack_few_body(unsigned bid, const float* part, float* out, int d0, int d1, int d2, long long s0, long long s1,
+                                                       long long s2, int accumulate) {
     const long long n = (long long)d0 * d1 * d2;
-    const long long i = ((long long)blockIdx.x * 256 + threadIdx.x) * 4;
+    const long long i = ((long long)bid * 256 + threadIdx.x) * 4;
     if (i >= n) return;
     u32x4 v[NS];
     DPC_UNROLL
@@ -190,6 +198,11 @@
         for (int k = 0; k < NS; ++k) t += unit_get<float>(v[k], e);
         o[e * s2] = accumulate ? (o[e * s2] + t) : t;
     }
+}
+template <int NS>
+__global__ __launch_bounds__(256) void reduce_unpack_few_kernel(const float* part, float* out, int d0, int d1, int d2, long long s0, long long s1,
+                                                                long long s2, int accumulate) {
+    reduce_unpack_few_body<NS>(blockIdx.x, part, out, d0, d1, d2, s0, s1, s2, accumulate);
 }
 
 constexpr int RUT_CW = 64, RUT_MAXT = 32;
@@ -225,29 +238,85 @@
     }
 }
 
+enum { RU_GENERIC = 0, RU_X4 = 1, RU_FEW = 2 };
+static inline bool reduce_is_transposing(int nsplit, int d0, int d1, int d2, int64_t s0, int64_t s1, int64_t s2) {
+    return nsplit <= 16 && d1 > 1 && d1 <= RUT_MAXT && s1 == 1 && s2 == d1 && s0 == (int64_t)d1 * d2 && d0 <= 65535;
+}
+static inline int reduce_kind(const float* part, int nsplit, int d2) {
+    if (d2 % 4 == 0 && ((uintptr_t)part % 16) == 0) return nsplit <= 8 ? RU_FEW : RU_X4;
+    return RU_GENERIC;
+}
+static inline unsigned reduce_blocks(int kind, long long n) {
+    if (kind == RU_FEW) return (unsigned)((n / 4 + 255) / 256);
+    if (kind == RU_X4) return (unsigned)((n / 4 + 31) / 32);
+    return (unsigned)((n + 31) / 32);
+}
+
 extern "C" int dpc_reduce_unpack(const float* part, int32_t nsplit, float* out, int32_t d0, int32_t d1, int32_t d2,
                                  int64_t s0, int64_t s1, int64_t s2, int32_t accumulate, dpc_stream_t stream_) {
     hipStream_t stream = (hipStream_t)stream_;
     if (!part || !out || nsplit <= 0 || d0 <= 0 || d1 <= 0 || d2 <= 0) return DPC_ERR_ARG;
-    if (nsplit <= 16 && d1 > 1 && d1 <= RUT_MAXT && s1 == 1 && s2 == d1 && s0 == (int64_t)d1 * d2 && d0 <= 65535) {
+    if (reduce_is_transposing(nsplit, d0, d1, d2, s0, s1, s2)) {
         DPC_LAUNCH(reduce_unpack_t_kernel, dim3((unsigned)d0, (unsigned)((d2 + RUT_CW - 1) / RUT_CW)), dim3(256), stream, part, nsplit, out, d0, d1, d2,
                    accumulate);
         return dpc_launch_status();
     }
     const long long n = (long long)d0 * d1 * d2;
-    if (d2 % 4 == 0 && ((uintptr_t)part % 16) == 0 && nsplit <= 8) {
-        const dim3 grid((unsigned)((n / 4 + 255) / 256)), block(256);
+    const int kind = reduce_kind(part, nsplit, d2);
+    if (kind == RU_FEW) {
+        const dim3 grid(reduce_blocks(kind, n)), block(256);
 #define DPC_RUF(NS) case NS: DPC_LAUNCH((reduce_unpack_few_kernel<NS>), grid, block, stream, part, out, d0, d1, d2, (long long)s0, (long long)s1, (long long)s2, accumulate); break
         switch (nsplit) { DPC_RUF(1); DPC_RUF(2); DPC_RUF(3); DPC_RUF(4); DPC_RUF(5); DPC_RUF(6); DPC_RUF(7); DPC_RUF(8); }
 #undef DPC_RUF
         return dpc_launch_status();
     }
-    if (d2 % 4 == 0 && ((uintptr_t)part % 16) == 0) {
-        DPC_LAUNCH(reduce_unpack4_kernel, dim3((unsigned)((n / 4 + 31) / 32)), dim3(256), stream, part, nsplit, out, d0, d1, d2, (long long)s0, (long long)s1,
+    if (kind == RU_X4) {
+        DPC_LAUNCH(reduce_unpack4_kernel, dim3(reduce_blocks(kind, n)), dim3(256), stream, part, nsplit, out, d0, d1, d2, (long long)s0, (long long)s1,
                    (long long)s2, accumulate);
         return dpc_launch_status();
     }
-    DPC_LAUNCH(reduce_unpack_kernel, dim3((unsigned)((n + 31) / 32)), dim3(256), stream, part, nsplit, out, d0, d1, d2, (long long)s0, (long long)s1, (long long)s2, accumulate);
+    DPC_LAUNCH(reduce_unpack_kernel, dim3(reduce_blocks(kind, n)), dim3(256), stream, part, nsplit, out, d0, d1, d2, (long long)s0, (long long)s1, (long long)s2, accumulate);
+    return dpc_launch_status();
+}
+
+struct ReduceGroup {
+    dpc_reduce_entry e[DPC_GROUP_MAX];
+    int kind[DPC_GROUP_MAX];
+    unsigned block0[DPC_GROUP_MAX + 1];
+    int n;
+};
+__global__ __launch_bounds__(256) void reduce_unpack_group_kernel(ReduceGroup G) {
+    const unsigned b = blockIdx.x;
+    int i = 0;
+    while (i + 1 < G.n && b >= G.block0[i + 1]) ++i;
+    const dpc_reduce_entry& e = G.e[i];
+    const unsigned bid = b - G.block0[i];
+    if (G.kind[i] == RU_FEW) {
+#define DPC_RUF(NS) case NS: reduce_unpack_few_body<NS>(bid, e.part, e.out, e.d0, e.d1, e.d2, (long long)e.s0, (long long)e.s1, (long long)e.s2, e.accumulate); break
+        switch (e.nsplit) { DPC_RUF(1); DPC_RUF(2); DPC_RUF(3); DPC_RUF(4); DPC_RUF(5); DPC_RUF(6); DPC_RUF(7); DPC_RUF(8); }
+#undef DPC_RUF
+    } else if (G.kind[i] == RU_X4) {
+        reduce_unpack4_body(bid, e.part, e.nsplit, e.out, e.d0, e.d1, e.d2, (long long)e.s0, (long long)e.s1, (long long)e.s2, e.accumulate);
+    } else {
+        reduce_unpack_body(bid, e.part, e.nsplit, e.out, e.d0, e.d1, e.d2, (long long)e.s0, (long long)e.s1, (long long)e.s2, e.accumulate);
+    }
+}
+
+extern "C" int dpc_reduce_unpack_group(const dpc_reduce_entry* entries, int32_t n, dpc_stream_t stream_) {
+    hipStream_t stream = (hipStream_t)stream_;
+    if (!entries || n <= 0 || n > DPC_GROUP_MAX) return DPC_ERR_ARG;
+    ReduceGroup G;
+    G.n = n; G.block0[0] = 0;
+    for (int i = 0; i < n; ++i) {
+        const dpc_reduce_entry& e = entries[i];
+        if (!e.part || !e.out || e.nsplit <= 0 || e.d0 <= 0 || e.d1 <= 0 || e.d2 <= 0) return DPC_ERR_ARG;
+        if (reduce_is_transposing(e.nsplit, e.d0, e.d1, e.d2, e.s0, e.s1, e.s2)) return DPC_ERR_UNSUPPORTED;
+        G.e[i] = e;
+        G.kind[i] = reduce_kind(e.part, e.nsplit, e.d2);
+        G.block0[i + 1] = G.block0[i] + reduce_blocks(G.kind[i], (long long)e.d0 * e.d1 * e.d2);
+    }
+    for (int i = n; i < DPC_GROUP_MAX; ++i) { G.e[i] = G.e[0]; G.kind[i] = G.kind[0]; G.block0[i + 1] = G.block0[n]; }
+    DPC_LAUNCH(reduce_unpack_group_kernel, dim3(G.block0[n]), dim3(256), stream, G);
     return dpc_launch_status();
 }
 
diff --git a/dpc_amd/engine.py b/dpc_amd/engine.py
--- a/dpc_amd/engine.py
+++ b/dpc_amd/engine.py
@@ -4,6 +4,7 @@
 import contextlib
 import ctypes as C
 import os
+import types
 import weakref
 import math
 from typing import Dict, List, Optional, Sequence, Tuple
@@ -427,7 +428,7 @@
     def __init__(self, shapes: "Dict[str, Tuple[int, ...]]", network: str, sample_size: int, num_seq: int, seq_len: int, batch: int,
                  device, compute_dtype, widths: Sequence[int], lib: Optional[L.Lib], lr: float, wd: float, gru_dropout: float, seed: int,
                  stem_fused: bool | None = None, fold: bool | None = None, reserve_cus: int | None = None,
-                 f32_matmul: str | None = None, bn_running: bool = False):
+                 f32_matmul: str | None = None, bn_running: bool = False, head_grouped: bool = True):
         self.device = torch.device(device)
         self.lib = L.lib_for(self.device, lib)
         self.cdtype = compute_dtype
@@ -466,6 +467,8 @@
 
         self._want_stem_fused = bool(int(os.environ.get("DPC_STEM_FUSED", "1"))) if stem_fused is None else bool(stem_fused)
         self.fold = bool(int(os.environ.get("DPC_FOLD", "1"))) if fold is None else bool(fold)
+        self._want_head_grouped = bool(head_grouped)
+        self._head_gemms, self._head_colsums, self._head_group = [], [], None
         self.reserve_cus = int(os.environ.get("DPC_RESERVE_CUS", "0")) if reserve_cus is None else int(reserve_cus)
         mm = (f32_matmul or os.environ.get("DPC_F32_MATMUL", "exact")).lower()
         if mm not in ("exact", "bf16x6"):
@@ -553,6 +556,10 @@
             self._need_wgrad(ns * M, co, kk)
         self.need_part(64 * 3 * D)
         self._gate_table = None
+        self._head_gemms += [(self.G_all, 3 * D, self.X_all, D, self.dWx, ns * M, 3 * D, D),
+                             (self.G_all, 3 * D, self.H_all, D, self.dWh, ns * M, 2 * D, D),
+                             (self.G_all[:, :, 2 * D:], 3 * D, self.HR_all, D, self.dWo, ns * M, D, D)]
+        self._head_colsums += [(self.G_all, 3 * D, ns * M, 3 * D, self.db)]
         gd, Pm = L.GruChainDesc(), self.PRM
         gd.dtype, gd.M, gd.D, gd.SQ, gd.P, gd.n_agg, gd.n_steps = L.dtype_code(dt), M, D, SQ, P, n_agg, ns
         gd.p_drop, gd.seed = float(self.p_drop), self.seed
@@ -565,11 +572,21 @@
         self.gru_desc = gd
 
     def _gru_param_grads(self, dc):
-        D, M, ns, Gm = self.D, self.M, self.n_steps, self.G
+        if self._use_head_group():
+            self._param_grads_grouped(dc)
+        else:
+            self._gru_param_grads_single(dc)
+
+    def _gru_param_grads_single(self, dc):
+        D, M, ns = self.D, self.M, self.n_steps
         self.gemm_tn(self.G_all, 3 * D, self.X_all, D, self.dWx, ns * M, 3 * D, D)
         self.gemm_tn(self.G_all, 3 * D, self.H_all, D, self.dWh, ns * M, 2 * D, D)
         self.gemm_tn(self.G_all[:, :, 2 * D:], 3 * D, self.HR_all, D, self.dWo, ns * M, D, D)
         self.call("dpc_colsum", self.G_all, dc, 3 * D, ns * M, 3 * D, self.db, 0, self.part, self.part.numel())
+        self._gate_scatter()
+
+    def _gate_scatter(self):
+        D, Gm = self.D, self.G
         if self._gate_table is None:
             ents = []
             for i, (g, n) in enumerate((("u", "update_gate"), ("r", "reset_gate"), ("o", "out_gate"))):
@@ -586,6 +603,50 @@
             self._gate_table = (raw.to(self.device), len(ents), blk)
         self.call("dpc_copy2d_multi", *self._gate_table)
 
+    def _plan_head_group(self):
+        gm = self._head_gemms
+        if not self._want_head_grouped or not gm or len(gm) > L.GROUP_MAX:
+            return
+        n = len(gm)
+        g = types.SimpleNamespace(n=n)
+        g.descs = (L.ConvDesc * n)(*[self._gemm_desc(M, Co, K, x_ld, K, Co) for (_, _, _, x_ld, _, M, Co, K) in gm])
+        g.dy = (C.c_void_p * n)(*[t[0].data_ptr() for t in gm])
+        g.src = (C.c_void_p * n)(*[t[2].data_ptr() for t in gm])
+        g.dy_ld = (C.c_int32 * n)(*[t[1] for t in gm])
+        g.off, g.ns = (C.c_int64 * (n + 1))(), (C.c_int32 * n)()
+        rc = self.lib._fn("dpc_gemm_tn_group")(g.descs, n, None, None, g.dy_ld, None, g.off, g.ns, self.lib.stream())
+        if rc == L.ERR_UNSUPPORTED:
+            return
+        if rc < 0:
+            raise L.DpcError(f"dpc_gemm_tn_group failed with code {rc}")
+        self.need_part(g.off[n])
+        self.need_part(sum(min((M + 255) // 256, 64) * D for (_, _, M, D, _) in self._head_colsums))
+        self._head_group = g
+
+    def _bind_head_group(self):
+        g = self._head_group
+        if g is None:
+            return
+        g.red = {}
+        for part in {self._part_main.data_ptr(): self._part_main, self._part_side.data_ptr(): self._part_side}.values():
+            ents = (L.ReduceEntry * g.n)()
+            for i, (_, _, _, _, out, _, Co, K) in enumerate(self._head_gemms):
+                ents[i] = L.ReduceEntry(part.data_ptr() + 4 * g.off[i], out.data_ptr(), g.ns[i], Co, 1, K, K, 0, 1, 0, 0)
+            g.red[part.data_ptr()] = ents
+        cs = self._head_colsums
+        g.ncs = len(cs)
+        g.cs = (L.ColsumEntry * g.ncs)(*[L.ColsumEntry(x.data_ptr(), out.data_ptr(), ld, M, D, 0) for (x, ld, M, D, out) in cs])
+
+    def _use_head_group(self) -> bool:
+        return self._head_group is not None and self.timer is None
+
+    def _param_grads_grouped(self, dc):
+        g, part = self._head_group, self.part
+        self.call("dpc_gemm_tn_group", g.descs, g.n, g.src, g.dy, g.dy_ld, part, g.off, g.ns)
+        self.call("dpc_reduce_unpack_group", g.red[part.data_ptr()], g.n)
+        self.call("dpc_colsum_group", g.cs, g.ncs, dc, part, part.numel())
+        self._gate_scatter()
+
     def dropout_masks_of_step(self) -> torch.Tensor:
         buf = self.empty((self.n_steps, self.M, self.D), torch.float32)
         self.call("dpc_dropout_mask", buf, buf.numel(), float(self.p_drop), self.seed, self.dev_draw)
@@ -593,6 +654,7 @@
 
     def _finish_buffers(self):
         widths, dt, f32 = self.widths, self.cdtype, torch.float32
+        self._plan_head_group()
         prs = C.c_int32(0)
         ps_ = self.pool_shape
         self.lib.call("dpc_pooled_bn_bwd_reduce", None, None, None, L.dtype_code(dt), ps_[0] * ps_[1] * ps_[2] * ps_[3], widths[0],
@@ -615,6 +677,7 @@
             self.stem_dz = None
         else:
             self.stem_dz = self.empty(tuple(self.stem.raw.shape), dt)
+        self._bind_head_group()
         self.packed_for_step = -1
 
     @property
@@ -1618,11 +1681,11 @@
                  pred_step: int = 3, batch: int = 4, device="cuda", compute_dtype=torch.float32,
                  widths: Sequence[int] = LAYER_WIDTH, lib: Optional[L.Lib] = None,
                  lr: float = 1e-3, wd: float = 1e-5, dropout: float = 0.1, seed: int = 233, score_path: str = "auto", stem_fused: bool | None = None,
-                 fold: bool | None = None, reserve_cus: int | None = None, f32_matmul: str | None = None):
+                 fold: bool | None = None, reserve_cus: int | None = None, f32_matmul: str | None = None, head_grouped: bool = True):
         self.P = pred_step
         self.score_mode = "materialised"
         super().__init__(param_shapes(network, widths), network, sample_size, num_seq, seq_len, batch, device, compute_dtype, widths, lib,
-                         lr, wd, dropout, seed, stem_fused, fold, reserve_cus, f32_matmul)
+                         lr, wd, dropout, seed, stem_fused, fold, reserve_cus, f32_matmul, head_grouped=head_grouped)
         self._build_head(score_path)
         self._finish_buffers()
 
@@ -1678,6 +1741,10 @@
         for name, t in (("bias_1", Pm["network_pred.0.bias"]), ("bias_2", Pm["network_pred.2.bias"]), ("P1_all", self.P1_all),
                         ("pred", self.pred), ("d_pred", self.d_pred), ("dP1", self.dP1), ("dP2", self.dP2)):
             setattr(gd, name, t.data_ptr())
+        Gm = self.G
+        self._head_gemms += [(self.dP1, D, self.Hpred, D, Gm["network_pred.0.weight"].view(D, D), P * M, D, D),
+                             (self.dP2, D, self.P1_all, D, Gm["network_pred.2.weight"].view(D, D), P * M, D, D)]
+        self._head_colsums += [(self.dP1, D, P * M, D, Gm["network_pred.0.bias"]), (self.dP2, D, P * M, D, Gm["network_pred.2.bias"])]
 
     def forward(self, block: torch.Tensor, train: bool = False, dropout_masks: Optional[torch.Tensor] = None,
                 materialise: bool = True, new_draw: bool = True):
@@ -1786,7 +1853,10 @@
 
     def _head_param_grads(self, dc):
         D, M, P, Gm = self.D, self.M, self.P, self.G
-        self._gru_param_grads(dc)
+        if self._use_head_group():
+            self._param_grads_grouped(dc)
+            return
+        self._gru_param_grads_single(dc)
         self.gemm_tn(self.dP1, D, self.Hpred, D, Gm["network_pred.0.weight"].view(D, D), P * M, D, D)
         self.gemm_tn(self.dP2, D, self.P1_all, D, Gm["network_pred.2.weight"].view(D, D), P * M, D, D)
         self.call("dpc_colsum", self.dP1, dc, D, P * M, D, Gm["network_pred.0.bias"], 0, self.part, self.part.numel())
diff --git a/dpc_amd/lc.py b/dpc_amd/lc.py
--- a/dpc_amd/lc.py
+++ b/dpc_amd/lc.py
@@ -42,11 +42,11 @@
     def __init__(self, network: str = "resnet18", sample_size: int = 128, num_seq: int = 8, seq_len: int = 5, batch: int = 4,
                  device="cuda", compute_dtype=torch.float32, widths: Sequence[int] = LAYER_WIDTH, lib: Optional[L.Lib] = None,
                  lr: float = 1e-3, wd: float = 1e-3, dropout: float = 0.5, num_class: int = 101, gru_dropout: float = 0.1,
-                 seed: int = 666):
+                 seed: int = 666, head_grouped: bool = True):
         self.num_class = int(num_class)
         self.p_drop_fc = float(dropout)
         super().__init__(lc_param_shapes(network, self.num_class, widths), network, sample_size, num_seq, seq_len, batch, device,
-                         compute_dtype, widths, lib, lr, wd, gru_dropout, seed, bn_running=True)
+                         compute_dtype, widths, lib, lr, wd, gru_dropout, seed, bn_running=True, head_grouped=head_grouped)
         self._build_head()
         self._finish_buffers()
 
diff --git a/include/dpc_hip.h b/include/dpc_hip.h
--- a/include/dpc_hip.h
+++ b/include/dpc_hip.h
@@ -52,6 +52,24 @@
 
 int dpc_conv_wgrad(const dpc_conv_desc* d, const void* src, const void* dy, int32_t dy_ld,
                    float* part, int32_t* nsplit, dpc_stream_t stream);
+
+#define DPC_GROUP_MAX 8
+int dpc_gemm_tn_group(const dpc_conv_desc* descs, int32_t n, const void* const* src, const void* const* dy, const int32_t* dy_ld,
+                      float* part, int64_t* part_off, int32_t* nsplit, dpc_stream_t stream);
+typedef struct dpc_reduce_entry {
+    const float* part;
+    float* out;
+    int32_t nsplit, d0, d1, d2;
+    int64_t s0, s1, s2;
+    int32_t accumulate, reserved;
+} dpc_reduce_entry;
+int dpc_reduce_unpack_group(const dpc_reduce_entry* entries, int32_t n, dpc_stream_t stream);
+typedef struct dpc_colsum_entry {
+    const void* x;
+    float* out;
+    int32_t ld, M, D, accumulate;
+} dpc_colsum_entry;
+int dpc_colsum_group(const dpc_colsum_entry* entries, int32_t n, int32_t dtype, float* ws, int64_t ws_floats, dpc_stream_t stream);
 
 #define DPC_PLAN_IGEMM 0
 #define DPC_PLAN_WGRAD 1
```

New measurement: 5091 clips/s (median of 6 runs). No clear change (+0.7%).
